# gradslam/gradslam

Measured on AMD Instinct MI355X. Metric: frames/sec PointFusion 640x480 RGB-D, higher is better.
Workload: dtype f32

## Files before the change

gradslam_amd/_C.py:

```python
import ctypes as C
import os

import torch

_HERE = os.path.dirname(os.path.abspath(__file__))
LIB_PATH = os.environ.get("GRADSLAM_HIP_LIB") or os.path.join(_HERE, "csrc", "libgradslam_hip.so")
if os.environ.get("GRADSLAM_HIP_LIB"):
    import warnings
    warnings.warn("GRADSLAM_HIP_LIB overrides the product library: %s" % LIB_PATH, RuntimeWarning)
ABI_VERSION = 3

_lib = None

_vp, _i64, _i32, _f = C.c_void_p, C.c_int64, C.c_int, C.c_float


class IcpParams(C.Structure):
    _fields_ = [("mode", C.c_int), ("numiters", C.c_int), ("damp", C.c_float),
                ("dist_thresh", C.c_float), ("lambda_max", C.c_float), ("B", C.c_float),
                ("B2", C.c_float), ("nu", C.c_float)]


class MapView(C.Structure):
    _fields_ = [("points", C.c_void_p), ("normals", C.c_void_p), ("colors", C.c_void_p), ("ccounts", C.c_void_p),
# ... 31 lines not shown
                ("depth_bar", C.c_void_p), ("color_bar", C.c_void_p), ("normal_bar", C.c_void_p),
                ("confidence_bar", C.c_void_p), ("points_bar", C.c_void_p), ("normals_bar", C.c_void_p),
                ("colors_bar", C.c_void_p), ("ccounts_bar", C.c_void_p), ("poses_bar", C.c_void_p),
                ("scratch", C.c_void_p)]


_PROTOS = {
    "gs_abi_version": [],
    "gs_last_error": [],
    "gs_scratch_bytes": [_i64, _i64],
    "gs_profile_begin": [_i32],
    "gs_profile_end": [],
    "gs_profile_read": [_i32, C.POINTER(C.c_double), C.POINTER(C.c_int64), C.POINTER(C.c_double)],
    "gs_frame_maps_f32": [_vp, _vp, _i32, _i32, _f, _vp, _vp, _vp, _vp, _vp],
    "gs_global_maps_f32": [_vp, _vp, _vp, _vp, _i32, _i32, _vp, _vp, _vp],
    "gs_alpha_f32": [_vp, _i64, _f, _f, _vp, _vp],
    "gs_alpha_backward_f32": [_vp, _i64, _f, _f, _vp, _vp, _vp, _vp],
    "gs_downsample_frame_f32": [_vp, _vp, _vp, _vp, _i32, _i32, _i32, _vp, _vp, _vp, _vp, _vp, _vp],
    "gs_project_map_f32": [_vp, _i64, _vp, _vp, _i32, _i32, _vp, _vp],
    "gs_active_table_i64": [_vp, _i64, _i32, _i64, _vp, _vp, _vp, _vp],
    "gs_select_targets_f32": [_vp, _i64, _i32, _i32, _vp, _vp, _vp, _vp, _vp, _vp, _i64, _vp, _vp, _vp],
    "gs_downsample_table_f32": [_vp, _i64, _i32, _vp, _vp, _vp, _vp, _vp, _vp, _vp, _vp, _vp],
    "gs_knn1_f32": [_vp, _i64, _vp, _i64, _vp, _vp, _vp, _vp],
    "gs_knn1_grid_scratch_bytes": [_i64, _i64],
    "gs_knn1_grid_f32": [_vp, _i64, _vp, _i64, _vp, _vp, _vp, C.POINTER(C.c_int64), _vp],
    "gs_gauss_newton_rows_f32": [_vp, _i64, _vp, _vp, _i64, _f, _vp, _vp, _vp, _vp, _vp, _vp],
    "gs_solve_normal_eq_f32": [_vp, _vp, _vp, _i64, _i32, _f, _vp, _vp],
    "gs_se3_exp_f32": [_vp, _vp, _vp],
    "gs_se3_exp_backward_f32": [_vp, _vp, _vp, _vp],
    "gs_transform_points_f32": [_vp, _i64, _vp, _vp, _vp],
    "gs_icp_scratch_bytes": [_i64, _i64],
    "gs_icp_f32": [_vp, _i64, _vp, _vp, _i64, _vp, _vp, C.POINTER(IcpParams), _vp, _vp, _vp, _vp],
    "gs_icp_trace_f32": [_vp, _i32, _vp, _vp],
    "gs_icp_dc_f32": [_vp, _i64, _vp, _vp, _vp, _i64, _vp, _vp, _vp, C.POINTER(IcpParams), _vp, _vp, _vp, _vp],
    "gs_frame_maps_backward_f32": [_vp, _vp, _i32, _i32, _f, _vp, _vp, _vp, _vp, _vp, _vp, _vp, _vp],
    "gs_frame_maps_backward_kbar_scratch_bytes": [_i32, _i32],
    "gs_global_maps_backward_f32": [_vp, _vp, _vp, _vp, _i32, _i32, _vp, _vp, _vp],
    "gs_downsample_frame_backward_f32": [_vp, _vp, _i32, _i32, _i32, _vp, _vp, _vp],
    "gs_icp_tape_bytes": [_i64, _i32],
    "gs_icp_tape_f32": [_vp, _i64, _vp, _vp, _i64, _vp, _vp, C.POINTER(IcpParams), _vp, _vp, _vp, _vp, _vp],
    "gs_icp_backward_scratch_bytes": [_i64, _i64],
    "gs_icp_backward_f32": [_vp, _vp, _i64, _vp, _vp, _i64, _vp, C.POINTER(IcpParams), _vp, _vp, _vp, _vp, _vp, _vp,
                            _vp],
    "gs_similar_rows_f32": [_vp, _i64, _vp, _vp, _vp, _vp, _i32, _f, _f, _vp, _vp],
    "gs_best_unique_rows_f32": [_vp, _i64, _vp, _vp, _vp, _i32, _i32, _i64, _vp, _vp, _vp, _vp, _vp],
    "gs_associate_f32": [_vp, _i64, _vp, _vp, _vp, _vp, _vp, _i32, _i32, _f, _f, _vp, _vp, _vp, _vp],
    "gs_best_table_i64": [_vp, _i32, _i32, _i64, _vp, _vp, _vp, _vp],
    "gs_rows_to_best_pix": [_vp, _i64, _i32, _i32, _vp, _vp],
    "gs_fuse_append_f32": [_vp, _vp, _vp, _vp, _i64, _i64, _vp, _vp, _vp, _vp, _vp, _vp, _i32, _i32, _i32,
                           _vp, _vp, _vp],
    "gs_append_valid_f32": [_vp, _vp, _vp, _vp, _i64, _i64, _vp, _vp, _vp, _vp, _vp, _i32, _i32, _vp, _vp, _vp],
    "gs_ingest_depth_u16_f32": [_vp, _i32, _i32, _vp, _i32, _i32, C.c_double, _vp],
    "gs_ingest_color_u8_f32": [_vp, _i32, _i32, _vp, _i32, _i32, _i32, _vp],
    "gs_ingest_frames_native_f32": [_vp, _vp, _i64, _i32, _i32, C.c_double, _i32, _vp, _vp, _vp],
    "gs_host_device_pointer": [_vp, C.POINTER(C.c_void_p)],
    "gs_global_maps_pose_backward_scratch_bytes": [_i32, _i32],
    "gs_global_maps_pose_backward_f32": [_vp, _vp, _vp, _vp, _vp, _i32, _i32, _vp, _vp, _vp],
    "gs_fuse_append_backward_f32": [_vp, _vp, _vp, _vp, _i64, _vp, _vp, _vp, _vp, _vp, _vp, _i32, _i32, _i32, _vp, _vp,
                                    _vp, _vp, _i64, _vp, _vp, _vp, _vp, _vp, _vp, _vp, _vp, _vp, _vp],
    "gs_update_map_scratch_bytes": [_i64, _i32, _i32],
    "gs_update_map_fusion_dc_f32": [_vp, _vp, _vp, _vp, _i64, _vp, _i64, _vp, _vp, _vp, _vp, _vp, _vp, _vp, _i32, _i32,
                                    _f, _f, _i32, _vp, _vp, _vp, _vp, _vp, _vp],
    "gs_icp_map_dc_f32": [_vp, _i64, _vp, _vp, _vp, _vp, _i64, _vp, _i32, _i32, _vp, _vp, C.POINTER(IcpParams), _vp, _vp,
                          _vp],
    "gs_lattice_source_f32": [_vp, _vp, _vp, _i32, _i32, _i32, _vp, _vp],
    "gs_relative_pose_f32": [_vp, _vp, _i64, _vp, _vp],
    "gs_project_map_dc_f32": [_vp, _i64, _vp, _vp, _vp, _i32, _i32, _vp, _vp],
    "gs_select_targets_dc_f32": [_vp, _i64, _vp, _i32, _i32, _vp, _vp, _vp, _vp, _vp, _vp, _i64, _vp, _vp, _vp],
    "gs_associate_dc_f32": [_vp, _i64, _vp, _vp, _vp, _vp, _vp, _vp, _i32, _i32, _f, _f, _vp, _vp, _vp, _vp],
    "gs_fuse_append_dc_f32": [_vp, _vp, _vp, _vp, _i64, _vp, _i64, _vp, _vp, _vp, _vp, _vp, _vp, _i32, _i32, _i32,
                              _vp, _vp, _vp],
    "gs_append_valid_dc_f32": [_vp, _vp, _vp, _vp, _i64, _vp, _i64, _vp, _vp, _vp, _vp, _vp, _i32, _i32, _vp, _vp,
                               _vp],
    "gs_frame_maps_batch_f32": [_vp, _i64, _i64, _vp, _i32, _i32, _i32, _i32, _f, _vp, _vp, _vp, _vp],
    "gs_localize_scratch_bytes": [_i32, _i32, _i32, _i64],
    "gs_localize_batch_f32": [C.POINTER(LocalizeSeq), _i32, _i32, _i32, _i32, C.POINTER(IcpParams), _vp],
    "gs_update_map_fusion_batch_f32": [C.POINTER(UpdateSeq), _i32, _i32, _i32, _f, _f, _i32, _vp],
    "gs_project_points_f32": [_vp, _i32, _i64, _vp, _i64, _vp, _vp],
    "gs_unproject_points_f32": [_vp, _i32, _i64, _vp, _i64, _vp, _vp, _vp],
    "gs_lie_small_f32": [_i32, _vp, _vp, _vp],
    "gs_localize_far_stats_i64": [_vp, _i32, _i32, _i32, _i64, C.POINTER(C.c_int64), _vp],
    "gs_localize_list_stats_i64": [_vp, _i32, _i32, _i32, _i64, C.POINTER(C.c_int64), _vp],
    "gs_localize_solve_stats_i64": [_vp, _i32, _i32, _i32, _i64, C.POINTER(C.c_int64), _vp],
    "gs_pointfusion_step_batch_f32": [C.POINTER(StepSeq), _i32, _i32, _i32, _i32, C.POINTER(IcpParams), _f, _f, _f, _i32, _vp],
    "gs_render_scratch_bytes": [_i32, _i32, _i32],
    "gs_render_map_dc_f32": [C.POINTER(RenderSeq), _i32, _i32, _i32, _i32, _i32, _f, _i32, _vp],
    "gs_render_backward_scratch_bytes": [_i32, _i32, _i32, _i64],
    "gs_render_map_backward_dc_f32": [C.POINTER(RenderBackwardSeq), _i32, _i32, _i32, _i32, _i32, _vp],
}
_RESTYPE = {"gs_last_error": C.c_char_p, "gs_scratch_bytes": _i64, "gs_icp_scratch_bytes": _i64,
            "gs_knn1_grid_scratch_bytes": _i64, "gs_update_map_scratch_bytes": _i64, "gs_global_maps_pose_backward_scratch_bytes": _i64, "gs_icp_tape_bytes": _i64, "gs_icp_backward_scratch_bytes": _i64,
            "gs_localize_scratch_bytes": _i64, "gs_frame_maps_backward_kbar_scratch_bytes": _i64,
            "gs_render_scratch_bytes": _i64, "gs_render_backward_scratch_bytes": _i64}
EXPORTS = tuple(_PROTOS)


class HipExtensionError(RuntimeError):
    pass


def lib():
    global _lib
    if _lib is None:
        if not os.path.exists(LIB_PATH):
            raise HipExtensionError(
                "gradslam_amd: %s is missing. Build it with `python -m gradslam_amd.csrc.build` "
                "(hipcc --offload-arch=gfx950). There is no CPU / PyTorch fallback." % LIB_PATH)
        handle = C.CDLL(LIB_PATH)
        for name, argtypes in _PROTOS.items():
            fn = getattr(handle, name)
            fn.argtypes = argtypes
            fn.restype = _RESTYPE.get(name, C.c_int)
        if handle.gs_abi_version() != ABI_VERSION:
            raise HipExtensionError("libgradslam_hip.so ABI %d != expected %d; rebuild"
                                    % (handle.gs_abi_version(), ABI_VERSION))
        _lib = handle
    return _lib


def check(status, what):
    if status != 0:
        raise HipExtensionError("%s failed (code %d): %s" % (what, status, lib().gs_last_error().decode()))


def require_device(*tensors):
    dev = None
    for t in tensors:
        if t is None:
            continue
        if not t.is_cuda:
            raise HipExtensionError(
                "gradslam_amd kernels run on the GPU only (got a %s tensor). Move the data to a HIP "
                "device; there is no CPU fallback." % t.device)
        if not t.is_contiguous():
            raise HipExtensionError("internal error: non-contiguous tensor passed to the HIP library")
        if dev is None:
            dev = t.device
        elif t.device != dev:
            raise HipExtensionError("tensors live on different devices: %s vs %s" % (dev, t.device))
    return dev


def ptr(t):
    return None if t is None else C.c_void_p(t.data_ptr())


def stream(device):
    return C.c_void_p(torch.cuda.current_stream(device).cuda_stream)


class Workspace:
    _instances = {}

    def __init__(self, device):
        self.device = device
        self._bufs = {}

    @classmethod
    def get(cls, device):
        device = torch.device(device)
        if device.index is None:
            device = torch.device("cuda", torch.cuda.current_device())
        key = (device, torch.cuda.current_stream(device).cuda_stream)
        ws = cls._instances.get(key)
        if ws is None:
            ws = cls._instances[key] = Workspace(device)
# ... 20 lines not shown
```

gradslam_amd/csrc/gs_common.h:

```cpp
#pragma once
#include <hip/hip_runtime.h>
#include <atomic>
#include <stdint.h>
#include <stdio.h>

#include "../../include/gradslam_hip.h"

#define GS_ABI_VERSION 3

constexpr int GS_MAX_BATCH = 8;
struct GsClearJob {
  int n;
  size_t bytes;
  char* ptr[GS_MAX_BATCH];
};
constexpr int GS_CLEAR_ITEMS = 8;
struct GsPixelTables {
  int n;
  uint64_t* key_pix[GS_MAX_BATCH];
  int32_t* best_pix[GS_MAX_BATCH];
  int32_t* any_flag[GS_MAX_BATCH];
  int32_t* call_flag;
};
int gs_frame_maps_batch_clear(const float* depth, int64_t depth_stride_seq, int64_t depth_stride_frame, const float* K16,
                              int n_frames, int frames_per_K, int H, int W, float two_sigma_sq, float* vertex,
                              float* normal, float* alpha, const GsClearJob* job, void* stream,
                              const GsPixelTables* tables = nullptr);

int gs_update_map_fusion_batch_impl(const gs_update_seq* seqs_host, int B, int H, int W, float dist_th, float dot_th,
                                    int renorm_all, void* stream, bool tables_ready);
int32_t* gs_update_map_call_flag(void* scratch_of_first_sequence);
void gs_update_map_tables(void* scratch, int32_t** any_flag, uint64_t** key_pix);

void gs_set_error(const char* fmt, ...);

#define GS_REQUIRE(cond, msg)                  \
  do {                                         \
    if (!(cond)) {                             \
      gs_set_error("%s: %s", __func__, msg);   \
      return GS_ERR_INVALID;                   \
    }                                          \
  } while (0)

#define GS_HIP(call)                                                            \
  do {                                                                          \
    hipError_t e_ = (call);                                                     \
    if (e_ != hipSuccess) {                                                     \
      gs_set_error("%s: %s -> %s", __func__, #call, hipGetErrorString(e_));     \
      return GS_ERR_HIP;                                                        \
    }                                                                           \
  } while (0)

#define GS_LAUNCH_CHECK() GS_HIP(hipGetLastError())

static inline hipStream_t gs_stream(void* s) { return reinterpret_cast<hipStream_t>(s); }
static inline int64_t gs_ceil_div(int64_t a, int64_t b) { return (a + b - 1) / b; }
static inline size_t gs_align(size_t x, size_t a = 256) { return (x + a - 1) / a * a; }

enum GsProfKind { GS_PROF_KNN = 0, GS_PROF_LINEARIZE = 1, GS_PROF_FRAME = 2, GS_PROF_PROJECT = 3,
                  GS_PROF_ASSOC = 4, GS_PROF_FUSE = 5, GS_PROF_COMPACT = 6, GS_PROF_SOLVE = 7, GS_PROF_ICP_FUSED = 8,
                  GS_PROF_KINDS = 9 };
extern std::atomic<bool> g_gs_prof_on;
int gs_prof_open(int kind, double work, hipStream_t st, int launches);
void gs_prof_close(int slot, hipStream_t st);
struct GsProf {
  int slot;
  hipStream_t st;
  GsProf(int kind, double work, hipStream_t s, int launches = 1) : slot(-1), st(s) {
    if (g_gs_prof_on) slot = gs_prof_open(kind, work, s, launches);
  }
  ~GsProf() {
    if (slot >= 0) gs_prof_close(slot, st);
  }
};

#define GS_DEV __device__ __forceinline__

GS_DEV float gs_fma(float a, float b, float c) { return __builtin_fmaf(a, b, c); }

GS_DEV float gs_dot3_fma(float a0, float a1, float a2, float b0, float b1, float b2) {
  float acc = a0 * b0;
  acc = gs_fma(a1, b1, acc);
  acc = gs_fma(a2, b2, acc);
  return acc;
}
GS_DEV float gs_dot3_plain(float a0, float a1, float a2, float b0, float b1, float b2) {
  float p0 = a0 * b0, p1 = a1 * b1, p2 = a2 * b2;
  float s = p0 + p1;
  return s + p2;
}
GS_DEV float gs_norm3(float x, float y, float z) {
  float acc = x * x;
  acc = gs_fma(y, y, acc);
  acc = gs_fma(z, z, acc);
  return __builtin_sqrtf(acc);
}

GS_DEV float gs_expf_spec(float x) {
  if (x < -87.0f) return 0.0f;
  if (x > 88.0f) return __builtin_inff();
  float n = __builtin_rintf(x * 1.44269504088896341f);
  float r = gs_fma(-n, 0.693359375f, x);
  r = gs_fma(-n, -2.12194440e-4f, r);
  float p = 1.9875691500e-4f;
  p = gs_fma(p, r, 1.3981999507e-3f);
  p = gs_fma(p, r, 8.3334519073e-3f);
  p = gs_fma(p, r, 4.1665795894e-2f);
  p = gs_fma(p, r, 1.6666665459e-1f);
  p = gs_fma(p, r, 5.0000001201e-1f);
  float r2 = r * r;
  float y = gs_fma(p, r2, r);
  y = y + 1.0f;
  int32_t bits = __float_as_int(y) + (((int32_t)n) << 23);
  return __int_as_float(bits);
}
// ... 86 lines not shown
```

gradslam_amd/csrc/gs_env.h:

```cpp
#pragma once
#include <stdlib.h>
#include <string.h>

struct GsEnv {
  bool icp_lists;
  int icp_lists_from;
  bool icp_wide;
  bool icp_far;
  bool icp_binned_normals;
  float icp_weak_room;
  bool icp_persist;
  bool icp_lanes_set;
  int icp_lanes;
  int icp_blocks_per_cu;
  const char* icp_timeline;
  const char* icp_persist_timeline;
  bool icp_timeline_it_set; int icp_timeline_it;
  int timeline_it(int numiters) const { return icp_timeline_it_set ? icp_timeline_it : numiters - 1; }
  bool knn_brute;
  int knn_spt;
  bool debug_grid;
};

inline const GsEnv& gs_env() {
  static const GsEnv env = [] {
    const auto num = [](const char* name, int unset) { const char* e = getenv(name); return e ? atoi(e) : unset; };
    GsEnv v;
    v.icp_lists = num("GRADSLAM_HIP_ICP_LISTS", 1) != 0;
    v.icp_lists_from = num("GRADSLAM_HIP_ICP_LISTS_FROM", -1);
    v.icp_wide = num("GRADSLAM_HIP_ICP_WIDE", 1) != 0;
    v.icp_far = num("GRADSLAM_HIP_ICP_FAR", 0) != 0;
    v.icp_binned_normals = num("GRADSLAM_HIP_ICP_BINNED_NORMALS", 1) != 0;
    const char* room = getenv("GRADSLAM_HIP_ICP_WEAK_ROOM");
    v.icp_weak_room = room ? (float)atof(room) : 0.0f;
    if (!(v.icp_weak_room >= 0.0f && v.icp_weak_room < 1.0f)) v.icp_weak_room = 0.0f;
    v.icp_persist = num("GRADSLAM_HIP_ICP_PERSIST", 0) == 1;
    v.icp_lanes_set = getenv("GRADSLAM_HIP_ICP_LANES") != nullptr;
    v.icp_lanes = num("GRADSLAM_HIP_ICP_LANES", 0);
    v.icp_blocks_per_cu = num("GRADSLAM_HIP_ICP_BLOCKS_PER_CU", 0);
    v.icp_timeline = getenv("GRADSLAM_HIP_ICP_TIMELINE");
    v.icp_persist_timeline = getenv("GRADSLAM_HIP_ICP_PERSIST_TIMELINE");
    v.icp_timeline_it_set = getenv("GRADSLAM_HIP_ICP_TIMELINE_IT") != nullptr;
    v.icp_timeline_it = num("GRADSLAM_HIP_ICP_TIMELINE_IT", 0);
    const char* knn = getenv("GRADSLAM_HIP_KNN");
    v.knn_brute = knn && strcmp(knn, "brute") == 0;
    v.knn_spt = num("GRADSLAM_HIP_KNN_SPT", 0);
    v.debug_grid = getenv("GRADSLAM_HIP_DEBUG_GRID") != nullptr;
    return v;
  }();
  return env;
}
```

gradslam_amd/csrc/gs_fuse.hip:

```cpp
#include "gs_assoc_dev.h"
#include "gs_compact.h"

__global__ void __launch_bounds__(256) gs_fuse_init_kernel(int32_t* __restrict__ pix_of, int64_t n,
                                                           int32_t* __restrict__ any_flag) {
  const int64_t i = (int64_t)blockIdx.x * 256 + threadIdx.x;
  if (i == 0) *any_flag = 0;
  if (i < n) pix_of[i] = -1;
}

__global__ void __launch_bounds__(256) gs_fuse_scatter_kernel(const int32_t* __restrict__ best_pix,
                                                              int64_t P, GsCount n_map_c,
                                                              int32_t* __restrict__ pix_of,
                                                              int32_t* __restrict__ any_flag) {
  const int64_t p = (int64_t)blockIdx.x * 256 + threadIdx.x;
  if (p >= P) return;
  const int32_t n = best_pix[p];
  if (n >= 0 && n < gs_count(n_map_c)) {
    pix_of[n] = (int32_t)p;
    *any_flag = 1;
  }
}

struct FrameGlobalMaps {
  const float* __restrict__ gvertex;
// ... 313 lines not shown
                                           void* scratch, void* stream) {
  GS_REQUIRE(H > 0 && W > 0 && n_old >= 0 && n_new >= n_old, "bad sizes");
  GS_REQUIRE(best_pix && gvertex && gnormal && rgb && alpha && depth && P_bar && N_bar && C_bar && F_bar && gvertex_bar &&
                 gnormal_bar && rgb_bar && alpha_bar && scratch,
             "NULL pointer");
  hipStream_t st = gs_stream(stream);
  const int64_t P = (int64_t)H * W;
  GS_HIP(hipMemsetAsync(gvertex_bar, 0, 12 * (size_t)P, st));
  GS_HIP(hipMemsetAsync(gnormal_bar, 0, 12 * (size_t)P, st));
  GS_HIP(hipMemsetAsync(rgb_bar, 0, 12 * (size_t)P, st));
  GS_HIP(hipMemsetAsync(alpha_bar, 0, 4 * (size_t)P, st));
  char* base = reinterpret_cast<char*>(scratch) + gs_cp_scratch_bytes(P > n_old ? P : n_old);
  int32_t* any_flag = reinterpret_cast<int32_t*>(base);
  int32_t* pix_of = reinterpret_cast<int32_t*>(base + 256);
  if (n_old > 0) {
    GS_REQUIRE(points && normals && colors && ccounts && old_points_bar && old_normals_bar && old_colors_bar &&
                   old_ccounts_bar,
               "NULL pointer");
    const GsCount n_old_c{n_old, nullptr};
    hipLaunchKernelGGL(gs_fuse_init_kernel, dim3((unsigned)gs_ceil_div(n_old, 256)), dim3(256), 0, st, pix_of, n_old,
                       any_flag);
    hipLaunchKernelGGL(gs_fuse_scatter_kernel, dim3((unsigned)gs_ceil_div(P, 256)), dim3(256), 0, st, best_pix, P,
                       n_old_c, pix_of, any_flag);
    hipLaunchKernelGGL(gs_fuse_bwd_rows_kernel, dim3((unsigned)gs_ceil_div(n_old, 256)), dim3(256), 0, st, points,
                       normals, colors, ccounts, n_old, pix_of, any_flag, gvertex, gnormal, rgb, alpha, renorm_all, P_bar,
                       N_bar, C_bar, F_bar, old_points_bar, old_normals_bar, old_colors_bar, old_ccounts_bar,
                       gvertex_bar, gnormal_bar, rgb_bar, alpha_bar);
    GS_LAUNCH_CHECK();
  }
  EmitAppendBackward emit{P_bar, N_bar, C_bar, F_bar, n_old, gvertex_bar, gnormal_bar, rgb_bar, alpha_bar};
  int64_t* cnt = reinterpret_cast<int64_t*>(base + 128);
  return gs_compact(P, PredNewPixel{depth, best_pix}, emit, cnt, 0, n_new - n_old, scratch, st);
}

constexpr int32_t MU_TIE_MARK = 0x7fffffff;
struct MuSeq {
  float* points; float* normals; float* colors; float* ccounts;
  GsCount n_map;
  int64_t capacity;
  const float* vertex; const float* normal; const float* depth; const float* rgb; const float* alpha;
  const float* pose16; const float* K16;
  float* gvertex; float* gnormal;
  int32_t* best_pix;
  int64_t* new_count_out;
  int32_t* any_flag;
  uint64_t* key_pix;
  int32_t* tile_counts;
  uint64_t* key_pt;
  int32_t* pix;
  int32_t* pix_of;
};
struct MuBatch {
  int B, H, W, renorm_all;
  int64_t P, ntiles;
  float u_hi, v_hi, dist_th, dot_th;
  int32_t* call_flag;
  int zero_call_flag;
  MuSeq s[GS_MAX_BATCH];
};

__global__ void __launch_bounds__(256) gs_mu_pixel_init_kernel(const MuBatch mb) {
  const MuSeq& q = mb.s[blockIdx.x % mb.B];
  const int64_t p = (int64_t)(blockIdx.x / mb.B) * 256 + threadIdx.x;
  if (p == 0) { q.any_flag[0] = 0; q.any_flag[1] = 0; }
  if (blockIdx.x == 0 && threadIdx.x == 0 && mb.zero_call_flag) *mb.call_flag = 0;
  if (p >= mb.P) return;
  float T[12];
#pragma unroll
  for (int i = 0; i < 12; ++i) T[i] = q.pose16[i];
  const float validf = q.depth[p] > 0.0f ? 1.0f : 0.0f;
  float g0, g1, g2;
  gs_rigid_fma(T, q.vertex[3 * p], q.vertex[3 * p + 1], q.vertex[3 * p + 2], g0, g1, g2);
  q.gvertex[3 * p] = g0 * validf;
  q.gvertex[3 * p + 1] = g1 * validf;
  q.gvertex[3 * p + 2] = g2 * validf;
  const float n0 = q.normal[3 * p], n1 = q.normal[3 * p + 1], n2 = q.normal[3 * p + 2];
  q.gnormal[3 * p] = gs_dot3_fma(T[0], T[1], T[2], n0, n1, n2);
  q.gnormal[3 * p + 1] = gs_dot3_fma(T[4], T[5], T[6], n0, n1, n2);
  q.gnormal[3 * p + 2] = gs_dot3_fma(T[8], T[9], T[10], n0, n1, n2);
  q.key_pix[p] = ~0ull;
  q.best_pix[p] = -1;
}

__global__ void __launch_bounds__(256) gs_mu_project_key_kernel(const MuBatch mb) {
  const MuSeq& q = mb.s[blockIdx.x % mb.B];
  const int64_t n = (int64_t)(blockIdx.x / mb.B) * 256 + threadIdx.x;
  if (n >= gs_count(q.n_map)) return;
  const GsCamera c = gs_camera(q.pose16, q.K16);
  const int32_t p = gs_project_point(c, q.points[3 * n], q.points[3 * n + 1], q.points[3 * n + 2], mb.H, mb.W, mb.u_hi,
                                     mb.v_hi);
  int32_t pk = -1;
  if (p >= 0) {
    float fp[3], fn[3];
    if (q.gvertex) FrameGlobalMaps{q.gvertex, q.gnormal}((int64_t)p, fp, fn);
    else frame_local_maps(q.vertex, q.normal, q.pose16)((int64_t)p, fp, fn);
    if (gs_is_similar_v(q.points, q.normals, fp, fn, n, mb.dist_th, mb.dot_th)) {
      const uint64_t k = gs_assoc_key_v(q.points, q.ccounts, fp, n);
      const unsigned long long old = atomicMin(reinterpret_cast<unsigned long long*>(&q.key_pix[p]), (unsigned long long)k);
      if (old == (unsigned long long)k) {
        q.best_pix[p] = MU_TIE_MARK;
        q.any_flag[1] = 1;
      }
      q.key_pt[n] = k;
      pk = p;
    }
  }
  q.pix[n] = pk;
}

GS_DEV void mu_settle_ties(const MuSeq& q, const unsigned blk, const unsigned nblk) {
  if (q.any_flag[1] == 0) return;
  const int64_t n_map = gs_count(q.n_map);
  for (int64_t n = (int64_t)blk * GS_CP_BLOCK + threadIdx.x; n < n_map; n += (int64_t)nblk * GS_CP_BLOCK) {
    const int32_t p = q.pix[n];
    if (p < 0 || q.best_pix[p] == -1) continue;
    if (q.key_pt[n] == q.key_pix[p]) atomicMin(reinterpret_cast<unsigned*>(&q.best_pix[p]), (unsigned)n);
  }
}

__global__ void __launch_bounds__(GS_CP_BLOCK) gs_mu_winner_count_kernel(const MuBatch mb) {
  __shared__ int smem[GS_CP_BLOCK / GS_WAVE + 1];
  const MuSeq& q = mb.s[blockIdx.x % mb.B];
  const unsigned blk = blockIdx.x / mb.B;
  const int64_t base = (int64_t)blk * GS_CP_TILE + (int64_t)threadIdx.x * GS_CP_ITEMS;
  int c = 0;
  uint64_t kk[GS_CP_ITEMS];
  float dd[GS_CP_ITEMS];
#pragma unroll
  for (int i = 0; i < GS_CP_ITEMS; ++i) {
    const int64_t pc = base + i < mb.P ? base + i : mb.P - 1;
    kk[i] = q.key_pix[pc];
    dd[i] = q.depth[pc];
  }
  bool any = false;
#pragma unroll
  for (int i = 0; i < GS_CP_ITEMS; ++i) {
    const int64_t p = base + i;
    if (p < mb.P) {
      const bool matched = kk[i] != ~0ull;
      any = any || matched;
      if (dd[i] > 0.0f && !matched) ++c;
    }
  }
  if (any) {
    q.any_flag[0] = 1;
    *mb.call_flag = 1;
  }
  int total;
  (void)gs_block_excl_scan<GS_CP_BLOCK>(c, smem, &total);
  if (threadIdx.x == 0) q.tile_counts[blk] = total;
  mu_settle_ties(q, blk, gridDim.x / mb.B);
}

GS_DEV void mu_merge_body(const MuBatch& mb, const unsigned bid) {
  const MuSeq& q = mb.s[bid % mb.B];
  const int64_t n = (int64_t)(bid / mb.B) * 256 + threadIdx.x;
  if (n >= gs_count(q.n_map)) return;
  if (*mb.call_flag == 0) return;
  int32_t p = q.pix[n];
  if (p >= 0) {
    bool win = q.key_pt[n] == q.key_pix[p];
    if (win) {
      const int32_t bp = q.best_pix[p];
      win = bp == -1 || bp == (int32_t)n;
      if (win && bp == -1) q.best_pix[p] = (int32_t)n;
    }
    if (!win) p = -1;
  }
  if (p < 0 && !mb.renorm_all) return;
  if (q.gvertex) fuse_merge_row(q.points, q.normals, q.colors, q.ccounts, n, p, FrameGlobalMaps{q.gvertex, q.gnormal}, q.rgb, q.alpha);
  else fuse_merge_row(q.points, q.normals, q.colors, q.ccounts, n, p, frame_local_maps(q.vertex, q.normal, q.pose16), q.rgb, q.alpha);
}

GS_DEV void mu_append_body(const MuBatch& mb, const unsigned bid) {
  __shared__ int smem[GS_CP_BLOCK / GS_WAVE + 1];
  const MuSeq& q = mb.s[bid % mb.B];
  const unsigned blk = bid / mb.B;
  int before = 0, all = 0;
  for (int64_t t = threadIdx.x; t < mb.ntiles; t += GS_CP_BLOCK) {
    const int v = q.tile_counts[t];
    all += v;
    if (t < (int64_t)blk) before += v;
  }
  int tile_prefix, total_new, tile_new;
  (void)gs_block_excl_scan<GS_CP_BLOCK>(before, smem, &tile_prefix);
  (void)gs_block_excl_scan<GS_CP_BLOCK>(all, smem, &total_new);
  const int64_t n_map = gs_count(q.n_map);
  if (blk == 0 && threadIdx.x == 0) q.new_count_out[0] = n_map + total_new;
  const int64_t base = (int64_t)blk * GS_CP_TILE + (int64_t)threadIdx.x * GS_CP_ITEMS;
  bool keep[GS_CP_ITEMS];
  int c = 0;
  {
    uint64_t kk[GS_CP_ITEMS];
    float dd[GS_CP_ITEMS];
#pragma unroll
    for (int i = 0; i < GS_CP_ITEMS; ++i) {
      const int64_t pc = base + i < mb.P ? base + i : mb.P - 1;
      kk[i] = q.key_pix[pc];
      dd[i] = q.depth[pc];
    }
#pragma unroll
    for (int i = 0; i < GS_CP_ITEMS; ++i) {
      keep[i] = base + i < mb.P && dd[i] > 0.0f && kk[i] == ~0ull;
      c += keep[i] ? 1 : 0;
    }
  }
  int w = gs_block_excl_scan<GS_CP_BLOCK>(c, smem, &tile_new);
  __shared__ unsigned short loc_s[GS_CP_TILE];
#pragma unroll
  for (int i = 0; i < GS_CP_ITEMS; ++i) {
    if (keep[i]) loc_s[w++] = (unsigned short)(threadIdx.x * GS_CP_ITEMS + i);
  }
  __syncthreads();
  const int64_t tile_base = (int64_t)blk * GS_CP_TILE;
  if (q.gvertex) {
    const EmitAppend emit{q.points, q.normals, q.colors, q.ccounts, q.n_map, FrameGlobalMaps{q.gvertex, q.gnormal}, q.rgb, q.alpha};
    for (int r = threadIdx.x; r < tile_new; r += GS_CP_BLOCK) {
      const int64_t pos = (int64_t)tile_prefix + r;
      if (n_map + pos < q.capacity) emit(tile_base + loc_s[r], pos);
    }
  } else {
    const EmitAppendT<FrameLocalMaps> emit{q.points, q.normals, q.colors, q.ccounts, q.n_map,
                                           frame_local_maps(q.vertex, q.normal, q.pose16), q.rgb, q.alpha};
    for (int r = threadIdx.x; r < tile_new; r += GS_CP_BLOCK) {
      const int64_t pos = (int64_t)tile_prefix + r;
      if (n_map + pos < q.capacity) emit(tile_base + loc_s[r], pos);
    }
  }
}

static_assert(GS_CP_BLOCK == 256, "merge and append blocks share a launch");
__global__ void __launch_bounds__(256) gs_mu_merge_append_kernel(const MuBatch mb, const unsigned nb_append) {
  if (blockIdx.x < nb_append) mu_append_body(mb, blockIdx.x);
  else mu_merge_body(mb, blockIdx.x - nb_append);
}

extern "C" int64_t gs_update_map_scratch_bytes(int64_t n_map_bound, int H, int W) {
  const int64_t P = (int64_t)H * W;
  return (int64_t)(256 + gs_align(8 * (size_t)P) + gs_align(4 * (size_t)gs_cp_tiles(P)) +
                   gs_align(8 * (size_t)(n_map_bound > 0 ? n_map_bound : 1)) +
                   2 * gs_align(4 * (size_t)(n_map_bound > 0 ? n_map_bound : 1)) + 4096);
}

int32_t* gs_update_map_call_flag(void* scratch0) { return reinterpret_cast<int32_t*>(scratch0) + 32; }
void gs_update_map_tables(void* scratch, int32_t** any_flag, uint64_t** key_pix) {
  *any_flag = reinterpret_cast<int32_t*>(scratch);
  *key_pix = reinterpret_cast<uint64_t*>(reinterpret_cast<char*>(scratch) + 256);
}

static int update_chunk(const gs_update_seq* seqs, int B, int H, int W, float dist_th, float dot_th, int renorm_all,
                        hipStream_t st, int phase, int32_t* call_flag, bool first_chunk, bool tables_ready) {
  MuBatch mb;
  mb.B = B; mb.H = H; mb.W = W; mb.renorm_all = renorm_all;
  mb.call_flag = call_flag; mb.zero_call_flag = first_chunk ? 1 : 0;
  mb.P = (int64_t)H * W;
  mb.ntiles = gs_cp_tiles(mb.P);
  mb.u_hi = (float)((double)W - 0.999); mb.v_hi = (float)((double)H - 0.999);
  mb.dist_th = dist_th; mb.dot_th = dot_th;
  int64_t n_max = 0;
  double bytes_assoc = 0.0, bytes_fuse = 0.0;
  for (int b = 0; b < B; ++b) {
    const gs_update_seq& u = seqs[b];
    const int64_t n_map = u.map.n_bound;
    n_max = n_map > n_max ? n_map : n_max;
    char* q = reinterpret_cast<char*>(u.scratch);
    MuSeq& m = mb.s[b];
    m.points = u.map.points; m.normals = u.map.normals; m.colors = u.map.colors; m.ccounts = u.map.ccounts;
    m.n_map = GsCount{u.map.n_bound, u.map.n_dev};
    m.capacity = u.map.capacity;
    m.vertex = u.vertex; m.normal = u.normal; m.depth = u.depth; m.rgb = u.rgb; m.alpha = u.alpha;
    m.pose16 = u.pose16; m.K16 = u.K16;
    m.gvertex = u.gvertex; m.gnormal = u.gnormal; m.best_pix = u.best_pix; m.new_count_out = u.new_count_out;
    m.any_flag = reinterpret_cast<int32_t*>(q); q += 256;
    m.key_pix = reinterpret_cast<uint64_t*>(q); q += gs_align(8 * (size_t)mb.P);
    m.tile_counts = reinterpret_cast<int32_t*>(q); q += gs_align(4 * (size_t)mb.ntiles);
    m.key_pt = reinterpret_cast<uint64_t*>(q); q += gs_align(8 * (size_t)(n_map > 0 ? n_map : 1));
    m.pix = reinterpret_cast<int32_t*>(q); q += gs_align(4 * (size_t)(n_map > 0 ? n_map : 1));
    m.pix_of = reinterpret_cast<int32_t*>(q);
    bytes_assoc += 72.0 * (double)n_map;
    bytes_fuse += 104.0 * (double)n_map + 49.0 * (double)mb.P;
  }
  const unsigned uB = (unsigned)B;
  const unsigned pb = uB * (unsigned)gs_ceil_div(mb.P, 256), nb = uB * (unsigned)gs_ceil_div(n_max > 0 ? n_max : 1, 256);
  if (phase == 0) {
    if (!tables_ready) {
      GsProf prof(GS_PROF_FRAME, (double)B * (double)mb.P * 64.0, st);
      hipLaunchKernelGGL(gs_mu_pixel_init_kernel, dim3(pb), dim3(256), 0, st, mb);
    }
    if (n_max > 0) {
      GsProf prof(GS_PROF_ASSOC, bytes_assoc, st, 1);
      hipLaunchKernelGGL(gs_mu_project_key_kernel, dim3(nb), dim3(256), 0, st, mb);
    }
    GsProf prof(GS_PROF_FUSE, bytes_fuse / 3.0, st, 1);
    hipLaunchKernelGGL(gs_mu_winner_count_kernel, dim3(uB * (unsigned)mb.ntiles), dim3(GS_CP_BLOCK), 0, st, mb);
  } else {
    GsProf prof(GS_PROF_FUSE, bytes_fuse * (2.0 / 3.0), st, 1);
    const unsigned nb_append = uB * (unsigned)mb.ntiles;
    hipLaunchKernelGGL(gs_mu_merge_append_kernel, dim3(nb_append + (n_max > 0 ? nb : 0u)), dim3(256), 0, st, mb, nb_append);
  }
  GS_LAUNCH_CHECK();
  return GS_OK;
}

int gs_update_map_fusion_batch_impl(const gs_update_seq* seqs_host, int B, int H, int W, float dist_th, float dot_th,
                                    int renorm_all, void* stream, bool tables_ready) {
  GS_REQUIRE(seqs_host && B > 0 && H > 0 && W > 0, "bad arguments");
  GS_REQUIRE((int64_t)H * W < (1ll << 31), "too large for int32 indices");
  for (int b = 0; b < B; ++b) {
    const gs_update_seq& u = seqs_host[b];
    GS_REQUIRE(u.map.n_bound >= 0 && u.map.n_bound < 0x7fffffff, "bad map size");
    GS_REQUIRE(u.map.capacity >= u.map.n_bound + (int64_t)H * W, "capacity must cover n_bound + H*W rows");
    GS_REQUIRE(u.map.points && u.map.normals && u.map.colors && u.map.ccounts && u.vertex && u.normal && u.depth && u.rgb &&
                   u.alpha && u.pose16 && u.K16 && u.best_pix && u.new_count_out && u.scratch,
               "NULL pointer");
    GS_REQUIRE((u.gvertex && u.gnormal) || (tables_ready && !u.gvertex && !u.gnormal), "gvertex / gnormal: both or none");
    GS_REQUIRE(u.new_count_out != u.map.n_dev, "new_count_out must not alias the map's device count");
  }
  hipStream_t st = gs_stream(stream);
  int32_t* call_flag = gs_update_map_call_flag(seqs_host[0].scratch);
  for (int phase = 0; phase < 2; ++phase) {
    for (int c0 = 0; c0 < B; c0 += GS_MAX_BATCH) {
      const int nb = B - c0 < GS_MAX_BATCH ? B - c0 : GS_MAX_BATCH;
      const int rc = update_chunk(seqs_host + c0, nb, H, W, dist_th, dot_th, renorm_all, st, phase, call_flag, c0 == 0,
                                  tables_ready);
      if (rc != GS_OK) return rc;
    }
  }
  return GS_OK;
}

extern "C" int gs_update_map_fusion_batch_f32(const gs_update_seq* seqs_host, int B, int H, int W, float dist_th,
                                              float dot_th, int renorm_all, void* stream) {
  return gs_update_map_fusion_batch_impl(seqs_host, B, H, W, dist_th, dot_th, renorm_all, stream, false);
}

extern "C" int gs_update_map_fusion_dc_f32(float* points, float* normals, float* colors, float* ccounts,
                                           int64_t n_map_bound, const int64_t* n_map_dev, int64_t capacity,
                                           const float* vertex, const float* normal, const float* depth,
                                           const float* rgb, const float* alpha, const float* pose16,
                                           const float* K16, int H, int W, float dist_th, float dot_th,
                                           int renorm_all, float* gvertex, float* gnormal, int32_t* best_pix,
                                           int64_t* new_count_out, void* scratch, void* stream) {
  gs_update_seq u;
  u.map = gs_map_view{points, normals, colors, ccounts, capacity, n_map_bound, n_map_dev};
  u.vertex = vertex; u.normal = normal; u.depth = depth; u.rgb = rgb; u.alpha = alpha;
  u.pose16 = pose16; u.K16 = K16;
  u.gvertex = gvertex; u.gnormal = gnormal; u.best_pix = best_pix; u.new_count_out = new_count_out; u.scratch = scratch;
  return gs_update_map_fusion_batch_f32(&u, 1, H, W, dist_th, dot_th, renorm_all, stream);
}
```

gradslam_amd/csrc/gs_icp_loop.hip:

```cpp
#include <stdlib.h>
#include <string.h>

#include <memory>
#include <mutex>
#include <type_traits>

#include "gs_env.h"
#include "gs_icp_math.h"
#include "gs_knn.h"
#include "gs_knn_bbox.h"

constexpr int GS_ICP_MAX_ITERS = 1024;
struct GsIcpState {
  IcpSmall s[2];
  float trace[GS_ICP_MAX_ITERS * 12];
};

struct TapePtrs {
  float* src;
  int32_t* idx;
  float* sys;
};
GS_DEV void tape_write_sys(float* __restrict__ sys, int it, const double* S, float damp) {
  float* t = sys + 28 * it;
// ... 659 lines not shown
          rr = (double)res * (double)res;
        }
        const double sum = gs_wave_sum_f64(rr);
        if (wl == 0) red2[wave] = sum;
      }
      __syncthreads();
      if (threadIdx.x < NU && u0 + (int)threadIdx.x < u_last)
        partials_out[(int64_t)(u0 + threadIdx.x) * LIN_NV + 27] = red2[2 * threadIdx.x] + red2[2 * threadIdx.x + 1];
      __syncthreads();
      continue;
    }
    for (int w = threadIdx.x; w < NU * FS_RG * LIN_NV; w += FS_BLOCK) {
      const int i = w % LIN_NV, part = (w / LIN_NV) % FS_RG, un = w / (LIN_NV * FS_RG);
      const int ia = fs_pa(i), ib = fs_pb(i);
      const float* r0 = qa_s[un * FS_QPB + FS_RPG * part];
      double t = (double)r0[ia] * (double)r0[ib];
#pragma unroll
      for (int u = 1; u < FS_RPG; ++u) t += (double)r0[8 * u + ia] * (double)r0[8 * u + ib];
      sub_s[un][part][i] = t;
    }
    __syncthreads();
    if (threadIdx.x < NU * LIN_NV) {
      const int i = threadIdx.x % LIN_NV, un = threadIdx.x / LIN_NV;
      if (u0 + un < u_last) {
        double t = sub_s[un][0][i];
#pragma unroll
        for (int k = 1; k < FS_RG; ++k) t += sub_s[un][k][i];
        partials_out[(int64_t)(u0 + un) * LIN_NV + i] = t;
      }
    }
    __syncthreads();
  } while (!LISTS && (u0 += NU) < u_last);
}

struct IcpHalfBatch {
  int B;
  int upb;
  float weak_room;
  unsigned long long* timeline;
  IcpHalfSeq s[GS_MAX_BATCH];
  IcpHalfLists l[GS_MAX_BATCH];
  IcpHalfWide w[GS_MAX_BATCH];
};
template <bool FULL, int G, bool FAR, int LMODE>
__global__ void __launch_bounds__(FS_BLOCK, 6) gs_icp_half_batch_kernel(const IcpHalfBatch hb, GsCount n_src_c,
                                                                        float dist_thresh, gs_icp_params prm, int it,
                                                                        int rows_in_reduced) {
  const unsigned B = (unsigned)hb.B, blk = blockIdx.x / B, nblk = gridDim.x / B;
  const unsigned X = (GS_XCDS % B == 0) ? GS_XCDS / B : 1u;
#ifdef GS_ICP_TIMELINE
  unsigned long long t0 = 0;
  if (hb.timeline && threadIdx.x == 0) t0 = wall_clock64();
#endif
  icp_half_body<FULL, G, FAR, LMODE>(hb.s[blockIdx.x % B], hb.l[blockIdx.x % B], hb.w[blockIdx.x % B], n_src_c, dist_thresh, prm, it, rows_in_reduced,
                                     gs_xcd_block(blk, nblk, X), hb.upb,
                                     hb.timeline ? hb.timeline + 72 * (size_t)blockIdx.x : nullptr, hb.weak_room);
#ifdef GS_ICP_TIMELINE
  if (hb.timeline && threadIdx.x == 0) {
    unsigned long long* r = hb.timeline + 72 * (size_t)blockIdx.x;
    r[0] = t0;
    r[1] = wall_clock64();
  }
#endif
}

#include "gs_icp_persist.h"

static size_t icp_rows(int64_t n_src) { return (size_t)gs_ceil_div(n_src, FS_QPB); }

struct IcpDevice { int cus = 256; bool ps_fits = false; };
static IcpDevice icp_device() {
  constexpr int MAX_DEV = 64;
  static IcpDevice facts[MAX_DEV]; static std::once_flag asked[MAX_DEV];
  int dev = 0;
  if (hipGetDevice(&dev) != hipSuccess || dev < 0 || dev >= MAX_DEV) return IcpDevice{};
  std::call_once(asked[dev], [dev] {
    int v = 0; hipDeviceProp_t p;
    if (hipDeviceGetAttribute(&v, hipDeviceAttributeMultiprocessorCount, dev) == hipSuccess && v > 0) facts[dev].cus = v;
    facts[dev].ps_fits = hipGetDeviceProperties(&p, dev) == hipSuccess && strncmp(p.gcnArchName, "gfx950", 6) == 0 &&
                         p.multiProcessorCount == (int)(GS_XCDS * PS_CUS_PER_XCD);
  });
  return facts[dev];
}

struct IcpHalfPlan { int G, nb, upb; };
static IcpHalfPlan icp_half_plan(const GsEnv& env, int cus, int64_t n_src, int B, int g_max = 8) {
  const int forced = env.icp_lanes;
  const int nunits = (int)icp_rows(n_src);
  int share = env.icp_blocks_per_cu;
  if (share <= 0) {
    const int NU2 = FS_BLOCK / 2 / FS_QPB;
    share = (nunits + NU2 - 1) / NU2 <= cus / B ? 1 : 2;
  }
  const int budget = (share * cus) / B > 0 ? (share * cus) / B : 1;
  IcpHalfPlan pl{2, 1, 1};
  for (int G = g_max; G >= 2; G >>= 1) {
    const int NU = FS_BLOCK / G / FS_QPB, need = (nunits + NU - 1) / NU;
    if ((forced == 0 && need <= budget) || forced == G || (forced == 0 && G == 2) || (forced > g_max && G == g_max)) {
      pl.G = G;
      pl.nb = need <= budget ? need : budget;
      pl.upb = NU * ((nunits + NU * pl.nb - 1) / (NU * pl.nb));
      pl.nb = (nunits + pl.upb - 1) / pl.upb;
      break;
    }
  }
  return pl;
}

#include "gs_icp_timeline.h"

template <bool FULL>
static void icp_half_launch(const IcpHalfPlan& pl, IcpHalfBatch& hb, GsCount n_src_c, const gs_icp_params* prm, int it,
                            int rows_in_reduced, hipStream_t st, int lmode = 0) {
  hb.upb = pl.upb;
  hb.timeline = icp_tl_arm(FULL, hb.B * pl.nb, it, prm->numiters, st);
  const dim3 grid((unsigned)(hb.B * pl.nb)), block(FS_BLOCK);
  const bool far = hb.s[0].far_cq != nullptr;
#define GS_HALF_LAUNCH(G_, FAR_, LMODE_)                                                                               \
  hipLaunchKernelGGL((gs_icp_half_batch_kernel<FULL, G_, FAR_, LMODE_>), grid, block, 0, st, hb, n_src_c,              \
                     prm->dist_thresh, *prm, it, rows_in_reduced)
#define GS_HALF_LAUNCH_L(G_)                                                 \
  do {                                                                       \
    if (lmode == 2) GS_HALF_LAUNCH(G_, false, 2);                            \
    else if (lmode == 1) GS_HALF_LAUNCH(G_, false, 1);                       \
    else if (lmode == 3 && G_ == 2) GS_HALF_LAUNCH(2, false, 3);             \
    else GS_HALF_LAUNCH(G_, false, 0);                                       \
  } while (0)
  if (pl.G == 8) GS_HALF_LAUNCH_L(8);
  else if (pl.G == 4) { if (far) GS_HALF_LAUNCH(4, true, 0); else GS_HALF_LAUNCH_L(4); }
  else { if (far) GS_HALF_LAUNCH(2, true, 0); else GS_HALF_LAUNCH_L(2); }
#undef GS_HALF_LAUNCH_L
#undef GS_HALF_LAUNCH
  if (hb.timeline && !FULL) icp_tl_dump(hb, pl, lmode, st);
  hb.timeline = nullptr;
}

constexpr int FS_REDUCE_ROWS = 1024;
__global__ void __launch_bounds__(FS_BLOCK) gs_icp_reduce_rows_kernel(const double* __restrict__ partials_in,
                                                                      GsCount n_src_c, double* __restrict__ row_out) {
  __shared__ double S[32];
  __shared__ double sub[FS_BLOCK / 32][32];
  const int nrows = (int)((gs_count(n_src_c) + FS_QPB - 1) / FS_QPB);
  icp_sum_rows<FS_BLOCK>(partials_in, nrows, S, sub);
  if (threadIdx.x < LIN_NV) row_out[threadIdx.x] = S[threadIdx.x];
}

__global__ void __launch_bounds__(FS_BLOCK) gs_icp_finish_kernel(const double* __restrict__ partials_in, GsCount n_src_c,
                                                                 GsIcpState* __restrict__ st, int buf,
                                                                 gs_icp_params prm, const float* __restrict__ compose16,
                                                                 float* __restrict__ out_T16) {
  __shared__ double red[FS_BLOCK / GS_WAVE];
  const int nrows_in = (int)((gs_count(n_src_c) + FS_QPB - 1) / FS_QPB);
  const double e1 = icp_sum_col27<FS_BLOCK>(partials_in, nrows_in, red);
  if (threadIdx.x != 0) return;
  IcpSmall sm = st->s[buf];
  const int it = prm.numiters - 1;
  icp_update_math((float)e1, sm, prm, it < GS_ICP_MAX_ITERS ? st->trace + 12 * it : nullptr);
  st->s[buf ^ 1] = sm;
  icp_write_result(sm, compose16, out_T16);
}

constexpr int LIN_BLOCK = 256;
constexpr int SUM_BLOCK = 1024;

template <bool FULL>
__global__ void __launch_bounds__(LIN_BLOCK) gs_icp_linearize_kernel(
// ... 74 lines not shown
                                                                  GsIcpState* __restrict__ st, gs_icp_params prm,
                                                                  int it, const float* __restrict__ compose16,
                                                                  float* __restrict__ out_T16) {
  __shared__ double red[SUM_BLOCK / GS_WAVE];
  const double e1 = icp_sum_col27<SUM_BLOCK>(partials, nrows, red);
  if (threadIdx.x != 0) return;
  IcpSmall sm = st->s[0];
  icp_update_math((float)e1, sm, prm, it < GS_ICP_MAX_ITERS ? st->trace + 12 * it : nullptr);
  st->s[0] = sm;
  if (it == prm.numiters - 1) icp_write_result(sm, compose16, out_T16);
}

__global__ void gs_icp_init_kernel(GsIcpState* __restrict__ st, const float* __restrict__ init16, float damp,
                                   int numiters, const float* __restrict__ compose16, float* __restrict__ out_T16) {
  if (threadIdx.x != 0) return;
  IcpSmall sm;
  for (int i = 0; i < 16; ++i) {
    sm.T_total[i] = init16[i];
    sm.T_step[i] = init16[i];
    sm.Tr[i] = (i % 5 == 0) ? 1.0f : 0.0f;
  }
  for (int i = 0; i < 8; ++i) sm.xi[i] = 0.0f;
  sm.damp = damp;
  sm.err = 0.0f;
  sm.pad[0] = sm.pad[1] = 0.0f;
  st->s[0] = sm;
  st->s[1] = sm;
  if (numiters == 0) icp_write_result(sm, compose16, out_T16);
}

template <class T>
static T* gs_at(void* base, size_t offset) { return reinterpret_cast<T*>(reinterpret_cast<char*>(base) + offset); }
struct GsTake { size_t end = 0; size_t operator()(size_t n) { end += n; return end - n; } };

constexpr int ICP_ROWRED_DOUBLES = 32;
struct IcpLayout { size_t state, rowred, sync, best, srcA, srcB, partials[2], grid, total; };
static IcpLayout icp_layout(int64_t n_src, int64_t n_tgt) {
  GsTake take;
  IcpLayout L;
  L.state = take(gs_align(sizeof(GsIcpState)));
  L.rowred = take(gs_align(sizeof(double) * ICP_ROWRED_DOUBLES));
  L.sync = L.rowred + sizeof(double) * LIN_NV;
  static_assert(8 * ICP_ROWRED_DOUBLES >= 8 * LIN_NV + 4 * PS_WORDS, "the sync record does not fit behind rowred + LIN_NV");
  L.best = take(gs_align(8 * (size_t)n_src));
  L.srcA = take(gs_align(12 * (size_t)n_src)); L.srcB = take(gs_align(12 * (size_t)n_src));
  for (int k = 0; k < 2; ++k) L.partials[k] = take(gs_align(sizeof(double) * LIN_NV * icp_rows(n_src)));
  L.grid = take(gs_knn_grid_scratch_bytes(n_src, n_tgt));
  L.total = take.end + 4096;
  return L;
}
struct IcpScratch {
  GsIcpState* state;
  double* rowred;
  unsigned* sync;
  unsigned long long* best; float *srcA, *srcB;
  double* partials[2]; void* grid;
};
static IcpScratch icp_carve(void* p, const IcpLayout& L) {
  return IcpScratch{gs_at<GsIcpState>(p, L.state), gs_at<double>(p, L.rowred), gs_at<unsigned>(p, L.sync),
                    gs_at<unsigned long long>(p, L.best), gs_at<float>(p, L.srcA), gs_at<float>(p, L.srcB),
                    {gs_at<double>(p, L.partials[0]), gs_at<double>(p, L.partials[1])}, gs_at<void>(p, L.grid)};
}

extern "C" int64_t gs_icp_scratch_bytes(int64_t n_src, int64_t n_tgt) { return (int64_t)icp_layout(n_src < 1 ? 1 : n_src, n_tgt).total; }

static int icp_tape_finish(void* tape, const GsIcpState* state, int64_t n_src, int numiters, hipStream_t st) {
  GsIcpTape t = gs_icp_tape_carve(tape, n_src, numiters);
  if (numiters > 0)
    GS_HIP(hipMemcpyAsync(t.trace, state->trace, sizeof(float) * 12 * (size_t)numiters, hipMemcpyDeviceToDevice, st));
  return GS_OK;
}

static double icp_alg_bytes(int numiters, int64_t n_slots, int64_t n_queries, int64_t n_binned) {
  const double rows = (double)gs_ceil_div(n_slots, FS_QPB);
  const double full = 12.0 * n_slots + 36.0 * n_queries + 8.0 * LIN_NV * rows + 16.0 * n_binned;
  const double look = 12.0 * n_slots + 24.0 * n_queries + 8.0 * rows + 16.0 * n_binned;
  return (double)numiters * (full + look);
}

static int icp_run(const float* src, int64_t n_src, const float* tgt, const float* tgt_normals,
                   int64_t n_tgt, const float* init16, const float* compose16,
                   const gs_icp_params* prm, float* out_T16, int64_t* out_idx, void* icp_scratch,
                   void* tape, void* stream, const int64_t* n_src_dev = nullptr,
                   const int64_t* n_tgt_dev = nullptr, GsTargetFilter flt = GsTargetFilter{nullptr, 1, 1}) {
  GS_REQUIRE(prm, "params_host must not be NULL");
  GS_REQUIRE(n_src > 0 && n_tgt > 0, "empty point set");
  GS_REQUIRE(n_tgt < 0x7fffffffll && n_src < 0x7fffffffll, "too many points");
  GS_REQUIRE(src && tgt && tgt_normals && init16 && out_T16 && icp_scratch, "NULL pointer");
  GS_REQUIRE(prm->numiters >= 0 && prm->numiters <= GS_ICP_MAX_ITERS, "numiters must be in [0, 1024]");
  GS_REQUIRE(prm->mode == 0 || prm->mode == 1, "mode must be 0 (ICP) or 1 (gradICP)");
  hipStream_t st = gs_stream(stream);
  IcpScratch sc = icp_carve(icp_scratch, icp_layout(n_src, n_tgt));
  hipLaunchKernelGGL(gs_icp_init_kernel, dim3(1), dim3(64), 0, st, sc.state, init16, prm->damp, prm->numiters,
                     compose16, out_T16);
  const bool dev_counts = n_src_dev || n_tgt_dev || flt.pix;
  const bool use_grid = prm->numiters > 0 && (dev_counts || (!gs_env().knn_brute && gs_knn_use_grid(n_src, n_tgt)));
  const GsCount n_src_c{n_src, n_src_dev}, n_tgt_c{n_tgt, n_tgt_dev};
  float* bufs[2] = {sc.srcA, sc.srcB};
  TapePtrs tp = {nullptr, nullptr, nullptr};
  if (tape) {
    GsIcpTape t = gs_icp_tape_carve(tape, n_src, prm->numiters);
    tp.src = t.src; tp.idx = t.idx; tp.sys = t.sys;
  }
  auto cloud = [&](int it) { return tp.src ? tp.src + (size_t)it * 3 * (size_t)n_src : bufs[it & 1]; };
  auto tidx = [&](int it, int which) { return tp.idx ? tp.idx + ((size_t)it * 2 + which) * (size_t)n_src : nullptr; };

  if (use_grid) {
    int rc = gs_knn_grid_build(tgt, n_tgt_c, n_src, sc.grid, st, flt, tgt_normals);
    if (rc != GS_OK) return rc;
    GridMem gm = grid_carve(sc.grid, n_src, n_tgt);
    const int nfs = (int)icp_rows(n_src);
    const bool reduce_rows = nfs > FS_REDUCE_ROWS;
    const float* cur_in = src;
    int h = 0;
    double prof_bytes = 0.0;
    if (g_gs_prof_on) {
      int64_t n_binned = n_tgt;
      if (flt.pix) {
        unsigned hits = 0;
        GS_HIP(hipMemcpyAsync(&hits, gm.bbox + 6, 4, hipMemcpyDeviceToHost, st));
        GS_HIP(hipStreamSynchronize(st));
        n_binned = hits;
      }
      prof_bytes = icp_alg_bytes(prm->numiters, n_src, n_src, n_binned);
    }
    std::unique_ptr<GsProf> prof_loop(new GsProf(GS_PROF_ICP_FUSED, prof_bytes, st, 2 * prm->numiters));
    const IcpHalfPlan plan = icp_half_plan(gs_env(), icp_device().cus, n_src, 1);
    IcpHalfBatch hb;
    hb.B = 1;
    hb.weak_room = 0.0f;
    hb.l[0] = IcpHalfLists{nullptr, nullptr, nullptr, nullptr};
    hb.w[0] = IcpHalfWide{nullptr, nullptr};
    for (int it = 0; it < prm->numiters; ++it) {
      float* cur = cloud(it);
      hb.s[0] = IcpHalfSeq{cur_in, cur, tgt, tgt_normals, n_tgt_c, gm.g, gm.cell_start, gm.sorted, gm.sorted_n,
                           reinterpret_cast<float*>(sc.best), sc.partials[(h + 1) & 1], sc.partials[h & 1], &sc.state->s[h & 1], &sc.state->s[(h + 1) & 1],
                           sc.state->trace, out_idx, tidx(it, 0), nullptr};
      icp_half_launch<true>(plan, hb, n_src_c, prm, it, 0, st);
      ++h;
      if (reduce_rows) {
        GsProf prof(GS_PROF_SOLVE, 1.0, st);
        hipLaunchKernelGGL(gs_icp_reduce_rows_kernel, dim3(1), dim3(FS_BLOCK), 0, st, sc.partials[(h + 1) & 1], n_src_c,
                           sc.rowred);
      }
      hb.s[0] = IcpHalfSeq{cur, nullptr, tgt, tgt_normals, n_tgt_c, gm.g, gm.cell_start, gm.sorted, gm.sorted_n,
                           reinterpret_cast<float*>(sc.best), reduce_rows ? sc.rowred : sc.partials[(h + 1) & 1], sc.partials[h & 1], &sc.state->s[h & 1],
                           &sc.state->s[(h + 1) & 1], sc.state->trace, nullptr, tidx(it, 1), tp.sys};
      icp_half_launch<false>(plan, hb, n_src_c, prm, it, reduce_rows ? 1 : 0, st);
      ++h;
      cur_in = cur;
    }
    prof_loop.reset();
    if (prm->numiters > 0) {
      GsProf prof(GS_PROF_SOLVE, 1.0, st);
      hipLaunchKernelGGL(gs_icp_finish_kernel, dim3(1), dim3(FS_BLOCK), 0, st, sc.partials[(h + 1) & 1], n_src_c,
                         sc.state, h & 1, *prm, compose16, out_T16);
    }
    GS_LAUNCH_CHECK();
    if (tape) return icp_tape_finish(tape, sc.state, n_src, prm->numiters, st);
    return GS_OK;
  }

  GS_HIP(hipMemsetAsync(sc.best, 0xff, 8 * (size_t)n_src, st));
  const int nblk = (int)gs_ceil_div(n_src, LIN_BLOCK);
  double* partials = sc.partials[0];
  const float* cur_in = src;
  for (int it = 0; it < prm->numiters; ++it) {
    float* cur = cloud(it);
    gs_knn_brute_launch(cur_in, sc.state->s[0].T_step, cur, n_src, tgt, n_tgt, sc.best, st);
    {
      GsProf prof(GS_PROF_LINEARIZE, 44.0 * (double)n_src, st);
      hipLaunchKernelGGL((gs_icp_linearize_kernel<true>), dim3(nblk), dim3(LIN_BLOCK), 0, st, cur, nullptr, n_src,
                         tgt, tgt_normals, n_tgt, sc.best, prm->dist_thresh, partials, out_idx, tidx(it, 0));
    }
    {
      GsProf prof(GS_PROF_SOLVE, 1.0, st);
      hipLaunchKernelGGL(gs_icp_solve_kernel, dim3(1), dim3(SUM_BLOCK), 0, st, partials, nblk, sc.state, it, tp.sys);
    }
    gs_knn_brute_launch(cur, sc.state->s[0].Tr, nullptr, n_src, tgt, n_tgt, sc.best, st);
    {
      GsProf prof(GS_PROF_LINEARIZE, 44.0 * (double)n_src, st);
      hipLaunchKernelGGL((gs_icp_linearize_kernel<false>), dim3(nblk), dim3(LIN_BLOCK), 0, st, cur,
                         sc.state->s[0].Tr, n_src, tgt, tgt_normals, n_tgt, sc.best, prm->dist_thresh, partials,
                         nullptr, tidx(it, 1));
    }
    {
      GsProf prof(GS_PROF_SOLVE, 1.0, st);
      hipLaunchKernelGGL(gs_icp_update_kernel, dim3(1), dim3(SUM_BLOCK), 0, st, partials, nblk, sc.state, *prm, it,
                         compose16, out_T16);
    }
    cur_in = cur;
  }
  GS_LAUNCH_CHECK();
  if (tape) return icp_tape_finish(tape, sc.state, n_src, prm->numiters, st);
  return GS_OK;
}

extern "C" int gs_icp_f32(const float* src, int64_t n_src, const float* tgt, const float* tgt_normals,
                          int64_t n_tgt, const float* init16, const float* compose16,
                          const gs_icp_params* prm, float* out_T16, int64_t* out_idx, void* icp_scratch,
                          void* stream) {
  return icp_run(src, n_src, tgt, tgt_normals, n_tgt, init16, compose16, prm, out_T16, out_idx, icp_scratch, nullptr,
                 stream);
}

extern "C" int gs_icp_dc_f32(const float* src, int64_t n_src_bound, const int64_t* n_src_dev, const float* tgt,
                             const float* tgt_normals, int64_t n_tgt_bound, const int64_t* n_tgt_dev,
                             const float* init16, const float* compose16, const gs_icp_params* prm, float* out_T16,
                             int64_t* out_idx, void* icp_scratch, void* stream) {
  return icp_run(src, n_src_bound, tgt, tgt_normals, n_tgt_bound, init16, compose16, prm, out_T16, out_idx,
                 icp_scratch, nullptr, stream, n_src_dev, n_tgt_dev);
}

extern "C" int gs_icp_map_dc_f32(const float* src, int64_t n_src_bound, const int64_t* n_src_dev,
                                 const float* map_points, const float* map_normals, const int32_t* pix,
                                 int64_t n_map_bound, const int64_t* n_map_dev, int W, int ds, const float* init16,
                                 const float* compose16, const gs_icp_params* prm, float* out_T16,
                                 void* icp_scratch, void* stream) {
  GS_REQUIRE(pix && W > 0 && ds > 0, "bad target filter");
  return icp_run(src, n_src_bound, map_points, map_normals, n_map_bound, init16, compose16, prm, out_T16, nullptr,
                 icp_scratch, nullptr, stream, n_src_dev, n_map_dev, GsTargetFilter{pix, W, ds});
}


struct LocSeq {
  const float* vertex;
  const float* depth;
  const float* pose16;
  float* lattice;
  GsIcpState* state;
  float* out_pose16;
  char* clear_ptr;
  int64_t* n_valid;
  int* far_n;
  int* lstat;
  float4* wl_cq;
  unsigned* sync;
};
struct LocBatch {
  int B, W, ds, Wl;
  int64_t n_lat;
  size_t clear_bytes;
  float damp;
  int numiters;
  int count_valid;
  LocSeq s[GS_MAX_BATCH];
};
constexpr int LP_CLEAR_ITEMS = 8;

GS_DEV void loc_prep_block(const LocBatch& lb, const unsigned bid, const unsigned nb_lat) {
  const LocSeq& q = lb.s[bid % lb.B];
  const unsigned blk = bid / lb.B;
  if (blk < nb_lat) {
    const int64_t e = (int64_t)blk * 256 + threadIdx.x;
    int valid = 0;
    if (e < lb.n_lat) {
      const int64_t p = (e / lb.Wl) * lb.ds * (int64_t)lb.W + (e % lb.Wl) * lb.ds;
      float g0 = __builtin_nanf(""), g1 = g0, g2 = g0;
      if (q.depth[p] > 0.0f) {
        float T[12];
#pragma unroll
        for (int i = 0; i < 12; ++i) T[i] = q.pose16[i];
        gs_rigid_fma(T, q.vertex[3 * p], q.vertex[3 * p + 1], q.vertex[3 * p + 2], g0, g1, g2);
        valid = 1;
      }
      q.lattice[3 * e] = g0; q.lattice[3 * e + 1] = g1; q.lattice[3 * e + 2] = g2;
      if (q.wl_cq) q.wl_cq[e] = make_float4(0.0f, 0.0f, 0.0f, 0.0f);
    }
    const unsigned long long m = lb.count_valid ? __ballot(valid) : 0ull;
    if ((threadIdx.x & 63) == 0 && m) atomicAdd(reinterpret_cast<unsigned long long*>(q.n_valid), (unsigned long long)__popcll(m));
    if (blk == 0 && threadIdx.x == 0) {
      IcpSmall sm;
      for (int i = 0; i < 16; ++i) {
        const float id = (i % 5 == 0) ? 1.0f : 0.0f;
        sm.T_total[i] = id; sm.T_step[i] = id; sm.Tr[i] = id;
      }
      for (int i = 0; i < 8; ++i) sm.xi[i] = 0.0f;
      sm.damp = lb.damp;
      sm.err = 0.0f;
      sm.pad[0] = sm.pad[1] = 0.0f;
      q.state->s[0] = sm;
      q.state->s[1] = sm;
      if (q.far_n)
        for (int i = 0; i < FS_FAR_PASSES; ++i) q.far_n[i] = 0;
      if (q.lstat)
        for (int i = 0; i < 3 * GL_STAT_LAUNCHES; ++i) q.lstat[i] = 0;
      if (q.sync)
        for (int i = 0; i < PS_WORDS; ++i) q.sync[i] = 0u;
      if (lb.numiters == 0) icp_write_result(sm, q.pose16, q.out_pose16);
    }
    return;
  }
  float4* dst = reinterpret_cast<float4*>(q.clear_ptr);
  const size_t n16 = lb.clear_bytes / 16;
  const size_t base = (size_t)(blk - nb_lat) * 256 * LP_CLEAR_ITEMS + threadIdx.x;
#pragma unroll
  for (int u = 0; u < LP_CLEAR_ITEMS; ++u) {
    const size_t i = base + (size_t)u * 256;
    if (i < n16) dst[i] = make_float4(0.0f, 0.0f, 0.0f, 0.0f);
  }
}
__global__ void __launch_bounds__(256) gs_loc_prep_kernel(const LocBatch lb, unsigned nb_lat) {
  loc_prep_block(lb, blockIdx.x, nb_lat);
}
static_assert(GB_BLOCK == 256, "lattice and bbox blocks share a launch");
__global__ void __launch_bounds__(256) gs_loc_prep_bbox_kernel(const LocBatch lb, const GsGridBatch gb, const unsigned nb_lat,
                                                               const float u_hi, const float v_hi) {
  const unsigned n_prep = (unsigned)lb.B * nb_lat;
  if (blockIdx.x < n_prep) loc_prep_block(lb, blockIdx.x, nb_lat);
  else gridb_bbox_block(gb, blockIdx.x - n_prep, u_hi, v_hi);
}

struct IcpRowsBatch {
  int B;
  const double* in[GS_MAX_BATCH];
  double* out[GS_MAX_BATCH];
};
__global__ void __launch_bounds__(FS_BLOCK) gs_icp_reduce_rows_batch_kernel(const IcpRowsBatch rb, GsCount n_src_c) {
  __shared__ double S[32];
  __shared__ double sub[FS_BLOCK / 32][32];
  const int nrows = (int)((gs_count(n_src_c) + FS_QPB - 1) / FS_QPB);
  icp_sum_rows<FS_BLOCK>(rb.in[blockIdx.x], nrows, S, sub);
  if (threadIdx.x < LIN_NV) rb.out[blockIdx.x][threadIdx.x] = S[threadIdx.x];
}

struct IcpFinishBatch {
  int B;
  const double* partials_in[GS_MAX_BATCH];
  GsIcpState* st[GS_MAX_BATCH];
  const float* compose16[GS_MAX_BATCH];
  float* out_T16[GS_MAX_BATCH];
  unsigned* sync[GS_MAX_BATCH];
  int nb, h0;
};
__global__ void __launch_bounds__(FS_BLOCK) gs_icp_finish_batch_kernel(const IcpFinishBatch fb, GsCount n_src_c, int buf,
                                                                       gs_icp_params prm) {
  __shared__ double red[FS_BLOCK / GS_WAVE];
  const int b = blockIdx.x;
  const int nrows_in = (int)((gs_count(n_src_c) + FS_QPB - 1) / FS_QPB);
  const double e1 = icp_sum_col27<FS_BLOCK>(fb.partials_in[b], nrows_in, red);
  if (threadIdx.x != 0) return;
  GsIcpState* st = fb.st[b];
  IcpSmall sm = st->s[buf];
  const int it = prm.numiters - 1;
  icp_update_math((float)e1, sm, prm, it < GS_ICP_MAX_ITERS ? st->trace + 12 * it : nullptr);
  st->s[buf ^ 1] = sm;
  icp_write_result(sm, fb.compose16[b], fb.out_T16[b]);
  if (unsigned* sy = fb.sync[b]) {
    const unsigned arrived = sy[PS_ARRIVED], want = (unsigned)fb.nb * (unsigned)(2 * prm.numiters - fb.h0);
    if (!(sy[PS_ERROR] == 0u && arrived == want && sy[PS_TICKET] >= (unsigned)fb.nb))
      for (int i = 0; i < 16; ++i) fb.out_T16[b][i] = __builtin_nanf("");
    sy[PS_NB] = (unsigned)fb.nb;
    sy[PS_H0] = (unsigned)fb.h0;
  }
}

static int64_t loc_lattice(int H, int W, int ds) { return (int64_t)((H + ds - 1) / ds) * ((W + ds - 1) / ds); }

struct ListMem {
  float4* lq;
  uint32_t* ls;
  int* stat;
};

struct FarMem {
  uint32_t* c;
  float4* cq;
  int* idx;
  int* n;
};

struct FarBuildSeq {
  const float* src;
  const int* idx;
  const int* n;
  const GsGrid* gp;
  const int* cell_start;
  const float4* sorted;
  float* d2prev;
  FarMem m;
};
struct FarBuildBatch {
  int B;
  FarBuildSeq s[GS_MAX_BATCH];
};
constexpr int FAR_BLOCK = 512;
constexpr int FAR_BLOCKS_PER_SEQ = 64;
__global__ void __launch_bounds__(FAR_BLOCK) gs_icp_far_build_kernel(const FarBuildBatch fb) {
  const FarBuildSeq& q = fb.s[blockIdx.x % fb.B];
  const int blk = (int)(blockIdx.x / fb.B);
  const int n = *q.n;
  if (blk >= n) return;
  constexpr int NG = FAR_BLOCK / FS_HG;
  __shared__ float qs[NG][3];
  __shared__ float d1_s[NG];
  __shared__ uint8_t flag_s[NG];
  __shared__ int unres_q[NG], sq_s[NG];
  __shared__ int unres_n;
  __shared__ uint32_t stage_s[NG][GS_FAR_SLOTS + 4];
  const GsGrid g = *q.gp;
  const int grp = threadIdx.x / FS_HG, l16 = threadIdx.x & (FS_HG - 1);
  for (int base = blk; base < n; base += FAR_BLOCKS_PER_SEQ * NG) {
    if (threadIdx.x == 0) unres_n = 0;
    __syncthreads();
    const int e = base + grp * FAR_BLOCKS_PER_SEQ;
    if (e < n) {
      const int sq = q.idx[e];
      const float hx = q.src[3 * (int64_t)sq], hy = q.src[3 * (int64_t)sq + 1], hz = q.src[3 * (int64_t)sq + 2];
      const float4 found = q.m.cq[sq];
      const float d1 = sqrtf(found.x);
      const int kdone = (int)found.y;
      if (kdone >= 0) {
        const float R = far_emit_cube<FS_HG>(g, q.cell_start, q.sorted, hx, hy, hz, l16, d1, kdone, stage_s[grp],
                                             reinterpret_cast<int*>(&stage_s[grp][GS_FAR_SLOTS]));
        for (int u = l16; u < GS_FAR_SLOTS; u += FS_HG) q.m.c[GS_FAR_SLOTS * (int64_t)sq + u] = stage_s[grp][u];
        if (l16 == 0) {
          q.m.cq[sq] = make_float4(hx, hy, hz, R);
          if (R > 0.0f) q.d2prev[sq] = __uint_as_float(__float_as_uint(q.d2prev[sq]) | 0x80000000u);
        }
      } else if (l16 == 0) {
        qs[grp][0] = hx; qs[grp][1] = hy; qs[grp][2] = hz;
        d1_s[grp] = d1;
        sq_s[grp] = sq;
        unres_q[atomicAdd(&unres_n, 1)] = grp;
      }
    }
    __syncthreads();
    const int nun = unres_n;
    for (int u = 0; u < nun; u += FS_BQ) {
      const int nq = nun - u < FS_BQ ? nun - u : FS_BQ;
      block_brute_collect_multi<FAR_BLOCK, FS_BQ>(qs, unres_q + u, nq, q.sorted, q.cell_start[g.ncell], d1_s,
                                                  GS_FAR_RADD * g.c, sq_s, q.m.cq, q.m.c, flag_s);
      if ((int)threadIdx.x < nq) {
        const int gq = unres_q[u + threadIdx.x];
        const int s2 = sq_s[gq];
        if (flag_s[gq]) q.d2prev[s2] = __uint_as_float(__float_as_uint(q.d2prev[s2]) | 0x80000000u);
      }
    }
    __syncthreads();
  }
}

static int64_t loc_rows(const gs_map_view& m) { return m.capacity > m.n_bound ? m.capacity : m.n_bound; }

struct LocLayout {
  int64_t n_lat, rows;
  IcpLayout sc;
  size_t lattice, pix, n_valid, icp, lq, ls, lstat, far_c, far_cq, far_idx, far_n, far_out4, total;
};
static LocLayout loc_layout(int64_t n_lat, int64_t rows) {
  GsTake take;
  LocLayout L;
  L.n_lat = n_lat; L.rows = rows > 0 ? rows : 1;
  L.lattice = take(gs_align(12 * (size_t)n_lat));
  L.pix = take(gs_align(4 * (size_t)L.rows));
  L.n_valid = take(256);
  L.sc = icp_layout(n_lat, L.rows);
  L.icp = take(L.sc.total);
  L.lq = take(gs_align(16 * (size_t)n_lat));
  L.ls = take(gs_align(4 * GL_SLOTS * (size_t)n_lat));
  L.lstat = take(gs_align(4 * 3 * GL_STAT_LAUNCHES));
  L.far_c = take(gs_align(4 * GS_FAR_SLOTS * (size_t)n_lat));
  L.far_cq = take(gs_align(16 * (size_t)n_lat));
  L.far_idx = take(gs_align(4 * FS_FAR_PASSES * (size_t)n_lat));
  L.far_n = take(256);
  L.far_out4 = L.far_n + 4 * 8;
  static_assert(FS_FAR_PASSES <= 8, "the far-list counters run into the result words");
  L.total = take.end;
  return L;
}
static bool loc_lists_fit(const LocLayout& L) { return L.total - (L.icp + L.sc.partials[1]) >= sizeof(double) * LIN_NV * FS_BLOCK; }

extern "C" int64_t gs_localize_scratch_bytes(int H, int W, int ds, int64_t n_map_bound) {
  if (H < 1 || W < 1 || ds < 1) return 0;
  return (int64_t)loc_layout(loc_lattice(H, W, ds), n_map_bound).total;
}

struct LocCarve {
  float* lattice; int32_t* pix; int64_t* n_valid;
  IcpScratch sc; GridMem gm; ListMem lm;
  FarMem fm; int* far_out4;
};
static LocCarve loc_carve(void* p, const LocLayout& L) {
  const IcpScratch sc = icp_carve(gs_at<char>(p, L.icp), L.sc);
  return LocCarve{gs_at<float>(p, L.lattice), gs_at<int32_t>(p, L.pix), gs_at<int64_t>(p, L.n_valid), sc,
                  grid_carve(sc.grid, L.n_lat, L.rows),
                  ListMem{gs_at<float4>(p, L.lq), gs_at<uint32_t>(p, L.ls), gs_at<int>(p, L.lstat)},
                  FarMem{gs_at<uint32_t>(p, L.far_c), gs_at<float4>(p, L.far_cq), gs_at<int>(p, L.far_idx), gs_at<int>(p, L.far_n)},
                  gs_at<int>(p, L.far_out4)};
}
static LocCarve loc_carve_of(const void* scratch, int H, int W, int ds, int64_t map_rows) {
  return loc_carve(const_cast<void*>(scratch), loc_layout(loc_lattice(H, W, ds), map_rows));
}

struct IcpEnginePlan {
  bool far_on, wide_on, lists_on, persist_on;
  bool binned_normals;
  bool reduce_rows;
  int lists_from;
  IcpHalfPlan half;
  int ps_it0, ps_nb, ps_upb;
  float weak_room;
  int lmode(int it, bool look_ahead) const {
    if (!lists_on || it < lists_from) return 0;
    if (it > lists_from) return 2;
    return look_ahead ? (persist_on ? 3 : 1) : 0;
  }
};
static IcpEnginePlan icp_engine_plan(const GsEnv& env, const IcpDevice& dev, int B, int64_t n_lat, int numiters,
                                     const LocLayout* layouts) {
  IcpEnginePlan p;
  const int64_t rows = (int64_t)icp_rows(n_lat);
  p.binned_normals = env.icp_binned_normals; p.weak_room = env.icp_weak_room;
  p.lists_from = env.icp_lists_from >= 0 ? env.icp_lists_from : FS_LISTS_FROM;
  p.reduce_rows = rows > FS_REDUCE_ROWS;
  p.far_on = env.icp_far && numiters > 0;
  p.wide_on = env.icp_wide && !p.far_on && numiters > 0;
  p.ps_upb = (int)gs_ceil_div(rows, PS_CUS_PER_XCD);
  p.ps_nb = (int)gs_ceil_div(rows, p.ps_upb > 0 ? p.ps_upb : 1);
  const bool persist_asked = env.icp_persist && env.icp_lists && !p.far_on && B <= (int)GS_XCDS && p.ps_upb <= PS_UPB &&
                             numiters > p.lists_from + 1 && !env.icp_timeline && !env.icp_lanes_set && dev.ps_fits &&
                             p.binned_normals;
  p.half = icp_half_plan(env, dev.cus, n_lat, B, p.far_on ? 4 : (persist_asked ? 2 : 8));
  p.lists_on = env.icp_lists && !p.far_on && p.half.upb * p.half.G * FS_QPB <= FS_BLOCK;
  for (int b = 0; b < B && p.lists_on; ++b) p.lists_on = loc_lists_fit(layouts[b]);
  p.persist_on = persist_asked && p.half.G == 2 && p.lists_on;
  p.ps_it0 = p.persist_on ? p.lists_from + 1 : numiters;
  return p;
}

static void loc_bind(const gs_localize_seq* seqs, int B, int H, int W, int ds, const gs_icp_params* prm,
                     const IcpEnginePlan& plan, LocCarve* c, LocBatch& lb, GsGridBatch& gb) {
  lb.B = gb.B = B; lb.W = gb.W = W; gb.H = H; lb.ds = gb.ds = ds;
  lb.Wl = (W + ds - 1) / ds; lb.n_lat = loc_lattice(H, W, ds); lb.damp = prm->damp; lb.numiters = prm->numiters;
  gb.cells_cap = gs_knn_grid_cells_cap(lb.n_lat);
  for (int b = 0; b < B; ++b) {
    const gs_localize_seq& q = seqs[b];
    if (!plan.binned_normals) c[b].gm.sorted_n = nullptr;
    lb.s[b] = LocSeq{q.vertex, q.depth, q.prev_pose16, c[b].lattice, c[b].sc.state, q.out_pose16,
                     reinterpret_cast<char*>(c[b].gm.g), c[b].n_valid, c[b].fm.n, c[b].lm.stat,
                     plan.wide_on ? c[b].fm.cq : nullptr, c[b].sc.sync};
    gb.s[b] = GsGridSeq{q.map.points, GsCount{q.map.n_bound, q.map.n_dev}, c[b].pix, q.prev_pose16, q.K16,
                        plan.binned_normals ? q.map.normals : nullptr, c[b].gm};
  }
  lb.count_valid = g_gs_prof_on ? 1 : 0;
  lb.clear_bytes = gs_knn_grid_clear_bytes(c[0].gm, gb.cells_cap);
}

static int loc_prep(const gs_localize_seq* seqs, const LocBatch& lb, const GsGridBatch& gb, hipStream_t st, bool grid_cleared) {
  const int B = lb.B;
  if (g_gs_prof_on)
    for (int b = 0; b < B; ++b) GS_HIP(hipMemsetAsync(lb.s[b].n_valid, 0, 8, st));
  const unsigned nb_lat = (unsigned)gs_ceil_div(lb.n_lat, 256);
  const unsigned nb_clear = (unsigned)gs_ceil_div((int64_t)(lb.clear_bytes / 16), 256 * LP_CLEAR_ITEMS);
  double bytes = 0.0;
  for (int b = 0; b < B; ++b) bytes += 28.0 * lb.n_lat + 24.0 * seqs[b].map.n_bound + 16.0 * gb.cells_cap;
  GsProf prof(GS_PROF_COMPACT, bytes, st, grid_cleared ? 4 : 5);
  if (grid_cleared) {
    const float u_hi = (float)((double)gb.W - 0.999), v_hi = (float)((double)gb.H - 0.999);
    hipLaunchKernelGGL(gs_loc_prep_bbox_kernel, dim3((unsigned)B * nb_lat + gs_knn_gridb_bbox_blocks(gb)), dim3(256), 0, st,
                       lb, gb, nb_lat, u_hi, v_hi);
    return gs_knn_grid_build_batch(gb, st, true);
  }
  hipLaunchKernelGGL(gs_loc_prep_kernel, dim3((unsigned)B * (nb_lat + nb_clear)), dim3(256), 0, st, lb, nb_lat);
  return gs_knn_grid_build_batch(gb, st);
}

static int loc_prof_bytes(int B, const LocCarve* c, int64_t n_lat, int numiters, hipStream_t st, double* bytes) {
  for (int b = 0; b < B; ++b) {
    unsigned hits = 0; int64_t nv = 0;
    GS_HIP(hipMemcpyAsync(&hits, c[b].gm.bbox + 6, 4, hipMemcpyDeviceToHost, st));
    GS_HIP(hipMemcpyAsync(&nv, c[b].n_valid, 8, hipMemcpyDeviceToHost, st));
    GS_HIP(hipStreamSynchronize(st));
    *bytes += icp_alg_bytes(numiters, n_lat, nv, hits);
  }
  return GS_OK;
}

static void loc_half_iterations(const gs_localize_seq* seqs, int B, const IcpEnginePlan& plan, const LocCarve* c,
                                int64_t n_lat, const gs_icp_params* prm, hipStream_t st) {
  const GsCount n_src_c{n_lat, nullptr};
  const FarMem no_far{nullptr, nullptr, nullptr, nullptr};
  IcpHalfBatch hb;
  hb.B = B; hb.weak_room = plan.weak_room;
  for (int it = 0; it < plan.ps_it0; ++it) {
    int h = 2 * it;
    for (int b = 0; b < B; ++b) {
      const gs_localize_seq& q = seqs[b];
      const IcpScratch& sc = c[b].sc; const GridMem& gm = c[b].gm;
      const FarMem& fm = plan.far_on ? c[b].fm : no_far;
      const float* cur_in = it == 0 ? c[b].lattice : (((it - 1) & 1) ? sc.srcB : sc.srcA);
      float* cur = (it & 1) ? sc.srcB : sc.srcA;
      hb.s[b] = IcpHalfSeq{cur_in, cur, q.map.points, q.map.normals, GsCount{q.map.n_bound, q.map.n_dev}, gm.g,
                           gm.cell_start, gm.sorted, gm.sorted_n, reinterpret_cast<float*>(sc.best),
                           sc.partials[(h + 1) & 1], sc.partials[h & 1], &sc.state->s[h & 1], &sc.state->s[(h + 1) & 1],
                           sc.state->trace, nullptr, nullptr, nullptr, fm.cq, fm.c, fm.idx, fm.n};
      hb.w[b] = plan.wide_on ? IcpHalfWide{c[b].fm.cq, c[b].fm.c} : IcpHalfWide{nullptr, nullptr};
      hb.l[b] = plan.lists_on ? IcpHalfLists{c[b].lm.lq, c[b].lm.ls, c[b].lm.stat, sc.sync + PS_WEAK}
                              : IcpHalfLists{nullptr, nullptr, nullptr, nullptr};
    }
    icp_half_launch<true>(plan.half, hb, n_src_c, prm, it, 0, st, plan.lmode(it, false));
    if (plan.far_on && fs_far_pass(it) >= 0) {
      const int fp = fs_far_pass(it);
      FarBuildBatch fbb; fbb.B = B;
      for (int b = 0; b < B; ++b)
        fbb.s[b] = FarBuildSeq{(it & 1) ? c[b].sc.srcB : c[b].sc.srcA, c[b].fm.idx + (int64_t)fp * n_lat, c[b].fm.n + fp,
                               c[b].gm.g, c[b].gm.cell_start, c[b].gm.sorted, reinterpret_cast<float*>(c[b].sc.best), c[b].fm};
      hipLaunchKernelGGL(gs_icp_far_build_kernel, dim3((unsigned)B * FAR_BLOCKS_PER_SEQ), dim3(FAR_BLOCK), 0, st, fbb);
    }
    ++h;
    if (plan.reduce_rows) {
      IcpRowsBatch rb; rb.B = B;
      for (int b = 0; b < B; ++b) { rb.in[b] = c[b].sc.partials[(h + 1) & 1]; rb.out[b] = c[b].sc.rowred; }
      hipLaunchKernelGGL(gs_icp_reduce_rows_batch_kernel, dim3((unsigned)B), dim3(FS_BLOCK), 0, st, rb, n_src_c);
    }
    for (int b = 0; b < B; ++b) {
      const IcpScratch& sc = c[b].sc;
      IcpHalfSeq& u = hb.s[b];
      u.src_in = (it & 1) ? sc.srcB : sc.srcA; u.src_out = nullptr;
      u.partials_in = plan.reduce_rows ? sc.rowred : sc.partials[(h + 1) & 1];
      u.partials_out = sc.partials[h & 1];
      u.st_in = &sc.state->s[h & 1]; u.st_out = &sc.state->s[(h + 1) & 1];
    }
    icp_half_launch<false>(plan.half, hb, n_src_c, prm, it, plan.reduce_rows ? 1 : 0, st, plan.lmode(it, true));
  }
// ... 67 lines not shown
  GS_REQUIRE((int64_t)H * W < (1ll << 31), "image too large for int32 pixel ids");
  for (int b = 0; b < B; ++b) {
    const gs_localize_seq& q = seqs_host[b];
    GS_REQUIRE(q.vertex && q.depth && q.K16 && q.prev_pose16 && q.out_pose16 && q.scratch, "NULL pointer");
    GS_REQUIRE(q.map.points && q.map.normals && q.map.n_bound > 0 && q.map.n_bound < 0x7fffffffll,
               "every sequence needs a non-empty map (points + normals)");
    GS_REQUIRE(q.map.capacity <= 0 || q.map.n_bound <= q.map.capacity, "map.n_bound exceeds map.capacity");
  }
  hipStream_t st = gs_stream(stream);
  for (int c0 = 0; c0 < B; c0 += GS_MAX_BATCH) {
    const int nb = B - c0 < GS_MAX_BATCH ? B - c0 : GS_MAX_BATCH;
    const int rc = localize_chunk(seqs_host + c0, nb, H, W, ds, prm, st, grid_cleared);
    if (rc != GS_OK) return rc;
  }
  return GS_OK;
}
extern "C" int gs_localize_batch_f32(const gs_localize_seq* seqs_host, int B, int H, int W, int ds,
                                     const gs_icp_params* prm, void* stream) {
  return localize_batch(seqs_host, B, H, W, ds, prm, stream, false);
}

__global__ void __launch_bounds__(256) gs_far_stats_kernel(const int* __restrict__ far_idx, const int* __restrict__ far_n,
                                                          const float* __restrict__ d2prev, const float4* __restrict__ far_cq,
                                                          int64_t n_lat, int* __restrict__ out4) {
  const int n0 = far_n[0], n = n0 < 0 ? 0 : (n0 > (int)n_lat ? (int)n_lat : n0);
  if (blockIdx.x == 0 && threadIdx.x == 0) { out4[0] = n; out4[2] = far_n[1]; }
  int c = 0, built = 0;
  for (int i = blockIdx.x * 256 + threadIdx.x; i < n; i += gridDim.x * 256) {
    const int s = far_idx[i];
    if (s < 0 || s >= (int)n_lat) continue;
    c += (__float_as_uint(d2prev[s]) >> 31) ? 1 : 0;
    built += far_cq[s].w > 0.0f ? 1 : 0;
  }
  if (c) atomicAdd(&out4[1], c);
  if (built) atomicAdd(&out4[3], built);
}
extern "C" int gs_localize_far_stats_i64(const void* scratch, int H, int W, int ds, int64_t map_rows, int64_t* out4_host,
                                         void* stream) {
  GS_REQUIRE(scratch && out4_host && H > 0 && W > 0 && ds > 0 && map_rows > 0, "bad arguments");
  const int64_t n_lat = loc_lattice(H, W, ds);
  const LocCarve cv = loc_carve_of(scratch, H, W, ds, map_rows);
  const FarMem& fm = cv.fm; hipStream_t st = gs_stream(stream);
  int* out4 = cv.far_out4;
  GS_HIP(hipMemsetAsync(out4, 0, 16, st));
  hipLaunchKernelGGL(gs_far_stats_kernel, dim3(64), dim3(256), 0, st, fm.idx, fm.n, reinterpret_cast<const float*>(cv.sc.best),
                     fm.cq, n_lat, out4);
  int h[4] = {0, 0, 0, 0};
  GsGrid g;
  GS_HIP(hipMemcpyAsync(h, out4, 16, hipMemcpyDeviceToHost, st));
  GS_HIP(hipMemcpyAsync(&g, cv.gm.g, sizeof(g), hipMemcpyDeviceToHost, st));
  GS_HIP(hipStreamSynchronize(st));
  for (int i = 0; i < 4; ++i) out4_host[i] = h[i];
  if (gs_env().debug_grid)
    fprintf(stderr, "grid: box (%.3f %.3f %.3f)-(%.3f %.3f %.3f) c %.4f cells %d x %d x %d = %d\n", g.ox, g.oy, g.oz, g.mx,
            g.my, g.mz, g.c, g.nx, g.ny, g.nz, g.ncell);
  return GS_OK;
}

extern "C" int gs_localize_list_stats_i64(const void* scratch, int H, int W, int ds, int64_t map_rows, int64_t* out192_host,
                                          void* stream) {
  GS_REQUIRE(scratch && out192_host && H > 0 && W > 0 && ds > 0 && map_rows > 0, "bad arguments");
  const ListMem lm = loc_carve_of(scratch, H, W, ds, map_rows).lm;
  int h[3 * GL_STAT_LAUNCHES];
  hipStream_t st = gs_stream(stream);
  GS_HIP(hipMemcpyAsync(h, lm.stat, sizeof(h), hipMemcpyDeviceToHost, st));
  GS_HIP(hipStreamSynchronize(st));
  for (int i = 0; i < 3 * GL_STAT_LAUNCHES; ++i) out192_host[i] = h[i];
  return GS_OK;
}

extern "C" int gs_localize_solve_stats_i64(const void* scratch, int H, int W, int ds, int64_t map_rows, int64_t* out8_host,
                                           void* stream) {
  GS_REQUIRE(scratch && out8_host && H > 0 && W > 0 && ds > 0 && map_rows > 0, "bad arguments");
  const LocCarve cv = loc_carve_of(scratch, H, W, ds, map_rows);
  unsigned h[PS_WORDS];
  hipStream_t st = gs_stream(stream);
  GS_HIP(hipMemcpyAsync(h, cv.sc.sync, sizeof(h), hipMemcpyDeviceToHost, st));
  GS_HIP(hipStreamSynchronize(st));
  static_assert(PS_WORDS == 8, "out8");
  for (int i = 0; i < PS_WORDS; ++i) out8_host[i] = h[i];
  return GS_OK;
}

extern "C" int gs_pointfusion_step_batch_f32(const gs_step_seq* seqs_host, int B, int H, int W, int ds,
                                             const gs_icp_params* prm, float two_sigma_sq, float dist_th, float dot_th,
                                             int renorm_all, void* stream) {
  GS_REQUIRE(seqs_host && prm && B > 0 && H > 0 && W > 0 && ds > 0, "bad arguments");
  const int64_t P = (int64_t)H * W;
  const gs_step_seq& s0 = seqs_host[0];
  const int64_t dstride = B > 1 ? seqs_host[1].depth - s0.depth : P;
  for (int b = 0; b < B; ++b) {
    const gs_step_seq& q = seqs_host[b];
    GS_REQUIRE(q.depth && q.rgb && q.K16 && q.prev_pose16 && q.out_pose16 && q.vertex && q.normal && q.alpha &&
                   q.best_pix && q.new_count_out && q.loc_scratch && q.upd_scratch, "NULL pointer");
    GS_REQUIRE((q.gvertex != nullptr) == (q.gnormal != nullptr) && (q.gvertex != nullptr) == (s0.gvertex != nullptr),
               "gvertex / gnormal: both or none, the same choice for every sequence");
    GS_REQUIRE(q.out_pose16 != q.prev_pose16, "out_pose16 must not alias prev_pose16");
    GS_REQUIRE(q.vertex == s0.vertex + 3 * P * b && q.normal == s0.normal + 3 * P * b && q.alpha == s0.alpha + P * b,
               "vertex / normal / alpha of the batch must be dense");
    GS_REQUIRE(q.depth == s0.depth + dstride * b && q.K16 == s0.K16 + 16 * (int64_t)b, "depth / K16 must be equally strided");
  }
  GS_REQUIRE(dstride >= P || B == 1, "overlapping depth images");
  const bool implicit_global = s0.gvertex == nullptr;
  std::unique_ptr<gs_update_seq[]> us(new gs_update_seq[B]);
  for (int c0 = 0; c0 < B; c0 += GS_MAX_BATCH) {
    const int nb = B - c0 < GS_MAX_BATCH ? B - c0 : GS_MAX_BATCH;
    const gs_step_seq* sq = seqs_host + c0;
    gs_localize_seq ls[GS_MAX_BATCH];
    for (int b = 0; b < nb; ++b) {
      const gs_step_seq& q = sq[b];
      ls[b].vertex = q.vertex; ls[b].depth = q.depth; ls[b].K16 = q.K16; ls[b].prev_pose16 = q.prev_pose16;
      ls[b].map = q.map; ls[b].out_pose16 = q.out_pose16; ls[b].scratch = q.loc_scratch;
      gs_update_seq& u = us[c0 + b];
      u.map = q.map; u.vertex = q.vertex; u.normal = q.normal; u.depth = q.depth; u.rgb = q.rgb;
      u.alpha = q.alpha; u.pose16 = q.out_pose16; u.K16 = q.K16; u.gvertex = q.gvertex;
      u.gnormal = q.gnormal; u.best_pix = q.best_pix; u.new_count_out = q.new_count_out;
      u.scratch = q.upd_scratch;
    }
    GsClearJob job;
    job.n = nb;
    for (int b = 0; b < nb; ++b) {
      GS_REQUIRE(ls[b].map.points && ls[b].map.n_bound > 0, "every sequence needs a non-empty map");
      const LocCarve cv = loc_carve_of(ls[b].scratch, H, W, ds, loc_rows(ls[b].map));
      job.ptr[b] = reinterpret_cast<char*>(cv.gm.g);
      if (b == 0) job.bytes = gs_knn_grid_clear_bytes(cv.gm, gs_knn_grid_cells_cap(loc_lattice(H, W, ds)));
    }
    GsPixelTables tabs{};
    tabs.n = implicit_global ? nb : 0;
    tabs.call_flag = c0 == 0 ? gs_update_map_call_flag(seqs_host[0].upd_scratch) : nullptr;
    for (int b = 0; b < tabs.n; ++b) {
      gs_update_map_tables(sq[b].upd_scratch, &tabs.any_flag[b], &tabs.key_pix[b]);
      tabs.best_pix[b] = sq[b].best_pix;
    }
    int rc = gs_frame_maps_batch_clear(sq[0].depth, dstride, P, sq[0].K16, nb, 1, H, W, two_sigma_sq, sq[0].vertex,
                                       sq[0].normal, sq[0].alpha, &job, stream, &tabs);
    if (rc != GS_OK) return rc;
    rc = localize_batch(ls, nb, H, W, ds, prm, stream, true);
    if (rc != GS_OK) return rc;
  }
  return gs_update_map_fusion_batch_impl(us.get(), B, H, W, dist_th, dot_th, renorm_all, stream, implicit_global);
}

extern "C" int64_t gs_icp_tape_bytes(int64_t n_src, int numiters) { return (int64_t)gs_icp_tape_size(n_src, numiters); }

extern "C" int gs_icp_tape_f32(const float* src, int64_t n_src, const float* tgt, const float* tgt_normals,
                               int64_t n_tgt, const float* init16, const float* compose16,
                               const gs_icp_params* prm, float* out_T16, int64_t* out_idx, void* icp_scratch,
                               void* tape, void* stream) {
  GS_REQUIRE(tape, "tape must not be NULL");
  return icp_run(src, n_src, tgt, tgt_normals, n_tgt, init16, compose16, prm, out_T16, out_idx, icp_scratch, tape,
                 stream);
}

extern "C" int gs_icp_trace_f32(const void* icp_scratch, int numiters, float* trace_out, void* stream) {
  GS_REQUIRE(icp_scratch && trace_out && numiters >= 0 && numiters <= GS_ICP_MAX_ITERS, "bad arguments");
  const GsIcpState* st = reinterpret_cast<const GsIcpState*>(icp_scratch);
  GS_HIP(hipMemcpyAsync(trace_out, st->trace, sizeof(float) * 12 * (size_t)numiters, hipMemcpyDeviceToDevice,
                        gs_stream(stream)));
  return GS_OK;
}
```

gradslam_amd/csrc/gs_knn.h:

```cpp
#pragma once
#include "gs_common.h"

GS_DEV unsigned long long knn_pack(float d, uint32_t idx) {
  return ((unsigned long long)__float_as_uint(d) << 32) | (unsigned long long)idx;
}

int gs_knn_brute_launch(const float* src_in, const float* Tapply, float* src_out, int64_t n_src,
                        const float* tgt, int64_t n_tgt, unsigned long long* best, hipStream_t st);

constexpr int GS_GRID_MAXCELL = 1 << 22;
constexpr int GS_GRID_RINGS = 3;
constexpr int GS_GRID_TILE = 1024;

struct GsGrid {
  float ox, oy, oz;
  float mx, my, mz;
  float c, inv_c;
  int nx, ny, nz, ncell;
};

struct GsTargetFilter {
  const int32_t* pix;
  int W, ds;
};
GS_DEV bool gs_is_target(const GsTargetFilter& f, int64_t n) {
  if (!f.pix) return true;
  const int32_t p = f.pix[n];
  return p >= 0 && ((p / f.W) % f.ds == 0) && ((p % f.W) % f.ds == 0);
}

struct GridMem {
  GsGrid* g;
  unsigned* bbox;
  int* unres_count;
  int* cell_count;
  int* cell_start;
  int* tile_sums;
  float4* sorted;
  float4* sorted_n;
  float4* tlist;
  int* unres_list;
};

static inline GridMem grid_carve(void* scratch, int64_t n_src, int64_t n_tgt) {
  char* p = reinterpret_cast<char*>(scratch);
  GridMem m;
  m.g = reinterpret_cast<GsGrid*>(p); p += 128;
  m.bbox = reinterpret_cast<unsigned*>(p); p += 128;
  m.unres_count = reinterpret_cast<int*>(p); p += 256;
  m.tile_sums = reinterpret_cast<int*>(p); p += gs_align(4 * (size_t)(GS_GRID_MAXCELL / GS_GRID_TILE + 2));
  m.cell_count = reinterpret_cast<int*>(p); p += gs_align(4 * (size_t)(GS_GRID_MAXCELL + 1));
  m.cell_start = reinterpret_cast<int*>(p); p += gs_align(4 * (size_t)(GS_GRID_MAXCELL + 1));
  m.sorted = reinterpret_cast<float4*>(p); p += gs_align(16 * (size_t)(n_tgt > 0 ? n_tgt : 1));
  m.sorted_n = reinterpret_cast<float4*>(p); p += gs_align(16 * (size_t)(n_tgt > 0 ? n_tgt : 1));
  m.tlist = reinterpret_cast<float4*>(p); p += gs_align(16 * (size_t)(n_tgt > 0 ? n_tgt : 1));
  m.unres_list = reinterpret_cast<int*>(p);
  (void)n_src;
  return m;
}

size_t gs_knn_grid_scratch_bytes(int64_t n_src, int64_t n_tgt);

struct GsGridSeq {
  const float* tgt;
  GsCount n_tgt;
  int32_t* pix;
  const float* pose16;
  const float* K16;
  const float* nrm;
  GridMem m;
};
struct GsGridBatch {
  int B, H, W, ds;
  int cells_cap;
  GsGridSeq s[GS_MAX_BATCH];
};
int gs_knn_grid_cells_cap(int64_t n_src);
size_t gs_knn_grid_clear_bytes(const GridMem& m, int cells_cap);
int gs_knn_grid_build_batch(const GsGridBatch& gb, hipStream_t st, bool bbox_done = false);

int gs_knn_grid_build(const float* tgt, GsCount n_tgt, int64_t n_src, void* grid_scratch, hipStream_t st,
                      GsTargetFilter filter = GsTargetFilter{nullptr, 1, 1}, const float* nrm = nullptr);
int gs_knn_grid_query(const float* src_in, const float* Tapply, float* src_out, int64_t n_src,
                      const float* tgt, int64_t n_tgt, unsigned long long* best, void* grid_scratch,
                      hipStream_t st);
static inline bool gs_knn_use_grid(int64_t n_src, int64_t n_tgt) { return n_tgt >= 2048 && n_src >= 256; }

GS_DEV int grid_axis(float v, float o, float inv_c, int n) {
  const float f = (v - o) * inv_c;
  return f >= 0.0f ? (f < (float)n ? (int)f : n - 1) : 0;
}
GS_DEV int grid_cell(const GsGrid& g, float x, float y, float z) {
  const int ix = grid_axis(x, g.ox, g.inv_c, g.nx);
  const int iy = grid_axis(y, g.oy, g.inv_c, g.ny);
  const int iz = grid_axis(z, g.oz, g.inv_c, g.nz);
  return (iz * g.ny + iy) * g.nx + ix;
}

constexpr int GQ_G = 8;
constexpr int GL_RING_NF = 2;

GS_DEV unsigned long long grid_key(float qx, float qy, float qz, const float4 p) {
  const float dx = qx - p.x, dy = qy - p.y, dz = qz - p.z;
  float d = dx * dx;
  d = gs_fma(dy, dy, d);
  d = gs_fma(dz, dz, d);
  return d == d ? knn_pack(d, (uint32_t)__float_as_int(p.w)) : ~0ull;
}

template <int G>
GS_DEV unsigned long long grid_group_min(unsigned long long key) {
#pragma unroll
  for (int d = G / 2; d > 0; d >>= 1) {
    const unsigned long long o = __shfl_xor(key, d, G);
    key = o < key ? o : key;
  }
  return key;
}

struct GsQueryCell {
  float px, py, pz;
  int cx, cy, cz;
};
GS_DEV GsQueryCell grid_query_cell(const GsGrid& g, float qx, float qy, float qz) {
  GsQueryCell c;
  c.px = qx < g.ox ? g.ox : (qx > g.mx ? g.mx : qx);
  c.py = qy < g.oy ? g.oy : (qy > g.my ? g.my : qy);
  c.pz = qz < g.oz ? g.oz : (qz > g.mz ? g.mz : qz);
  c.cx = grid_axis(c.px, g.ox, g.inv_c, g.nx); c.cy = grid_axis(c.py, g.oy, g.inv_c, g.ny);
  c.cz = grid_axis(c.pz, g.oz, g.inv_c, g.nz);
  return c;
}

template <int G>
GS_DEV unsigned long long grid_search_stage0(const GsGrid& g, const int* __restrict__ cell_start,
                                             const float4* __restrict__ sorted, float qx, float qy, float qz, int lane,
                                             bool* resolved, int* win, const float rball = __builtin_inff()) {
  const GsQueryCell qc = grid_query_cell(g, qx, qy, qz);
  const float px = qc.px, py = qc.py, pz = qc.pz;
  const int cx = qc.cx, cy = qc.cy, cz = qc.cz;
  unsigned long long key = ~0ull;
  int bt = -1;
  const float fx = (px - g.ox) * g.inv_c - (float)cx, fy = (py - g.oy) * g.inv_c - (float)cy,
              fz = (pz - g.oz) * g.inv_c - (float)cz;
  const int x0 = (fx < 0.5f) ? cx - 1 : cx, y0 = (fy < 0.5f) ? cy - 1 : cy, z0 = (fz < 0.5f) ? cz - 1 : cz;
  const float BIG = 3.0e38f;
  const float ax = fminf(x0 >= 1 ? fx + (float)(cx - x0) : BIG, x0 + 2 < g.nx ? (float)(x0 + 2 - cx) - fx : BIG);
  const float ay = fminf(y0 >= 1 ? fy + (float)(cy - y0) : BIG, y0 + 2 < g.ny ? (float)(y0 + 2 - cy) - fy : BIG);
  const float az = fminf(z0 >= 1 ? fz + (float)(cz - z0) : BIG, z0 + 2 < g.nz ? (float)(z0 + 2 - cz) - fz : BIG);
  const float amin = fminf(ax, fminf(ay, az));
  const float rc = rball * g.inv_c * 1.0001f + 0.002f;
  const bool prune = rc < amin - 0.001f;
  bool ulx = true, uhx = true, uly = true, uhy = true, ulz = true, uhz = true;
  if (prune) {
    const float tx = fx + (float)(cx - x0), ty = fy + (float)(cy - y0), tz = fz + (float)(cz - z0);
    ulx = tx - rc < 1.0f; uhx = tx + rc >= 1.0f;
    uly = ty - rc < 1.0f; uhy = ty + rc >= 1.0f;
    ulz = tz - rc < 1.0f; uhz = tz + rc >= 1.0f;
  }
  int sb0 = 0, sb1 = 0, sb2 = 0, sb3 = 0, e1 = 0, e2 = 0, e3 = 0, total = 0;
  {
    const int xa = (x0 >= 0 && ulx) ? x0 : x0 + 1, xb = (x0 + 1 < g.nx && uhx) ? x0 + 1 : x0;
    const bool zl = z0 >= 0 && ulz, zh = z0 + 1 < g.nz && uhz, yl = y0 >= 0 && uly, yh = y0 + 1 < g.ny && uhy;
    const int r0 = (z0 * g.ny + y0) * g.nx, r1 = r0 + g.nx, r2 = r0 + g.ny * g.nx, r3 = r2 + g.nx;
    int se0 = 0, se1 = 0, se2 = 0, se3 = 0;
// ... 620 lines not shown
```

gradslam_amd/csrc/gs_knn.hip:

```cpp
#include "gs_knn.h"

#include <stdlib.h>

#include "gs_assoc_dev.h"
#include "gs_env.h"
#include "gs_knn_bbox.h"

constexpr int KNN_BLOCK = 256;
constexpr int KNN_TCHUNK = 512;

template <bool LISTED, int KNN_SPT>
__global__ void __launch_bounds__(KNN_BLOCK) gs_knn1_kernel(
    const float* __restrict__ src_in, const float* __restrict__ Tapply, float* __restrict__ src_out,
    int64_t n_src, const float* __restrict__ tgt, int64_t n_tgt, unsigned long long* __restrict__ best,
    const int* __restrict__ list, const int* __restrict__ count) {
  constexpr int KNN_STILE = KNN_BLOCK * KNN_SPT;
  __shared__ float4 tl[KNN_TCHUNK];
  const int64_t n_q = LISTED ? (int64_t)(*count) : n_src;
  if (LISTED && n_q == 0) return;
  const int64_t j0 = (int64_t)blockIdx.y * KNN_TCHUNK;
  const int cnt = (int)((n_tgt - j0) < KNN_TCHUNK ? (n_tgt - j0) : KNN_TCHUNK);
  if (cnt <= 0) return;
  for (int i = threadIdx.x; i < cnt; i += KNN_BLOCK) {
    const float* t = tgt + 3 * (j0 + i);
// ... 3 lines not shown
  if (Tapply) {
#pragma unroll
    for (int i = 0; i < 12; ++i) T[i] = Tapply[i];
  }
  __syncthreads();
  for (int64_t tile = blockIdx.x; tile * KNN_STILE < n_q; tile += gridDim.x) {
    float sx[KNN_SPT], sy[KNN_SPT], sz[KNN_SPT], bd[KNN_SPT];
    int bi[KNN_SPT];
    int64_t sidx[KNN_SPT];
#pragma unroll
    for (int k = 0; k < KNN_SPT; ++k) {
      const int64_t q = tile * KNN_STILE + k * KNN_BLOCK + threadIdx.x;
      int64_t s = -1;
      if (q < n_q) s = LISTED ? (int64_t)list[q] : q;
      float p0 = 0.0f, p1 = 0.0f, p2 = 0.0f;
      if (s >= 0) {
        p0 = src_in[3 * s];
        p1 = src_in[3 * s + 1];
        p2 = src_in[3 * s + 2];
        if (Tapply) {
          float q0, q1, q2;
          gs_rigid_fma(T, p0, p1, p2, q0, q1, q2);
          p0 = q0; p1 = q1; p2 = q2;
        }
        if (!LISTED && src_out && blockIdx.y == 0) {
          src_out[3 * s] = p0;
          src_out[3 * s + 1] = p1;
          src_out[3 * s + 2] = p2;
        }
      }
      sidx[k] = s;
      sx[k] = p0; sy[k] = p1; sz[k] = p2;
      bd[k] = __builtin_inff();
      bi[k] = 0;
    }
#pragma unroll 4
    for (int j = 0; j < cnt; ++j) {
      const float4 t = tl[j];
#pragma unroll
      for (int k = 0; k < KNN_SPT; ++k) {
        const float dx = sx[k] - t.x, dy = sy[k] - t.y, dz = sz[k] - t.z;
        float d = dx * dx;
        d = gs_fma(dy, dy, d);
        d = gs_fma(dz, dz, d);
        const bool lt = d < bd[k];
        bd[k] = lt ? d : bd[k];
        bi[k] = lt ? j : bi[k];
      }
    }
#pragma unroll
    for (int k = 0; k < KNN_SPT; ++k)
      if (sidx[k] >= 0) atomicMin(&best[sidx[k]], knn_pack(bd[k], (uint32_t)(j0 + bi[k])));
    if (!LISTED) break;
  }
}

int gs_knn_brute_launch(const float* src_in, const float* Tapply, float* src_out, int64_t n_src,
                        const float* tgt, int64_t n_tgt, unsigned long long* best, hipStream_t st) {
  const int spt_env = gs_env().knn_spt;
  const int spt = spt_env == 4 || spt_env == 8 ? spt_env : (n_src * n_tgt >= (int64_t)1 << 27 ? 8 : 4);
  GsProf prof(GS_PROF_KNN, (double)n_src * (double)n_tgt, st);
  if (spt == 8) {
    dim3 grid((unsigned)gs_ceil_div(n_src, KNN_BLOCK * 8), (unsigned)gs_ceil_div(n_tgt, KNN_TCHUNK));
    hipLaunchKernelGGL((gs_knn1_kernel<false, 8>), grid, dim3(KNN_BLOCK), 0, st, src_in, Tapply, src_out, n_src, tgt,
                       n_tgt, best, nullptr, nullptr);
  } else {
    dim3 grid((unsigned)gs_ceil_div(n_src, KNN_BLOCK * 4), (unsigned)gs_ceil_div(n_tgt, KNN_TCHUNK));
    hipLaunchKernelGGL((gs_knn1_kernel<false, 4>), grid, dim3(KNN_BLOCK), 0, st, src_in, Tapply, src_out, n_src, tgt,
                       n_tgt, best, nullptr, nullptr);
  }
  return GS_OK;
}

size_t gs_knn_grid_scratch_bytes(int64_t n_src, int64_t n_tgt) {
  return 512 + 2 * gs_align(4 * (size_t)(GS_GRID_MAXCELL + 1)) + gs_align(4 * (size_t)(GS_GRID_MAXCELL / GS_GRID_TILE + 2)) +
         3 * gs_align(16 * (size_t)(n_tgt > 0 ? n_tgt : 1)) + gs_align(4 * (size_t)(n_src > 0 ? n_src : 1)) + 256;
}

__global__ void __launch_bounds__(GB_BLOCK) gs_grid_bbox_kernel(const float* __restrict__ tgt, GsCount n_tgt_c,
                                                                 const GsTargetFilter flt,
                                                                 unsigned* __restrict__ bbox,
                                                                 int* __restrict__ unres_count,
                                                                 float4* __restrict__ tlist) {
  grid_bbox_body(tgt, gs_count(n_tgt_c), flt, nullptr, 0, 0.0f, 0.0f, nullptr, bbox, unres_count, tlist, blockIdx.x);
}

GS_DEV GsGrid grid_from_bbox(const unsigned* __restrict__ bbox, int64_t n_tgt, int cells_cap) {
  float o[3], m[3];
#pragma unroll
  for (int k = 0; k < 3; ++k) {
    const unsigned cl = bbox[k], ch = bbox[3 + k];
    float a = 0.0f, b = 0.0f;
    if (cl != 0u && ch != 0u) { a = grid_decode(~cl); b = grid_decode(ch); }
    o[k] = a; m[k] = b;
  }
  const float tiny = 1e-6f;
  const float ex = (m[0] - o[0]) + tiny, ey = (m[1] - o[1]) + tiny, ez = (m[2] - o[2]) + tiny;
  const float n = (float)(n_tgt > 0 ? n_tgt : 1);
  const float area = ex * ey + ey * ez + ex * ez;
  float c = 1.5f * sqrtf(area / n);
  const float cv = 0.5f * cbrtf((ex * ey * ez) / n);
  c = cv > c ? cv : c;
  const float emax = ex > ey ? (ex > ez ? ex : ez) : (ey > ez ? ey : ez);
  c = c > emax * (1.0f / 1024.0f) ? c : emax * (1.0f / 1024.0f);
  c = c > 1e-6f ? c : 1e-6f;
  int nx, ny, nz;
  for (;;) {
    nx = (int)(ex / c) + 1; ny = (int)(ey / c) + 1; nz = (int)(ez / c) + 1;
    if ((double)nx * (double)ny * (double)nz <= (double)cells_cap) break;
    c *= 1.26f;
  }
  GsGrid g;
  g.ox = o[0]; g.oy = o[1]; g.oz = o[2];
  g.mx = m[0]; g.my = m[1]; g.mz = m[2];
  g.c = c; g.inv_c = 1.0f / c;
  g.nx = nx; g.ny = ny; g.nz = nz; g.ncell = nx * ny * nz;
  return g;
}

GS_DEV void grid_count_body(const float* __restrict__ tgt, const int64_t n_tgt, const GsTargetFilter flt,
                            const unsigned* __restrict__ bbox, GsGrid* __restrict__ gp, int* __restrict__ cell_count,
                            int* __restrict__ tile_sums, int cells_cap, const float4* __restrict__ tlist,
                            const unsigned blk, const unsigned nblk) {
  __shared__ GsGrid gsh;
  __shared__ int th[GS_GRID_MAXCELL / GS_GRID_TILE + 1];
  const int64_t n_items = flt.pix ? (int64_t)bbox[6] : n_tgt;
  if ((int64_t)blk * 256 >= n_items && blk != 0) return;
  if (threadIdx.x == 0) {
    gsh = grid_from_bbox(bbox, n_items, cells_cap);
    if (blk == 0) *gp = gsh;
  }
  __syncthreads();
  const GsGrid g = gsh;
  const int ntile = g.ncell / GS_GRID_TILE + 1;
  for (int t = threadIdx.x; t < ntile; t += 256) th[t] = 0;
  __syncthreads();
  if (flt.pix) {
    for (int64_t i = (int64_t)blk * 256 + threadIdx.x; i < n_items; i += (int64_t)nblk * 256) {
      const float4 t = tlist[i];
      const int cid = grid_cell(g, t.x, t.y, t.z);
      atomicAdd(&cell_count[cid], 1);
      atomicAdd(&th[cid / GS_GRID_TILE], 1);
    }
  } else {
    const int64_t i = (int64_t)blk * 256 + threadIdx.x;
    if (i < n_tgt) {
      const int cid = grid_cell(g, tgt[3 * i], tgt[3 * i + 1], tgt[3 * i + 2]);
      atomicAdd(&cell_count[cid], 1);
      atomicAdd(&th[cid / GS_GRID_TILE], 1);
    }
  }
  __syncthreads();
  for (int t = threadIdx.x; t < ntile; t += 256) {
    const int v = th[t];
    if (v) atomicAdd(&tile_sums[t], v);
  }
}
__global__ void __launch_bounds__(256) gs_grid_count_kernel(const float* __restrict__ tgt, GsCount n_tgt_c,
                                                            const GsTargetFilter flt,
                                                            const unsigned* __restrict__ bbox,
                                                            GsGrid* __restrict__ gp,
                                                            int* __restrict__ cell_count, int* __restrict__ tile_sums,
                                                            int cells_cap, const float4* __restrict__ tlist) {
  grid_count_body(tgt, gs_count(n_tgt_c), flt, bbox, gp, cell_count, tile_sums, cells_cap, tlist, blockIdx.x, gridDim.x);
}

GS_DEV void grid_scan_body(const int* __restrict__ cell_count, const GsGrid* __restrict__ gp,
                           const int* __restrict__ tile_sums, int* __restrict__ cell_start, const unsigned blk) {
  __shared__ int smem[256 / GS_WAVE + 1];
  const int n = gp->ncell + 1;
  if ((int)(blk * GS_GRID_TILE) >= n) return;
  int pre = 0;
  for (int t = threadIdx.x; t < (int)blk; t += 256) pre += tile_sums[t];
  int tile_prefix;
  (void)gs_block_excl_scan<256>(pre, smem, &tile_prefix);
  const int base = blk * GS_GRID_TILE + threadIdx.x * 4;
  int v[4], c = 0;
#pragma unroll
  for (int i = 0; i < 4; ++i) {
    v[i] = (base + i < n) ? cell_count[base + i] : 0;
    c += v[i];
  }
  int total;
  int run = tile_prefix + gs_block_excl_scan<256>(c, smem, &total);
#pragma unroll
  for (int i = 0; i < 4; ++i) {
    if (base + i < n) cell_start[base + i] = run;
    run += v[i];
  }
}
__global__ void __launch_bounds__(256) gs_grid_scan_kernel(const int* __restrict__ cell_count,
                                                           const GsGrid* __restrict__ gp,
                                                           const int* __restrict__ tile_sums,
                                                           int* __restrict__ cell_start) {
  grid_scan_body(cell_count, gp, tile_sums, cell_start, blockIdx.x);
}

GS_DEV void grid_scatter_body(const float* __restrict__ tgt, const int64_t n_tgt, const GsTargetFilter flt,
                              const GsGrid* __restrict__ gp, const int* __restrict__ cell_start,
                              int* __restrict__ cell_count, float4* __restrict__ sorted,
                              const float4* __restrict__ tlist, const unsigned* __restrict__ bbox,
                              const float* __restrict__ nrm, float4* __restrict__ sorted_n, const unsigned blk,
                              const unsigned nblk) {
  if (flt.pix) {
    const int64_t n_list = (int64_t)bbox[6];
    if ((int64_t)blk * 256 >= n_list) return;
    const GsGrid g = *gp;
    for (int64_t i = (int64_t)blk * 256 + threadIdx.x; i < n_list; i += (int64_t)nblk * 256) {
      const float4 t = tlist[i];
      const int cid = grid_cell(g, t.x, t.y, t.z);
      const int slot = cell_start[cid] + atomicSub(&cell_count[cid], 1) - 1;
      sorted[slot] = t;
      if (nrm) {
        const int64_t r = (int64_t)__float_as_int(t.w);
        sorted_n[slot] = make_float4(nrm[3 * r], nrm[3 * r + 1], nrm[3 * r + 2], 0.0f);
      }
    }
    return;
  }
  const int64_t i = (int64_t)blk * 256 + threadIdx.x;
  if (i >= n_tgt) return;
  const GsGrid g = *gp;
  const float x = tgt[3 * i], y = tgt[3 * i + 1], z = tgt[3 * i + 2];
  const int cid = grid_cell(g, x, y, z);
  const int slot = cell_start[cid] + atomicSub(&cell_count[cid], 1) - 1;
  sorted[slot] = make_float4(x, y, z, __int_as_float((int)i));
  if (nrm) sorted_n[slot] = make_float4(nrm[3 * i], nrm[3 * i + 1], nrm[3 * i + 2], 0.0f);
}
__global__ void __launch_bounds__(256) gs_grid_scatter_kernel(const float* __restrict__ tgt, GsCount n_tgt_c,
                                                              const GsTargetFilter flt,
                                                              const GsGrid* __restrict__ gp,
                                                              const int* __restrict__ cell_start,
                                                              int* __restrict__ cell_count,
                                                              float4* __restrict__ sorted,
                                                              const float4* __restrict__ tlist,
                                                              const unsigned* __restrict__ bbox,
                                                              const float* __restrict__ nrm,
                                                              float4* __restrict__ sorted_n) {
  grid_scatter_body(tgt, gs_count(n_tgt_c), flt, gp, cell_start, cell_count, sorted, tlist, bbox, nrm, sorted_n, blockIdx.x,
                    gridDim.x);
}

__global__ void __launch_bounds__(GB_BLOCK) gs_gridb_bbox_kernel(const GsGridBatch gb, float u_hi, float v_hi) {
  gridb_bbox_block(gb, blockIdx.x, u_hi, v_hi);
}
__global__ void __launch_bounds__(256) gs_gridb_count_kernel(const GsGridBatch gb) {
  const GsGridSeq& q = gb.s[blockIdx.x % gb.B];
  grid_count_body(q.tgt, gs_count(q.n_tgt), GsTargetFilter{q.pix, gb.W, gb.ds}, q.m.bbox, q.m.g, q.m.cell_count,
                  q.m.tile_sums, gb.cells_cap, q.m.tlist, blockIdx.x / gb.B, gridDim.x / gb.B);
}
__global__ void __launch_bounds__(256) gs_gridb_scan_kernel(const GsGridBatch gb) {
  const GsGridSeq& q = gb.s[blockIdx.x % gb.B];
  grid_scan_body(q.m.cell_count, q.m.g, q.m.tile_sums, q.m.cell_start, blockIdx.x / gb.B);
}
__global__ void __launch_bounds__(256) gs_gridb_scatter_kernel(const GsGridBatch gb) {
  const GsGridSeq& q = gb.s[blockIdx.x % gb.B];
  grid_scatter_body(q.tgt, gs_count(q.n_tgt), GsTargetFilter{q.pix, gb.W, gb.ds}, q.m.g, q.m.cell_start, q.m.cell_count,
                    q.m.sorted, q.m.tlist, q.m.bbox, q.nrm, q.m.sorted_n, blockIdx.x / gb.B, gridDim.x / gb.B);
}

static int grid_cells_cap(int64_t n_src, int64_t n_tgt_exact) {
  int64_t want = 48 * n_src;
  if (16 * n_tgt_exact > want) want = 16 * n_tgt_exact;
  int cells_cap = 1 << 20;
  while (cells_cap < GS_GRID_MAXCELL && cells_cap < want) cells_cap <<= 1;
  return cells_cap;
}
int gs_knn_grid_cells_cap(int64_t n_src) { return grid_cells_cap(n_src, 0); }
size_t gs_knn_grid_clear_bytes(const GridMem& m, int cells_cap) {
  return gs_align((size_t)(reinterpret_cast<char*>(m.cell_count) - reinterpret_cast<char*>(m.g)) +
                  4 * (size_t)(cells_cap + 1));
}

int gs_knn_grid_build_batch(const GsGridBatch& gb, hipStream_t st, bool bbox_done) {
  int64_t n_max = 1;
  for (int b = 0; b < gb.B; ++b) n_max = gb.s[b].n_tgt.host > n_max ? gb.s[b].n_tgt.host : n_max;
  const unsigned B = (unsigned)gb.B;
  const float u_hi = (float)((double)gb.W - 0.999), v_hi = (float)((double)gb.H - 0.999);
  if (!bbox_done)
    hipLaunchKernelGGL(gs_gridb_bbox_kernel, dim3(gs_knn_gridb_bbox_blocks(gb)), dim3(GB_BLOCK), 0, st, gb, u_hi, v_hi);
  bool listed = true;
  for (int b = 0; b < gb.B; ++b) listed = listed && gb.s[b].pix != nullptr;
  const int64_t slots = (int64_t)gs_ceil_div(gb.H, gb.ds) * gs_ceil_div(gb.W, gb.ds);
  unsigned nb_pts = (unsigned)gs_ceil_div(n_max, 256);
  if (listed && gb.H > 0 && (unsigned)gs_ceil_div(3 * slots, 256) < nb_pts) nb_pts = (unsigned)gs_ceil_div(3 * slots, 256);
  hipLaunchKernelGGL(gs_gridb_count_kernel, dim3(B * nb_pts), dim3(256), 0, st, gb);
  const unsigned ntile = (unsigned)gs_ceil_div(gb.cells_cap + 1, GS_GRID_TILE);
  hipLaunchKernelGGL(gs_gridb_scan_kernel, dim3(B * ntile), dim3(256), 0, st, gb);
  hipLaunchKernelGGL(gs_gridb_scatter_kernel, dim3(B * nb_pts), dim3(256), 0, st, gb);
  hipError_t e = hipGetLastError();
  if (e != hipSuccess) { gs_set_error("gs_knn_grid_build_batch: %s", hipGetErrorString(e)); return GS_ERR_HIP; }
  return GS_OK;
}

int gs_knn_grid_build(const float* tgt, GsCount n_tgt_c, int64_t n_src, void* grid_scratch, hipStream_t st,
                      GsTargetFilter flt, const float* nrm) {
  const int64_t n_tgt = n_tgt_c.host;
  GridMem m = grid_carve(grid_scratch, n_src, n_tgt);
  const int cells_cap = grid_cells_cap(n_src, n_tgt_c.dev ? 0 : n_tgt);
  GsProf prof(GS_PROF_COMPACT, 28.0 * (double)n_tgt + 8.0 * (double)cells_cap, st);
  const size_t clear = gs_knn_grid_clear_bytes(m, cells_cap);
  hipError_t e = hipMemsetAsync(m.g, 0, clear, st);
  if (e != hipSuccess) { gs_set_error("gs_knn_grid_build: %s", hipGetErrorString(e)); return GS_ERR_HIP; }
  hipLaunchKernelGGL(gs_grid_bbox_kernel, dim3((unsigned)gs_ceil_div(n_tgt > 0 ? n_tgt : 1, GB_BLOCK * GB_ITEMS)),
                     dim3(GB_BLOCK), 0, st, tgt, n_tgt_c, flt, m.bbox, m.unres_count, m.tlist);
  hipLaunchKernelGGL(gs_grid_count_kernel, dim3((unsigned)gs_ceil_div(n_tgt > 0 ? n_tgt : 1, 256)), dim3(256), 0, st,
                     tgt, n_tgt_c, flt, m.bbox, m.g, m.cell_count, m.tile_sums, cells_cap, m.tlist);
  const unsigned ntile = (unsigned)gs_ceil_div(cells_cap + 1, GS_GRID_TILE);
  hipLaunchKernelGGL(gs_grid_scan_kernel, dim3(ntile), dim3(256), 0, st, m.cell_count, m.g, m.tile_sums,
                     m.cell_start);
  hipLaunchKernelGGL(gs_grid_scatter_kernel, dim3((unsigned)gs_ceil_div(n_tgt, 256)), dim3(256), 0, st, tgt,
                     n_tgt_c, flt, m.g, m.cell_start, m.cell_count, m.sorted, m.tlist, m.bbox, nrm, m.sorted_n);
  return GS_OK;
}

constexpr int GQ_BLOCK = 256;

__global__ void __launch_bounds__(GQ_BLOCK) gs_grid_query_kernel(
    const float* __restrict__ src_in, const float* __restrict__ Tapply, float* __restrict__ src_out,
    int64_t n_src, const GsGrid* __restrict__ gp, const int* __restrict__ cell_start,
    const float4* __restrict__ sorted, unsigned long long* __restrict__ best, int* __restrict__ unres_count,
    int* __restrict__ unres_next, int* __restrict__ unres_list) {
  const int lane = threadIdx.x & (GQ_G - 1);
  const int64_t s = ((int64_t)blockIdx.x * GQ_BLOCK + threadIdx.x) / GQ_G;
  if (blockIdx.x == 0 && threadIdx.x == 0) *unres_next = 0;
  if (s >= n_src) return;
  const GsGrid g = *gp;
  float qx = src_in[3 * s], qy = src_in[3 * s + 1], qz = src_in[3 * s + 2];
  if (Tapply) {
    float T[12];
#pragma unroll
    for (int i = 0; i < 12; ++i) T[i] = Tapply[i];
    float t0, t1, t2;
    gs_rigid_fma(T, qx, qy, qz, t0, t1, t2);
    qx = t0; qy = t1; qz = t2;
  }
  if (src_out && lane == 0) {
    src_out[3 * s] = qx;
    src_out[3 * s + 1] = qy;
    src_out[3 * s + 2] = qz;
  }
  bool done;
  const unsigned long long key = grid_search_group(g, cell_start, sorted, qx, qy, qz, lane, &done);
  if (lane == 0) {
    if (done) {
      best[s] = key;
    } else {
      best[s] = ~0ull;
      unres_list[atomicAdd(unres_count, 1)] = (int)s;
    }
  }
}

int gs_knn_grid_query(const float* src_in, const float* Tapply, float* src_out, int64_t n_src,
                      const float* tgt, int64_t n_tgt, unsigned long long* best, void* grid_scratch,
                      hipStream_t st) {
  static unsigned seq = 0;
  GridMem m = grid_carve(grid_scratch, n_src, n_tgt);
  int* cnt = m.unres_count + (seq & 1);
  int* nxt = m.unres_count + ((seq + 1) & 1);
  ++seq;
  GsProf prof(GS_PROF_KNN, (double)n_src * (double)n_tgt, st);
  hipLaunchKernelGGL(gs_grid_query_kernel, dim3((unsigned)gs_ceil_div(n_src * GQ_G, GQ_BLOCK)), dim3(GQ_BLOCK), 0, st,
                     src_in, Tapply, src_out, n_src, m.g, m.cell_start, m.sorted, best, cnt, nxt, m.unres_list);
  unsigned gx = (unsigned)gs_ceil_div(n_src, KNN_BLOCK * 4);
// ... 64 lines not shown
```

gradslam_amd/csrc/gs_knn_bbox.h:

```cpp
#pragma once
#include "gs_assoc_dev.h"
#include "gs_knn.h"

GS_DEV unsigned grid_code(float v) {
  const unsigned b = __float_as_uint(v);
  return (b & 0x80000000u) ? ~b : (b | 0x80000000u);
}
GS_DEV float grid_decode(unsigned c) {
  return __uint_as_float((c & 0x80000000u) ? (c & 0x7fffffffu) : ~c);
}
constexpr int GB_BLOCK = 256;
constexpr int GB_ITEMS = 8;
GS_DEV void grid_bbox_body(const float* __restrict__ tgt, const int64_t n_tgt, const GsTargetFilter flt,
                           const GsCamera* cam, int H, float u_hi, float v_hi, int32_t* __restrict__ pix_out,
                           unsigned* __restrict__ bbox, int* __restrict__ unres_count, float4* __restrict__ tlist,
                           const unsigned blk) {
  if (blk == 0 && threadIdx.x == 0) { unres_count[0] = 0; unres_count[1] = 0; }
  if ((int64_t)blk * GB_BLOCK * GB_ITEMS >= n_tgt) return;
  __shared__ float red[6][GB_BLOCK / GS_WAVE];
  __shared__ int scan_s[GB_BLOCK / GS_WAVE + 1];
  __shared__ unsigned base_s;
  int hits = 0;
  unsigned hitmask = 0;
  float lo[3] = {3.0e38f, 3.0e38f, 3.0e38f}, hi[3] = {-3.0e38f, -3.0e38f, -3.0e38f};
  const int64_t i0 = (int64_t)blk * GB_ITEMS * GB_BLOCK + threadIdx.x;
  if (cam) {
    float v[GB_ITEMS][3];
#pragma unroll
    for (int u = 0; u < GB_ITEMS; ++u) {
      const int64_t i = i0 + (int64_t)u * GB_BLOCK, ic = i < n_tgt ? i : n_tgt - 1;
      v[u][0] = tgt[3 * ic]; v[u][1] = tgt[3 * ic + 1]; v[u][2] = tgt[3 * ic + 2];
    }
#pragma unroll
    for (int u = 0; u < GB_ITEMS; ++u) {
      const int64_t i = i0 + (int64_t)u * GB_BLOCK;
      if (i < n_tgt) {
        int ph = 0, pw = 0;
        const bool in = gs_project_point_hw(*cam, v[u][0], v[u][1], v[u][2], H, flt.W, u_hi, v_hi, ph, pw);
        pix_out[i] = in ? (int32_t)(ph * flt.W + pw) : -1;
        if (in && gs_on_lattice(ph, pw, flt.ds)) {
          ++hits;
          hitmask |= 1u << u;
#pragma unroll
          for (int k = 0; k < 3; ++k) {
            const float w = v[u][k];
            if (w > -3.0e38f && w < 3.0e38f) {
              lo[k] = w < lo[k] ? w : lo[k];
              hi[k] = w > hi[k] ? w : hi[k];
            }
          }
        }
      }
    }
  } else {
    bool t[GB_ITEMS];
    if (flt.pix) {
      int32_t px[GB_ITEMS];
#pragma unroll
      for (int u = 0; u < GB_ITEMS; ++u) {
        const int64_t i = i0 + (int64_t)u * GB_BLOCK;
        px[u] = flt.pix[i < n_tgt ? i : n_tgt - 1];
      }
#pragma unroll
      for (int u = 0; u < GB_ITEMS; ++u) {
        const int32_t p = px[u];
        t[u] = (i0 + (int64_t)u * GB_BLOCK < n_tgt) && p >= 0 && ((p / flt.W) % flt.ds == 0) && ((p % flt.W) % flt.ds == 0);
      }
    } else {
#pragma unroll
      for (int u = 0; u < GB_ITEMS; ++u) t[u] = i0 + (int64_t)u * GB_BLOCK < n_tgt;
    }
#pragma unroll
    for (int u = 0; u < GB_ITEMS; ++u) {
      if (t[u]) {
        const int64_t i = i0 + (int64_t)u * GB_BLOCK;
        ++hits;
        hitmask |= 1u << u;
#pragma unroll
        for (int k = 0; k < 3; ++k) {
          const float w = tgt[3 * i + k];
          if (w > -3.0e38f && w < 3.0e38f) {
            lo[k] = w < lo[k] ? w : lo[k];
            hi[k] = w > hi[k] ? w : hi[k];
          }
        }
      }
    }
  }
  const int lane = threadIdx.x & 63, wave = threadIdx.x >> 6;
#pragma unroll
  for (int k = 0; k < 3; ++k) {
    float a = lo[k], b = hi[k];
#pragma unroll
    for (int d = 32; d > 0; d >>= 1) {
      const float a2 = __shfl_down(a, d, GS_WAVE), b2 = __shfl_down(b, d, GS_WAVE);
      a = a2 < a ? a2 : a;
      b = b2 > b ? b2 : b;
    }
    if (lane == 0) { red[k][wave] = a; red[3 + k][wave] = b; }
  }
  const bool filtered = flt.pix != nullptr || cam != nullptr;
  __syncthreads();
  if (filtered) {
    int total;
    int pos = gs_block_excl_scan<GB_BLOCK>(hits, scan_s, &total);
    if (threadIdx.x == 0 && total) base_s = atomicAdd(&bbox[6], (unsigned)total);
    __syncthreads();
    if (hitmask) {
      const unsigned base = base_s;
#pragma unroll
      for (int u = 0; u < GB_ITEMS; ++u) {
        if (hitmask & (1u << u)) {
          const int64_t i = ((int64_t)blk * GB_ITEMS + u) * GB_BLOCK + threadIdx.x;
          tlist[base + (unsigned)pos] = make_float4(tgt[3 * i], tgt[3 * i + 1], tgt[3 * i + 2], __int_as_float((int)i));
          ++pos;
        }
      }
    }
  }
  if (threadIdx.x < 3) {
    const int k = threadIdx.x;
    float a = red[k][0], b = red[3 + k][0];
    for (int w = 1; w < GB_BLOCK / GS_WAVE; ++w) {
      a = red[k][w] < a ? red[k][w] : a;
      b = red[3 + k][w] > b ? red[3 + k][w] : b;
    }
    if (a <= b) {
      atomicMax(&bbox[k], ~grid_code(a));
      atomicMax(&bbox[3 + k], grid_code(b));
    }
  }
}

GS_DEV void gridb_bbox_block(const GsGridBatch& gb, const unsigned bid, float u_hi, float v_hi) {
  const GsGridSeq& q = gb.s[bid % gb.B];
  const unsigned blk = bid / gb.B;
  const GsTargetFilter flt{q.pix, gb.W, gb.ds};
  if (q.pose16) {
    const GsCamera cam = gs_camera(q.pose16, q.K16);
    grid_bbox_body(q.tgt, gs_count(q.n_tgt), flt, &cam, gb.H, u_hi, v_hi, q.pix, q.m.bbox, q.m.unres_count, q.m.tlist,
                   blk);
  } else {
    grid_bbox_body(q.tgt, gs_count(q.n_tgt), flt, nullptr, 0, 0.0f, 0.0f, nullptr, q.m.bbox, q.m.unres_count, q.m.tlist,
                   blk);
  }
}
static inline unsigned gs_knn_gridb_bbox_blocks(const GsGridBatch& gb) {
  int64_t n_max = 1;
  for (int b = 0; b < gb.B; ++b) n_max = gb.s[b].n_tgt.host > n_max ? gb.s[b].n_tgt.host : n_max;
  return (unsigned)gb.B * (unsigned)gs_ceil_div(n_max, GB_BLOCK * GB_ITEMS);
}
```

gradslam_amd/ops.py:

```python
import collections
import os

import torch

from . import _C
from ._C import Workspace, check, lib, ptr, require_device, stream

f32 = torch.float32

DEVICE_COUNTS = os.environ.get("GRADSLAM_HIP_DEVICE_COUNTS", "1") != "0"


def _thresh(dist_thresh):
    if dist_thresh is None:
        return -1.0
    return max(float(dist_thresh), 0.0)


def two_sigma_sq(sigma):
    if torch.is_tensor(sigma):
        sigma = float(sigma)
    return float(torch.tensor(2 * (float(sigma) ** 2), dtype=torch.float64).to(torch.float32))


# ... 602 lines not shown


def _batch_view(t, inner_ndim):
    if t.dtype != f32:
        t = t.to(f32)
    inner = t.shape[t.ndim - inner_ndim:]
    want, acc = [], 1
    for d in reversed(inner):
        want.append(acc)
        acc *= int(d)
    if tuple(t.stride()[t.ndim - inner_ndim:]) != tuple(reversed(want)) or (t.shape[0] > 1 and t.stride(0) < acc):
        t = t.contiguous()
    return t, t.data_ptr(), (t.stride(0) if t.shape[0] > 1 else acc) * 4


def _map_view(bufs, cap, n_bound, n_dev):
    P, N, Cc, F = bufs
    return _C.MapView(P.data_ptr(), N.data_ptr(), 0 if Cc is None else Cc.data_ptr(), 0 if F is None else F.data_ptr(),
                      int(cap), int(n_bound), 0 if n_dev is None else n_dev.data_ptr())


def localize_batch(vertex, depth, K, prev_poses, maps, ds, mode=1, numiters=20, damp=1e-8, dist_thresh=None,
                   lambda_max=2.0, B=1.0, B2=1.0, nu=200.0, out=None):
    K, prev_poses = _c(K), _c(prev_poses)
    Bn, H, W = depth.shape
    vertex, v0, vs = _batch_view(vertex, 3)
    depth, d0, dstr = _batch_view(depth, 2)
    dev = require_device(K, prev_poses)
    if vertex.device != dev or depth.device != dev or not vertex.is_cuda:
        raise _C.HipExtensionError("gradslam_amd kernels run on the GPU only; all tensors on one device")
    T = torch.empty((Bn, 4, 4), dtype=f32, device=dev) if out is None else out
    assert T.shape == (Bn, 4, 4) and T.dtype == f32 and T.is_contiguous() and T.device == dev
    prm = _C.IcpParams(int(mode), int(numiters), float(damp), _thresh(dist_thresh), float(lambda_max), float(B),
                       float(B2), float(nu))
    ws = Workspace.get(dev)
    seqs = (_C.LocalizeSeq * Bn)()
    L = lib()
    k0, p0, t0 = K.data_ptr(), prev_poses.data_ptr(), T.data_ptr()
    for b in range(Bn):
        P, N, n_bound, n_dev = maps[b]
        require_device(P, N, n_dev)
        if P.dtype != f32 or N.dtype != f32 or N.shape[0] < P.shape[0]:
            raise _C.HipExtensionError("localize_batch needs float32 map points / normals on buffers of equal capacity "
                                       "(got %s / %s, %d / %d rows)" % (P.dtype, N.dtype, P.shape[0], N.shape[0]))
        cap = P.shape[0]
        scratch = ws.bytes("localize%d" % b, L.gs_localize_scratch_bytes(H, W, int(ds), cap))
        q = seqs[b]
        q.vertex, q.depth, q.K16, q.prev_pose16 = v0 + b * vs, d0 + b * dstr, k0 + b * 64, p0 + b * 64
        q.map = _map_view((P, N, None, None), cap, n_bound, n_dev)
        q.out_pose16, q.scratch = t0 + b * 64, scratch.data_ptr()
    check(L.gs_localize_batch_f32(seqs, Bn, H, W, int(ds), prm, stream(dev)), "gs_localize_batch_f32")
    return T


def localize_far_stats(device, b, H, W, ds, capacity):
    L = lib()
    scratch = Workspace.get(device).bytes("localize%d" % b, L.gs_localize_scratch_bytes(H, W, int(ds), int(capacity)))
    import ctypes
    out = (ctypes.c_int64 * 4)()
    check(L.gs_localize_far_stats_i64(scratch.data_ptr(), H, W, int(ds), int(capacity), out, stream(device)),
          "gs_localize_far_stats_i64")
    return tuple(int(v) for v in out)


def localize_list_stats(device, b, H, W, ds, capacity):
    L = lib()
    scratch = Workspace.get(device).bytes("localize%d" % b, L.gs_localize_scratch_bytes(H, W, int(ds), int(capacity)))
    import ctypes
    out = (ctypes.c_int64 * 192)()
    check(L.gs_localize_list_stats_i64(scratch.data_ptr(), H, W, int(ds), int(capacity), out, stream(device)),
          "gs_localize_list_stats_i64")
    v = [int(x) for x in out]
    return v[:64], v[64:128], v[128:]


def localize_solve_stats(device, b, H, W, ds, capacity):
    L = lib()
    scratch = Workspace.get(device).bytes("localize%d" % b, L.gs_localize_scratch_bytes(H, W, int(ds), int(capacity)))
    import ctypes
    out = (ctypes.c_int64 * 8)()
    check(L.gs_localize_solve_stats_i64(scratch.data_ptr(), H, W, int(ds), int(capacity), out, stream(device)),
          "gs_localize_solve_stats_i64")
    return dict(zip(("ticket", "arrived", "error", "weak", "nb", "h0"), (int(x) for x in out[:6])))


def update_map_fusion_batch_(maps, vertex, normal, depth, rgb, alpha, poses, K, dist_th, dot_th, renorm_all=True,
                             out=None):
    poses, K = _c(poses), _c(K)
    dev = require_device(poses, K)
    Bn, H, W = depth.shape
    views = [_batch_view(t, nd) for t, nd in ((vertex, 3), (normal, 3), (depth, 2), (rgb, 3), (alpha, 2))]
    if any(v[0].device != dev for v in views):
        raise _C.HipExtensionError("gradslam_amd kernels run on the GPU only; all tensors on one device")
    gv, gn = out if out is not None else (torch.empty((Bn, H, W, 3), dtype=f32, device=dev),
                                          torch.empty((Bn, H, W, 3), dtype=f32, device=dev))
    gviews = [_batch_view(t, 3) for t in (gv, gn)]
    assert gviews[0][0] is gv and gviews[1][0] is gn, "output global maps must have contiguous (H, W, 3) slices"
    best = torch.empty((Bn, H * W), dtype=torch.int32, device=dev)
    cnt = torch.empty(Bn, dtype=torch.int64, device=dev)
    ws = Workspace.get(dev)
    seqs = (_C.UpdateSeq * Bn)()
    L = lib()
    P1 = H * W * 4
    base = [t.data_ptr() for t in (poses, K, best, cnt)]
    for b in range(Bn):
        P, N, Cc, F, n_bound, n_dev = maps[b]
        require_device(P, N, Cc, F, n_dev)
        cap = P.shape[0]
        scratch = ws.bytes("map_update%d" % b, L.gs_update_map_scratch_bytes(cap, H, W))
        u = seqs[b]
        u.map = _map_view((P, N, Cc, F), cap, n_bound, n_dev)
        u.vertex, u.normal, u.depth, u.rgb, u.alpha = (v[1] + b * v[2] for v in views)
        u.pose16, u.K16 = base[0] + b * 64, base[1] + b * 64
        u.gvertex, u.gnormal = gviews[0][1] + b * gviews[0][2], gviews[1][1] + b * gviews[1][2]
        u.best_pix, u.new_count_out, u.scratch = base[2] + b * P1, base[3] + b * 8, scratch.data_ptr()
    check(L.gs_update_map_fusion_batch_f32(seqs, Bn, H, W, float(dist_th), float(dot_th), 1 if renorm_all else 0,
                                           stream(dev)), "gs_update_map_fusion_batch_f32")
    return cnt, gv, gn, best


RenderedViews = collections.namedtuple("RenderedViews", ["depth", "color", "normal", "confidence", "index"])


def render_map_batch(maps, poses, K, H, W, radius=0, min_confidence=0.0, cull_backfaces=False, out=None,
                     differentiable=False, guard=None):
    if differentiable:
        if out is not None:
            raise ValueError("render_map: out= cannot be combined with differentiable=True (autograd owns the outputs)")
        if len(maps) != int(poses.shape[0]) or K.ndim != 3 or K.shape[0] != len(maps):
            raise ValueError("render_map: expected poses (B, L, 4, 4) and K (B, 4, 4) for B = %d maps; got %s and %s"
                             % (len(maps), tuple(poses.shape), tuple(K.shape)))
        poses = poses.to(f32)
        per = [RenderMapFunction.apply(m[0], m[1], m[2], m[3], poses[b], K[b].detach(), m[4], m[5], int(H), int(W),
                                       int(radius), float(min_confidence), bool(cull_backfaces), guard)
               for b, m in enumerate(maps)]
        if any((per[0][i] is None) != (r[i] is None) for r in per for i in range(5)):
            raise ValueError("render_map: every map of a batch must carry the same attributes")
        return RenderedViews(*[None if per[0][i] is None else
                               (per[0][i].unsqueeze(0) if len(per) == 1 else torch.stack([r[i] for r in per]))
                               for i in range(5)])
    _warn_detached("render_map", poses, K, *[t for m in maps for t in m[:4]])
    poses, K = _c(poses.detach()), _c(K.detach())
    dev = require_device(poses, K)
    Bn, Lv = int(poses.shape[0]), int(poses.shape[1])
    H, W = int(H), int(W)
    if len(maps) != Bn or tuple(poses.shape[2:]) != (4, 4) or tuple(K.shape) != (Bn, 4, 4):
        raise ValueError("render_map: expected poses (B, L, 4, 4) and K (B, 4, 4) for B = %d maps; got %s and %s"
                         % (len(maps), tuple(poses.shape), tuple(K.shape)))
    if Lv == 0 or H <= 0 or W <= 0:
        raise ValueError("render_map: needs at least one view and a positive image size")
    held = [tuple(None if t is None else _c(t.detach()) for t in m[:4]) for m in maps]
    have = [all(h[i] is not None for h in held) for i in range(4)]
    if not have[0]:
        raise ValueError("render_map: a map without points")
    shapes = ((Bn, Lv, H, W, 1), (Bn, Lv, H, W, 3), (Bn, Lv, H, W, 3), (Bn, Lv, H, W, 1), (Bn, Lv, H, W))
    wanted = (True, have[2], have[1], have[3], True)
    imgs = []
    for i, (shape, want) in enumerate(zip(shapes, wanted)):
        t = None if out is None else out[i]
        if t is None and want:
            t = torch.empty(shape, dtype=torch.int64 if i == 4 else f32, device=dev)
        elif t is not None:
            if not want:
                raise ValueError("render_map: out.%s given but the maps lack the attribute it shows" % RenderedViews._fields[i])
            if tuple(t.shape) != shape or t.dtype != (torch.int64 if i == 4 else f32) or not t.is_contiguous():
                raise ValueError("render_map: out.%s must be a contiguous %s tensor of shape %s"
# ... 310 lines not shown
```

include/gradslam_hip.h:

```cpp
#ifndef GRADSLAM_HIP_H
#define GRADSLAM_HIP_H

#include <stdint.h>

#ifdef __cplusplus
extern "C" {
#endif

#define GS_API __attribute__((visibility("default")))

#define GS_OK 0
#define GS_ERR_INVALID 1
#define GS_ERR_HIP 2
#define GS_ERR_CAPACITY 3

GS_API int gs_abi_version(void);
GS_API const char* gs_last_error(void);
GS_API int64_t gs_scratch_bytes(int64_t n_map, int64_t n_pix);

GS_API int gs_profile_begin(int max_records);
GS_API int gs_profile_end(void);
GS_API int gs_profile_read(int kind, double* ms_total, int64_t* launches, double* work_total);

GS_API int gs_frame_maps_f32(const float* depth, const float* K16, int H, int W, float two_sigma_sq,
// ... 147 lines not shown
                                 float* out_pts, void* stream);

GS_API int gs_ingest_depth_u16_f32(const uint16_t* raw, int H0, int W0, float* out, int H, int W,
                                   double scale_div, void* stream);
GS_API int gs_ingest_color_u8_f32(const uint8_t* raw, int H0, int W0, float* out, int H, int W, int normalize,
                                  void* stream);
GS_API int gs_ingest_frames_native_f32(const uint16_t* depth_raw, const uint8_t* color_raw, int64_t n_frames, int H, int W,
                                       double scale_div, int normalize, float* depth_out, float* color_out, void* stream);
GS_API int gs_host_device_pointer(const void* host_ptr, void** dev_ptr_out);

GS_API int gs_project_map_dc_f32(const float* points, int64_t n_map_bound, const int64_t* n_map_dev,
                                 const float* pose16, const float* K16, int H, int W, int32_t* pix,
                                 void* stream);
GS_API int gs_select_targets_dc_f32(const int32_t* pix, int64_t n_map_bound, const int64_t* n_map_dev, int W,
                                    int ds, const float* points, const float* normals, const float* colors,
                                    float* out_pts, float* out_nrm, float* out_rgb, int64_t cap,
                                    int64_t* count_out, void* scratch, void* stream);
GS_API int gs_associate_dc_f32(const int32_t* pix, int64_t n_map_bound, const int64_t* n_map_dev,
                               const float* points, const float* normals, const float* ccounts,
                               const float* gvertex, const float* gnormal, int H, int W, float dist_th,
                               float dot_th, int32_t* best_pix, uint8_t* similar, void* scratch, void* stream);
GS_API int gs_fuse_append_dc_f32(float* points, float* normals, float* colors, float* ccounts,
                                 int64_t n_map_bound, const int64_t* n_map_dev, int64_t capacity,
                                 const int32_t* best_pix, const float* gvertex, const float* gnormal,
                                 const float* rgb, const float* alpha, const float* depth, int H, int W,
                                 int renorm_all, int64_t* new_count_out, void* scratch, void* stream);
GS_API int gs_append_valid_dc_f32(float* points, float* normals, float* colors, float* ccounts,
                                  int64_t n_map_bound, const int64_t* n_map_dev, int64_t capacity,
                                  const float* gvertex, const float* gnormal, const float* rgb,
                                  const float* alpha, const float* depth, int H, int W,
                                  int64_t* new_count_out, void* scratch, void* stream);

GS_API int gs_fuse_append_backward_f32(const float* points, const float* normals, const float* colors,
                                       const float* ccounts, int64_t n_old, const int32_t* best_pix,
                                       const float* gvertex, const float* gnormal, const float* rgb,
                                       const float* alpha, const float* depth, int H, int W, int renorm_all,
                                       const float* P_bar, const float* N_bar, const float* C_bar,
                                       const float* F_bar, int64_t n_new, float* old_points_bar,
                                       float* old_normals_bar, float* old_colors_bar, float* old_ccounts_bar,
                                       float* gvertex_bar, float* gnormal_bar, float* rgb_bar, float* alpha_bar,
                                       void* scratch, void* stream);

GS_API int64_t gs_update_map_scratch_bytes(int64_t n_map_bound, int H, int W);
GS_API int gs_update_map_fusion_dc_f32(float* points, float* normals, float* colors, float* ccounts,
                                       int64_t n_map_bound, const int64_t* n_map_dev, int64_t capacity,
                                       const float* vertex, const float* normal, const float* depth,
                                       const float* rgb, const float* alpha, const float* pose16, const float* K16,
                                       int H, int W, float dist_th, float dot_th, int renorm_all, float* gvertex,
                                       float* gnormal, int32_t* best_pix, int64_t* new_count_out, void* scratch,
                                       void* stream);

typedef struct gs_map_view {
  float* points;
  float* normals;
  float* colors;
  float* ccounts;
  int64_t capacity;
  int64_t n_bound;
  const int64_t* n_dev;
} gs_map_view;

GS_API int gs_frame_maps_batch_f32(const float* depth, int64_t depth_stride_seq, int64_t depth_stride_frame,
                                   const float* K16, int n_frames, int frames_per_K, int H, int W, float two_sigma_sq,
                                   float* vertex, float* normal, float* alpha, void* stream);

typedef struct gs_localize_seq {
  const float* vertex;
  const float* depth;
  const float* K16;
  const float* prev_pose16;
  gs_map_view map;
  float* out_pose16;
  void* scratch;
} gs_localize_seq;
GS_API int64_t gs_localize_scratch_bytes(int H, int W, int ds, int64_t n_map_bound);
GS_API int gs_localize_batch_f32(const gs_localize_seq* seqs_host, int B, int H, int W, int ds,
                                 const gs_icp_params* params_host, void* stream);
GS_API int gs_localize_far_stats_i64(const void* scratch, int H, int W, int ds, int64_t map_rows, int64_t* out4_host,
                                     void* stream);
GS_API int gs_localize_list_stats_i64(const void* scratch, int H, int W, int ds, int64_t map_rows, int64_t* out192_host,
                                      void* stream);
GS_API int gs_localize_solve_stats_i64(const void* scratch, int H, int W, int ds, int64_t map_rows, int64_t* out8_host,
                                       void* stream);

typedef struct gs_update_seq {
  gs_map_view map;
  const float* vertex;
  const float* normal;
  const float* depth;
  const float* rgb;
  const float* alpha;
  const float* pose16;
  const float* K16;
  float* gvertex;
  float* gnormal;
  int32_t* best_pix;
  int64_t* new_count_out;
  void* scratch;
} gs_update_seq;
GS_API int gs_update_map_fusion_batch_f32(const gs_update_seq* seqs_host, int B, int H, int W, float dist_th,
                                          float dot_th, int renorm_all, void* stream);

typedef struct gs_step_seq {
  const float* depth;
  const float* rgb;
  const float* K16;
  const float* prev_pose16;
  float* out_pose16;
  float* vertex;
  float* normal;
  float* alpha;
  float* gvertex;
  float* gnormal;
  int32_t* best_pix;
  int64_t* new_count_out;
  gs_map_view map;
  void* loc_scratch;
  void* upd_scratch;
} gs_step_seq;
GS_API int gs_pointfusion_step_batch_f32(const gs_step_seq* seqs_host, int B, int H, int W, int ds,
                                         const gs_icp_params* params_host, float two_sigma_sq, float dist_th,
                                         float dot_th, int renorm_all, void* stream);

GS_API int gs_project_points_f32(const float* cam_coords, int cdim, int64_t n, const float* proj16, int64_t pts_per_mat,
                                 float* out_uv, void* stream);
GS_API int gs_unproject_points_f32(const float* pixel_coords, int pdim, int64_t n, const float* kinv9,
                                   int64_t pts_per_mat, const float* depths, float* out_xyz, void* stream);
GS_API int gs_lie_small_f32(int op, const float* in, float* out, void* stream);

typedef struct gs_render_seq {
  gs_map_view map;
  const float* poses16;
  const float* K16;
  float* depth;
  float* color;
  float* normal;
  float* confidence;
  int64_t* index;
  void* scratch;
} gs_render_seq;
GS_API int64_t gs_render_scratch_bytes(int views, int H, int W);
GS_API int gs_render_map_dc_f32(const gs_render_seq* seqs_host, int B, int L, int H, int W, int radius,
                                float min_confidence, int cull_backfaces, void* stream);

typedef struct gs_render_backward_seq {
  gs_map_view map;
  const float* poses16;
  const float* K16;
  const int64_t* index;
  const float* depth_bar;
  const float* color_bar;
  const float* normal_bar;
  const float* confidence_bar;
  float* points_bar;
  float* normals_bar;
  float* colors_bar;
  float* ccounts_bar;
  float* poses_bar;
  void* scratch;
} gs_render_backward_seq;
GS_API int64_t gs_render_backward_scratch_bytes(int views, int H, int W, int64_t n_bound);
GS_API int gs_render_map_backward_dc_f32(const gs_render_backward_seq* seqs_host, int B, int L, int H, int W,
                                         int radius, void* stream);

#ifdef __cplusplus
}
// ... 3 lines not shown
```

Before: 3669.

## Add grid-stride map passes and drop per-row pixel buffer in localize bbox

Turns the map-row kernels (fusion project-key, merge, and grid bbox) into grid-stride loops whose block count comes from a new helper that can cap blocks per CU or take an env override. The default per-CU constant is zero, so the block count still equals the full need. Localization no longer writes a per-map-row pixel index array, because the target list is driven by a new 'listed' flag. A debug export for reading the target list is also added. The main intended saving is the dropped pixel-array stores and its scratch, at the cost of templated bbox code with more branching.

```diff
diff --git a/gradslam_amd/_C.py b/gradslam_amd/_C.py
--- a/gradslam_amd/_C.py
+++ b/gradslam_amd/_C.py
@@ -137,6 +137,7 @@
     "gs_localize_far_stats_i64": [_vp, _i32, _i32, _i32, _i64, C.POINTER(C.c_int64), _vp],
     "gs_localize_list_stats_i64": [_vp, _i32, _i32, _i32, _i64, C.POINTER(C.c_int64), _vp],
     "gs_localize_solve_stats_i64": [_vp, _i32, _i32, _i32, _i64, C.POINTER(C.c_int64), _vp],
+    "gs_localize_targets_f32": [_vp, _i32, _i32, _i32, _i64, C.POINTER(C.c_uint32), _vp, _i64, _vp],
     "gs_pointfusion_step_batch_f32": [C.POINTER(StepSeq), _i32, _i32, _i32, _i32, C.POINTER(IcpParams), _f, _f, _f, _i32, _vp],
     "gs_render_scratch_bytes": [_i32, _i32, _i32],
     "gs_render_map_dc_f32": [C.POINTER(RenderSeq), _i32, _i32, _i32, _i32, _i32, _f, _i32, _vp],
diff --git a/gradslam_amd/csrc/gs_common.h b/gradslam_amd/csrc/gs_common.h
--- a/gradslam_amd/csrc/gs_common.h
+++ b/gradslam_amd/csrc/gs_common.h
@@ -31,6 +31,9 @@
                                     int renorm_all, void* stream, bool tables_ready);
 int32_t* gs_update_map_call_flag(void* scratch_of_first_sequence);
 void gs_update_map_tables(void* scratch, int32_t** any_flag, uint64_t** key_pix);
+
+constexpr int GS_MAP_PASS_BLOCKS_PER_CU = 0;
+unsigned gs_map_pass_blocks(int B, int64_t rows_bound, int rows_per_block);
 
 void gs_set_error(const char* fmt, ...);
 
diff --git a/gradslam_amd/csrc/gs_env.h b/gradslam_amd/csrc/gs_env.h
--- a/gradslam_amd/csrc/gs_env.h
+++ b/gradslam_amd/csrc/gs_env.h
@@ -13,6 +13,7 @@
   bool icp_lanes_set;
   int icp_lanes;
   int icp_blocks_per_cu;
+  int map_pass_blocks;
   const char* icp_timeline;
   const char* icp_persist_timeline;
   bool icp_timeline_it_set; int icp_timeline_it;
@@ -38,6 +39,7 @@
     v.icp_lanes_set = getenv("GRADSLAM_HIP_ICP_LANES") != nullptr;
     v.icp_lanes = num("GRADSLAM_HIP_ICP_LANES", 0);
     v.icp_blocks_per_cu = num("GRADSLAM_HIP_ICP_BLOCKS_PER_CU", 0);
+    v.map_pass_blocks = num("GRADSLAM_HIP_MAP_PASS_BLOCKS", 0);
     v.icp_timeline = getenv("GRADSLAM_HIP_ICP_TIMELINE");
     v.icp_persist_timeline = getenv("GRADSLAM_HIP_ICP_PERSIST_TIMELINE");
     v.icp_timeline_it_set = getenv("GRADSLAM_HIP_ICP_TIMELINE_IT") != nullptr;
diff --git a/gradslam_amd/csrc/gs_fuse.hip b/gradslam_amd/csrc/gs_fuse.hip
--- a/gradslam_amd/csrc/gs_fuse.hip
+++ b/gradslam_amd/csrc/gs_fuse.hip
@@ -419,30 +419,38 @@
   q.best_pix[p] = -1;
 }
 
+template <class Frame>
+GS_DEV void mu_key_rows(const MuBatch& mb, const MuSeq& q, const GsCamera& c, const Frame& frame, const int64_t n_map,
+                        const unsigned blk, const unsigned nblk) {
+  for (int64_t n = (int64_t)blk * 256 + threadIdx.x; n < n_map; n += (int64_t)nblk * 256) {
+    const int32_t p = gs_project_point(c, q.points[3 * n], q.points[3 * n + 1], q.points[3 * n + 2], mb.H, mb.W, mb.u_hi,
+                                       mb.v_hi);
+    int32_t pk = -1;
+    if (p >= 0) {
+      float fp[3], fn[3];
+      frame((int64_t)p, fp, fn);
+      if (gs_is_similar_v(q.points, q.normals, fp, fn, n, mb.dist_th, mb.dot_th)) {
+        const uint64_t k = gs_assoc_key_v(q.points, q.ccounts, fp, n);
+        const unsigned long long old = atomicMin(reinterpret_cast<unsigned long long*>(&q.key_pix[p]), (unsigned long long)k);
+        if (old == (unsigned long long)k) {
+          q.best_pix[p] = MU_TIE_MARK;
+          q.any_flag[1] = 1;
+        }
+        q.key_pt[n] = k;
+        pk = p;
+      }
+    }
+    q.pix[n] = pk;
+  }
+}
 __global__ void __launch_bounds__(256) gs_mu_project_key_kernel(const MuBatch mb) {
   const MuSeq& q = mb.s[blockIdx.x % mb.B];
-  const int64_t n = (int64_t)(blockIdx.x / mb.B) * 256 + threadIdx.x;
-  if (n >= gs_count(q.n_map)) return;
+  const unsigned blk = blockIdx.x / mb.B, nblk = gridDim.x / mb.B;
+  const int64_t n_map = gs_count(q.n_map);
+  if ((int64_t)blk * 256 >= n_map) return;
   const GsCamera c = gs_camera(q.pose16, q.K16);
-  const int32_t p = gs_project_point(c, q.points[3 * n], q.points[3 * n + 1], q.points[3 * n + 2], mb.H, mb.W, mb.u_hi,
-                                     mb.v_hi);
-  int32_t pk = -1;
-  if (p >= 0) {
-    float fp[3], fn[3];
-    if (q.gvertex) FrameGlobalMaps{q.gvertex, q.gnormal}((int64_t)p, fp, fn);
-    else frame_local_maps(q.vertex, q.normal, q.pose16)((int64_t)p, fp, fn);
-    if (gs_is_similar_v(q.points, q.normals, fp, fn, n, mb.dist_th, mb.dot_th)) {
-      const uint64_t k = gs_assoc_key_v(q.points, q.ccounts, fp, n);
-      const unsigned long long old = atomicMin(reinterpret_cast<unsigned long long*>(&q.key_pix[p]), (unsigned long long)k);
-      if (old == (unsigned long long)k) {
-        q.best_pix[p] = MU_TIE_MARK;
-        q.any_flag[1] = 1;
-      }
-      q.key_pt[n] = k;
-      pk = p;
-    }
-  }
-  q.pix[n] = pk;
+  if (q.gvertex) mu_key_rows(mb, q, c, FrameGlobalMaps{q.gvertex, q.gnormal}, n_map, blk, nblk);
+  else mu_key_rows(mb, q, c, frame_local_maps(q.vertex, q.normal, q.pose16), n_map, blk, nblk);
 }
 
 GS_DEV void mu_settle_ties(const MuSeq& q, const unsigned blk, const unsigned nblk) {
@@ -489,24 +497,32 @@
   mu_settle_ties(q, blk, gridDim.x / mb.B);
 }
 
-GS_DEV void mu_merge_body(const MuBatch& mb, const unsigned bid) {
+template <class Frame>
+GS_DEV void mu_merge_rows(const MuBatch& mb, const MuSeq& q, const Frame& frame, const int64_t n_map, const unsigned blk,
+                          const unsigned nblk) {
+  for (int64_t n = (int64_t)blk * 256 + threadIdx.x; n < n_map; n += (int64_t)nblk * 256) {
+    int32_t p = q.pix[n];
+    if (p >= 0) {
+      bool win = q.key_pt[n] == q.key_pix[p];
+      if (win) {
+        const int32_t bp = q.best_pix[p];
+        win = bp == -1 || bp == (int32_t)n;
+        if (win && bp == -1) q.best_pix[p] = (int32_t)n;
+      }
+      if (!win) p = -1;
+    }
+    if (p < 0 && !mb.renorm_all) continue;
+    fuse_merge_row(q.points, q.normals, q.colors, q.ccounts, n, p, frame, q.rgb, q.alpha);
+  }
+}
+GS_DEV void mu_merge_body(const MuBatch& mb, const unsigned bid, const unsigned nblk) {
   const MuSeq& q = mb.s[bid % mb.B];
-  const int64_t n = (int64_t)(bid / mb.B) * 256 + threadIdx.x;
-  if (n >= gs_count(q.n_map)) return;
+  const unsigned blk = bid / mb.B;
+  const int64_t n_map = gs_count(q.n_map);
+  if ((int64_t)blk * 256 >= n_map) return;
   if (*mb.call_flag == 0) return;
-  int32_t p = q.pix[n];
-  if (p >= 0) {
-    bool win = q.key_pt[n] == q.key_pix[p];
-    if (win) {
-      const int32_t bp = q.best_pix[p];
-      win = bp == -1 || bp == (int32_t)n;
-      if (win && bp == -1) q.best_pix[p] = (int32_t)n;
-    }
-    if (!win) p = -1;
-  }
-  if (p < 0 && !mb.renorm_all) return;
-  if (q.gvertex) fuse_merge_row(q.points, q.normals, q.colors, q.ccounts, n, p, FrameGlobalMaps{q.gvertex, q.gnormal}, q.rgb, q.alpha);
-  else fuse_merge_row(q.points, q.normals, q.colors, q.ccounts, n, p, frame_local_maps(q.vertex, q.normal, q.pose16), q.rgb, q.alpha);
+  if (q.gvertex) mu_merge_rows(mb, q, FrameGlobalMaps{q.gvertex, q.gnormal}, n_map, blk, nblk);
+  else mu_merge_rows(mb, q, frame_local_maps(q.vertex, q.normal, q.pose16), n_map, blk, nblk);
 }
 
 GS_DEV void mu_append_body(const MuBatch& mb, const unsigned bid) {
@@ -569,7 +585,7 @@
 static_assert(GS_CP_BLOCK == 256, "merge and append blocks share a launch");
 __global__ void __launch_bounds__(256) gs_mu_merge_append_kernel(const MuBatch mb, const unsigned nb_append) {
   if (blockIdx.x < nb_append) mu_append_body(mb, blockIdx.x);
-  else mu_merge_body(mb, blockIdx.x - nb_append);
+  else mu_merge_body(mb, blockIdx.x - nb_append, (gridDim.x - nb_append) / mb.B);
 }
 
 extern "C" int64_t gs_update_map_scratch_bytes(int64_t n_map_bound, int H, int W) {
@@ -618,7 +634,7 @@
     bytes_fuse += 104.0 * (double)n_map + 49.0 * (double)mb.P;
   }
   const unsigned uB = (unsigned)B;
-  const unsigned pb = uB * (unsigned)gs_ceil_div(mb.P, 256), nb = uB * (unsigned)gs_ceil_div(n_max > 0 ? n_max : 1, 256);
+  const unsigned pb = uB * (unsigned)gs_ceil_div(mb.P, 256), nb = uB * gs_map_pass_blocks(B, n_max, 256);
   if (phase == 0) {
     if (!tables_ready) {
       GsProf prof(GS_PROF_FRAME, (double)B * (double)mb.P * 64.0, st);
diff --git a/gradslam_amd/csrc/gs_icp_loop.hip b/gradslam_amd/csrc/gs_icp_loop.hip
--- a/gradslam_amd/csrc/gs_icp_loop.hip
+++ b/gradslam_amd/csrc/gs_icp_loop.hip
@@ -765,6 +765,15 @@
   });
   return facts[dev];
 }
+unsigned gs_map_pass_blocks(int B, int64_t rows_bound, int rows_per_block) {
+  const int forced = gs_env().map_pass_blocks;
+  const int64_t need0 = gs_ceil_div(rows_bound > 0 ? rows_bound : 1, rows_per_block);
+  int64_t cap = forced > 0 ? forced
+                : (GS_MAP_PASS_BLOCKS_PER_CU > 0 ? (int64_t)icp_device().cus * GS_MAP_PASS_BLOCKS_PER_CU / (B > 0 ? B : 1) : need0);
+  cap = cap > 0 ? cap : 1;
+  const int64_t need = gs_ceil_div(rows_bound > 0 ? rows_bound : 1, rows_per_block);
+  return (unsigned)(need < cap ? need : cap);
+}
 
 struct IcpHalfPlan { int G, nb, upb; };
 static IcpHalfPlan icp_half_plan(const GsEnv& env, int cus, int64_t n_src, int B, int g_max = 8) {
@@ -1005,7 +1014,7 @@
                    int64_t n_tgt, const float* init16, const float* compose16,
                    const gs_icp_params* prm, float* out_T16, int64_t* out_idx, void* icp_scratch,
                    void* tape, void* stream, const int64_t* n_src_dev = nullptr,
-                   const int64_t* n_tgt_dev = nullptr, GsTargetFilter flt = GsTargetFilter{nullptr, 1, 1}) {
+                   const int64_t* n_tgt_dev = nullptr, GsTargetFilter flt = GsTargetFilter{nullptr, 1, 1, 0}) {
   GS_REQUIRE(prm, "params_host must not be NULL");
   GS_REQUIRE(n_src > 0 && n_tgt > 0, "empty point set");
   GS_REQUIRE(n_tgt < 0x7fffffffll && n_src < 0x7fffffffll, "too many points");
@@ -1142,7 +1151,7 @@
                                  void* icp_scratch, void* stream) {
   GS_REQUIRE(pix && W > 0 && ds > 0, "bad target filter");
   return icp_run(src, n_src_bound, map_points, map_normals, n_map_bound, init16, compose16, prm, out_T16, nullptr,
-                 icp_scratch, nullptr, stream, n_src_dev, n_map_dev, GsTargetFilter{pix, W, ds});
+                 icp_scratch, nullptr, stream, n_src_dev, n_map_dev, gs_target_filter(pix, W, ds));
 }
 
 
@@ -1231,7 +1240,7 @@
                                                                const float u_hi, const float v_hi) {
   const unsigned n_prep = (unsigned)lb.B * nb_lat;
   if (blockIdx.x < n_prep) loc_prep_block(lb, blockIdx.x, nb_lat);
-  else gridb_bbox_block(gb, blockIdx.x - n_prep, u_hi, v_hi);
+  else gridb_bbox_block(gb, blockIdx.x - n_prep, (gridDim.x - n_prep) / gb.B, u_hi, v_hi);
 }
 
 struct IcpRowsBatch {
@@ -1369,14 +1378,13 @@
 struct LocLayout {
   int64_t n_lat, rows;
   IcpLayout sc;
-  size_t lattice, pix, n_valid, icp, lq, ls, lstat, far_c, far_cq, far_idx, far_n, far_out4, total;
+  size_t lattice, n_valid, icp, lq, ls, lstat, far_c, far_cq, far_idx, far_n, far_out4, total;
 };
 static LocLayout loc_layout(int64_t n_lat, int64_t rows) {
   GsTake take;
   LocLayout L;
   L.n_lat = n_lat; L.rows = rows > 0 ? rows : 1;
   L.lattice = take(gs_align(12 * (size_t)n_lat));
-  L.pix = take(gs_align(4 * (size_t)L.rows));
   L.n_valid = take(256);
   L.sc = icp_layout(n_lat, L.rows);
   L.icp = take(L.sc.total);
@@ -1400,13 +1408,13 @@
 }
 
 struct LocCarve {
-  float* lattice; int32_t* pix; int64_t* n_valid;
+  float* lattice; int64_t* n_valid;
   IcpScratch sc; GridMem gm; ListMem lm;
   FarMem fm; int* far_out4;
 };
 static LocCarve loc_carve(void* p, const LocLayout& L) {
   const IcpScratch sc = icp_carve(gs_at<char>(p, L.icp), L.sc);
-  return LocCarve{gs_at<float>(p, L.lattice), gs_at<int32_t>(p, L.pix), gs_at<int64_t>(p, L.n_valid), sc,
+  return LocCarve{gs_at<float>(p, L.lattice), gs_at<int64_t>(p, L.n_valid), sc,
                   grid_carve(sc.grid, L.n_lat, L.rows),
                   ListMem{gs_at<float4>(p, L.lq), gs_at<uint32_t>(p, L.ls), gs_at<int>(p, L.lstat)},
                   FarMem{gs_at<uint32_t>(p, L.far_c), gs_at<float4>(p, L.far_cq), gs_at<int>(p, L.far_idx), gs_at<int>(p, L.far_n)},
@@ -1463,7 +1471,7 @@
     lb.s[b] = LocSeq{q.vertex, q.depth, q.prev_pose16, c[b].lattice, c[b].sc.state, q.out_pose16,
                      reinterpret_cast<char*>(c[b].gm.g), c[b].n_valid, c[b].fm.n, c[b].lm.stat,
                      plan.wide_on ? c[b].fm.cq : nullptr, c[b].sc.sync};
-    gb.s[b] = GsGridSeq{q.map.points, GsCount{q.map.n_bound, q.map.n_dev}, c[b].pix, q.prev_pose16, q.K16,
+    gb.s[b] = GsGridSeq{q.map.points, GsCount{q.map.n_bound, q.map.n_dev}, nullptr, q.prev_pose16, q.K16,
                         plan.binned_normals ? q.map.normals : nullptr, c[b].gm};
   }
   lb.count_valid = g_gs_prof_on ? 1 : 0;
@@ -1697,6 +1705,21 @@
   return GS_OK;
 }
 
+extern "C" int gs_localize_targets_f32(const void* scratch, int H, int W, int ds, int64_t map_rows, uint32_t* bbox7_host,
+                                       float* targets_out, int64_t cap, void* stream) {
+  GS_REQUIRE(scratch && bbox7_host && H > 0 && W > 0 && ds > 0 && map_rows > 0 && cap >= 0, "bad arguments");
+  GS_REQUIRE(targets_out || cap == 0, "NULL pointer");
+  const GridMem gm = loc_carve_of(scratch, H, W, ds, map_rows).gm;
+  hipStream_t st = gs_stream(stream);
+  GS_HIP(hipMemcpyAsync(bbox7_host, gm.bbox, 7 * sizeof(uint32_t), hipMemcpyDeviceToHost, st));
+  GS_HIP(hipStreamSynchronize(st));
+  int64_t n = (int64_t)bbox7_host[6];
+  n = n < cap ? n : cap;
+  n = n < map_rows ? n : map_rows;
+  if (n > 0) GS_HIP(hipMemcpyAsync(targets_out, gm.tlist, 16 * (size_t)n, hipMemcpyDeviceToDevice, st));
+  return GS_OK;
+}
+
 extern "C" int gs_pointfusion_step_batch_f32(const gs_step_seq* seqs_host, int B, int H, int W, int ds,
                                              const gs_icp_params* prm, float two_sigma_sq, float dist_th, float dot_th,
                                              int renorm_all, void* stream) {
diff --git a/gradslam_amd/csrc/gs_knn.h b/gradslam_amd/csrc/gs_knn.h
--- a/gradslam_amd/csrc/gs_knn.h
+++ b/gradslam_amd/csrc/gs_knn.h
@@ -22,11 +22,10 @@
 struct GsTargetFilter {
   const int32_t* pix;
   int W, ds;
+  int listed;
 };
-GS_DEV bool gs_is_target(const GsTargetFilter& f, int64_t n) {
-  if (!f.pix) return true;
-  const int32_t p = f.pix[n];
-  return p >= 0 && ((p / f.W) % f.ds == 0) && ((p % f.W) % f.ds == 0);
+static inline GsTargetFilter gs_target_filter(const int32_t* pix, int W, int ds) {
+  return GsTargetFilter{pix, W, ds, pix != nullptr ? 1 : 0};
 }
 
 struct GridMem {
@@ -75,12 +74,16 @@
   int cells_cap;
   GsGridSeq s[GS_MAX_BATCH];
 };
+static inline __host__ __device__ bool gs_gridb_listed(const GsGridSeq& q) { return q.pix != nullptr || q.pose16 != nullptr; }
+static inline __host__ __device__ GsTargetFilter gs_gridb_filter(const GsGridBatch& gb, const GsGridSeq& q) {
+  return GsTargetFilter{q.pix, gb.W, gb.ds, gs_gridb_listed(q) ? 1 : 0};
+}
 int gs_knn_grid_cells_cap(int64_t n_src);
 size_t gs_knn_grid_clear_bytes(const GridMem& m, int cells_cap);
 int gs_knn_grid_build_batch(const GsGridBatch& gb, hipStream_t st, bool bbox_done = false);
 
 int gs_knn_grid_build(const float* tgt, GsCount n_tgt, int64_t n_src, void* grid_scratch, hipStream_t st,
-                      GsTargetFilter filter = GsTargetFilter{nullptr, 1, 1}, const float* nrm = nullptr);
+                      GsTargetFilter filter = GsTargetFilter{nullptr, 1, 1, 0}, const float* nrm = nullptr);
 int gs_knn_grid_query(const float* src_in, const float* Tapply, float* src_out, int64_t n_src,
                       const float* tgt, int64_t n_tgt, unsigned long long* best, void* grid_scratch,
                       hipStream_t st);
diff --git a/gradslam_amd/csrc/gs_knn.hip b/gradslam_amd/csrc/gs_knn.hip
--- a/gradslam_amd/csrc/gs_knn.hip
+++ b/gradslam_amd/csrc/gs_knn.hip
@@ -109,7 +109,8 @@
                                                                  unsigned* __restrict__ bbox,
                                                                  int* __restrict__ unres_count,
                                                                  float4* __restrict__ tlist) {
-  grid_bbox_body(tgt, gs_count(n_tgt_c), flt, nullptr, 0, 0.0f, 0.0f, nullptr, bbox, unres_count, tlist, blockIdx.x);
+  grid_bbox_body<false>(tgt, gs_count(n_tgt_c), flt, GsCamera{}, 0, 0.0f, 0.0f, nullptr, bbox, unres_count, tlist,
+                        blockIdx.x, gridDim.x);
 }
 
 GS_DEV GsGrid grid_from_bbox(const unsigned* __restrict__ bbox, int64_t n_tgt, int cells_cap) {
@@ -151,7 +152,7 @@
                             const unsigned blk, const unsigned nblk) {
   __shared__ GsGrid gsh;
   __shared__ int th[GS_GRID_MAXCELL / GS_GRID_TILE + 1];
-  const int64_t n_items = flt.pix ? (int64_t)bbox[6] : n_tgt;
+  const int64_t n_items = flt.listed ? (int64_t)bbox[6] : n_tgt;
   if ((int64_t)blk * 256 >= n_items && blk != 0) return;
   if (threadIdx.x == 0) {
     gsh = grid_from_bbox(bbox, n_items, cells_cap);
@@ -162,7 +163,7 @@
   const int ntile = g.ncell / GS_GRID_TILE + 1;
   for (int t = threadIdx.x; t < ntile; t += 256) th[t] = 0;
   __syncthreads();
-  if (flt.pix) {
+  if (flt.listed) {
     for (int64_t i = (int64_t)blk * 256 + threadIdx.x; i < n_items; i += (int64_t)nblk * 256) {
       const float4 t = tlist[i];
       const int cid = grid_cell(g, t.x, t.y, t.z);
@@ -229,7 +230,7 @@
                               const float4* __restrict__ tlist, const unsigned* __restrict__ bbox,
                               const float* __restrict__ nrm, float4* __restrict__ sorted_n, const unsigned blk,
                               const unsigned nblk) {
-  if (flt.pix) {
+  if (flt.listed) {
     const int64_t n_list = (int64_t)bbox[6];
     if ((int64_t)blk * 256 >= n_list) return;
     const GsGrid g = *gp;
@@ -269,11 +270,11 @@
 }
 
 __global__ void __launch_bounds__(GB_BLOCK) gs_gridb_bbox_kernel(const GsGridBatch gb, float u_hi, float v_hi) {
-  gridb_bbox_block(gb, blockIdx.x, u_hi, v_hi);
+  gridb_bbox_block(gb, blockIdx.x, gridDim.x / gb.B, u_hi, v_hi);
 }
 __global__ void __launch_bounds__(256) gs_gridb_count_kernel(const GsGridBatch gb) {
   const GsGridSeq& q = gb.s[blockIdx.x % gb.B];
-  grid_count_body(q.tgt, gs_count(q.n_tgt), GsTargetFilter{q.pix, gb.W, gb.ds}, q.m.bbox, q.m.g, q.m.cell_count,
+  grid_count_body(q.tgt, gs_count(q.n_tgt), gs_gridb_filter(gb, q), q.m.bbox, q.m.g, q.m.cell_count,
                   q.m.tile_sums, gb.cells_cap, q.m.tlist, blockIdx.x / gb.B, gridDim.x / gb.B);
 }
 __global__ void __launch_bounds__(256) gs_gridb_scan_kernel(const GsGridBatch gb) {
@@ -282,7 +283,7 @@
 }
 __global__ void __launch_bounds__(256) gs_gridb_scatter_kernel(const GsGridBatch gb) {
   const GsGridSeq& q = gb.s[blockIdx.x % gb.B];
-  grid_scatter_body(q.tgt, gs_count(q.n_tgt), GsTargetFilter{q.pix, gb.W, gb.ds}, q.m.g, q.m.cell_start, q.m.cell_count,
+  grid_scatter_body(q.tgt, gs_count(q.n_tgt), gs_gridb_filter(gb, q), q.m.g, q.m.cell_start, q.m.cell_count,
                     q.m.sorted, q.m.tlist, q.m.bbox, q.nrm, q.m.sorted_n, blockIdx.x / gb.B, gridDim.x / gb.B);
 }
 
@@ -307,7 +308,7 @@
   if (!bbox_done)
     hipLaunchKernelGGL(gs_gridb_bbox_kernel, dim3(gs_knn_gridb_bbox_blocks(gb)), dim3(GB_BLOCK), 0, st, gb, u_hi, v_hi);
   bool listed = true;
-  for (int b = 0; b < gb.B; ++b) listed = listed && gb.s[b].pix != nullptr;
+  for (int b = 0; b < gb.B; ++b) listed = listed && gs_gridb_listed(gb.s[b]);
   const int64_t slots = (int64_t)gs_ceil_div(gb.H, gb.ds) * gs_ceil_div(gb.W, gb.ds);
   unsigned nb_pts = (unsigned)gs_ceil_div(n_max, 256);
   if (listed && gb.H > 0 && (unsigned)gs_ceil_div(3 * slots, 256) < nb_pts) nb_pts = (unsigned)gs_ceil_div(3 * slots, 256);
diff --git a/gradslam_amd/csrc/gs_knn_bbox.h b/gradslam_amd/csrc/gs_knn_bbox.h
--- a/gradslam_amd/csrc/gs_knn_bbox.h
+++ b/gradslam_amd/csrc/gs_knn_bbox.h
@@ -11,39 +11,78 @@
 }
 constexpr int GB_BLOCK = 256;
 constexpr int GB_ITEMS = 8;
+template <bool CAM>
 GS_DEV void grid_bbox_body(const float* __restrict__ tgt, const int64_t n_tgt, const GsTargetFilter flt,
-                           const GsCamera* cam, int H, float u_hi, float v_hi, int32_t* __restrict__ pix_out,
+                           const GsCamera& cam, int H, float u_hi, float v_hi, int32_t* __restrict__ pix_out,
                            unsigned* __restrict__ bbox, int* __restrict__ unres_count, float4* __restrict__ tlist,
-                           const unsigned blk) {
+                           const unsigned blk, const unsigned nblk) {
   if (blk == 0 && threadIdx.x == 0) { unres_count[0] = 0; unres_count[1] = 0; }
-  if ((int64_t)blk * GB_BLOCK * GB_ITEMS >= n_tgt) return;
+  constexpr int64_t CHUNK = (int64_t)GB_BLOCK * GB_ITEMS;
+  if ((int64_t)blk * CHUNK >= n_tgt) return;
   __shared__ float red[6][GB_BLOCK / GS_WAVE];
   __shared__ int scan_s[GB_BLOCK / GS_WAVE + 1];
   __shared__ unsigned base_s;
-  int hits = 0;
-  unsigned hitmask = 0;
+  const bool filtered = flt.listed != 0;
   float lo[3] = {3.0e38f, 3.0e38f, 3.0e38f}, hi[3] = {-3.0e38f, -3.0e38f, -3.0e38f};
-  const int64_t i0 = (int64_t)blk * GB_ITEMS * GB_BLOCK + threadIdx.x;
-  if (cam) {
-    float v[GB_ITEMS][3];
+  for (int64_t chunk = blk; chunk * CHUNK < n_tgt; chunk += nblk) {
+    int hits = 0;
+    unsigned hitmask = 0;
+    const int64_t i0 = chunk * CHUNK + threadIdx.x;
+    if (CAM) {
+      float v[GB_ITEMS][3];
 #pragma unroll
-    for (int u = 0; u < GB_ITEMS; ++u) {
-      const int64_t i = i0 + (int64_t)u * GB_BLOCK, ic = i < n_tgt ? i : n_tgt - 1;
-      v[u][0] = tgt[3 * ic]; v[u][1] = tgt[3 * ic + 1]; v[u][2] = tgt[3 * ic + 2];
-    }
+      for (int u = 0; u < GB_ITEMS; ++u) {
+        const int64_t i = i0 + (int64_t)u * GB_BLOCK, ic = i < n_tgt ? i : n_tgt - 1;
+        v[u][0] = tgt[3 * ic]; v[u][1] = tgt[3 * ic + 1]; v[u][2] = tgt[3 * ic + 2];
+      }
 #pragma unroll
-    for (int u = 0; u < GB_ITEMS; ++u) {
-      const int64_t i = i0 + (int64_t)u * GB_BLOCK;
-      if (i < n_tgt) {
-        int ph = 0, pw = 0;
-        const bool in = gs_project_point_hw(*cam, v[u][0], v[u][1], v[u][2], H, flt.W, u_hi, v_hi, ph, pw);
-        pix_out[i] = in ? (int32_t)(ph * flt.W + pw) : -1;
-        if (in && gs_on_lattice(ph, pw, flt.ds)) {
+      for (int u = 0; u < GB_ITEMS; ++u) {
+        const int64_t i = i0 + (int64_t)u * GB_BLOCK;
+        if (i < n_tgt) {
+          int ph = 0, pw = 0;
+          const bool in = gs_project_point_hw(cam, v[u][0], v[u][1], v[u][2], H, flt.W, u_hi, v_hi, ph, pw);
+          if (pix_out) pix_out[i] = in ? (int32_t)(ph * flt.W + pw) : -1;
+          if (in && gs_on_lattice(ph, pw, flt.ds)) {
+            ++hits;
+            hitmask |= 1u << u;
+#pragma unroll
+            for (int k = 0; k < 3; ++k) {
+              const float w = v[u][k];
+              if (w > -3.0e38f && w < 3.0e38f) {
+                lo[k] = w < lo[k] ? w : lo[k];
+                hi[k] = w > hi[k] ? w : hi[k];
+              }
+            }
+          }
+        }
+      }
+    } else {
+      bool t[GB_ITEMS];
+      if (flt.pix) {
+        int32_t px[GB_ITEMS];
+#pragma unroll
+        for (int u = 0; u < GB_ITEMS; ++u) {
+          const int64_t i = i0 + (int64_t)u * GB_BLOCK;
+          px[u] = flt.pix[i < n_tgt ? i : n_tgt - 1];
+        }
+#pragma unroll
+        for (int u = 0; u < GB_ITEMS; ++u) {
+          const int32_t p = px[u];
+          t[u] = (i0 + (int64_t)u * GB_BLOCK < n_tgt) && p >= 0 && ((p / flt.W) % flt.ds == 0) && ((p % flt.W) % flt.ds == 0);
+        }
+      } else {
+#pragma unroll
+        for (int u = 0; u < GB_ITEMS; ++u) t[u] = i0 + (int64_t)u * GB_BLOCK < n_tgt;
+      }
+#pragma unroll
+      for (int u = 0; u < GB_ITEMS; ++u) {
+        if (t[u]) {
+          const int64_t i = i0 + (int64_t)u * GB_BLOCK;
           ++hits;
           hitmask |= 1u << u;
 #pragma unroll
           for (int k = 0; k < 3; ++k) {
-            const float w = v[u][k];
+            const float w = tgt[3 * i + k];
             if (w > -3.0e38f && w < 3.0e38f) {
               lo[k] = w < lo[k] ? w : lo[k];
               hi[k] = w > hi[k] ? w : hi[k];
@@ -52,36 +91,19 @@
         }
       }
     }
-  } else {
-    bool t[GB_ITEMS];
-    if (flt.pix) {
-      int32_t px[GB_ITEMS];
+    if (filtered) {
+      int total;
+      int pos = gs_block_excl_scan<GB_BLOCK>(hits, scan_s, &total);
+      if (threadIdx.x == 0 && total) base_s = atomicAdd(&bbox[6], (unsigned)total);
+      __syncthreads();
+      if (hitmask) {
+        const unsigned base = base_s;
 #pragma unroll
-      for (int u = 0; u < GB_ITEMS; ++u) {
-        const int64_t i = i0 + (int64_t)u * GB_BLOCK;
-        px[u] = flt.pix[i < n_tgt ? i : n_tgt - 1];
-      }
-#pragma unroll
-      for (int u = 0; u < GB_ITEMS; ++u) {
-        const int32_t p = px[u];
-        t[u] = (i0 + (int64_t)u * GB_BLOCK < n_tgt) && p >= 0 && ((p / flt.W) % flt.ds == 0) && ((p % flt.W) % flt.ds == 0);
-      }
-    } else {
-#pragma unroll
-      for (int u = 0; u < GB_ITEMS; ++u) t[u] = i0 + (int64_t)u * GB_BLOCK < n_tgt;
-    }
-#pragma unroll
-    for (int u = 0; u < GB_ITEMS; ++u) {
-      if (t[u]) {
-        const int64_t i = i0 + (int64_t)u * GB_BLOCK;
-        ++hits;
-        hitmask |= 1u << u;
-#pragma unroll
-        for (int k = 0; k < 3; ++k) {
-          const float w = tgt[3 * i + k];
-          if (w > -3.0e38f && w < 3.0e38f) {
-            lo[k] = w < lo[k] ? w : lo[k];
-            hi[k] = w > hi[k] ? w : hi[k];
+        for (int u = 0; u < GB_ITEMS; ++u) {
+          if (hitmask & (1u << u)) {
+            const int64_t i = i0 + (int64_t)u * GB_BLOCK;
+            tlist[base + (unsigned)pos] = make_float4(tgt[3 * i], tgt[3 * i + 1], tgt[3 * i + 2], __int_as_float((int)i));
+            ++pos;
           }
         }
       }
@@ -99,25 +121,7 @@
     }
     if (lane == 0) { red[k][wave] = a; red[3 + k][wave] = b; }
   }
-  const bool filtered = flt.pix != nullptr || cam != nullptr;
   __syncthreads();
-  if (filtered) {
-    int total;
-    int pos = gs_block_excl_scan<GB_BLOCK>(hits, scan_s, &total);
-    if (threadIdx.x == 0 && total) base_s = atomicAdd(&bbox[6], (unsigned)total);
-    __syncthreads();
-    if (hitmask) {
-      const unsigned base = base_s;
-#pragma unroll
-      for (int u = 0; u < GB_ITEMS; ++u) {
-        if (hitmask & (1u << u)) {
-          const int64_t i = ((int64_t)blk * GB_ITEMS + u) * GB_BLOCK + threadIdx.x;
-          tlist[base + (unsigned)pos] = make_float4(tgt[3 * i], tgt[3 * i + 1], tgt[3 * i + 2], __int_as_float((int)i));
-          ++pos;
-        }
-      }
-    }
-  }
   if (threadIdx.x < 3) {
     const int k = threadIdx.x;
     float a = red[k][0], b = red[3 + k][0];
@@ -132,21 +136,21 @@
   }
 }
 
-GS_DEV void gridb_bbox_block(const GsGridBatch& gb, const unsigned bid, float u_hi, float v_hi) {
+GS_DEV void gridb_bbox_block(const GsGridBatch& gb, const unsigned bid, const unsigned nblk, float u_hi, float v_hi) {
   const GsGridSeq& q = gb.s[bid % gb.B];
   const unsigned blk = bid / gb.B;
-  const GsTargetFilter flt{q.pix, gb.W, gb.ds};
+  const GsTargetFilter flt = gs_gridb_filter(gb, q);
   if (q.pose16) {
     const GsCamera cam = gs_camera(q.pose16, q.K16);
-    grid_bbox_body(q.tgt, gs_count(q.n_tgt), flt, &cam, gb.H, u_hi, v_hi, q.pix, q.m.bbox, q.m.unres_count, q.m.tlist,
-                   blk);
+    grid_bbox_body<true>(q.tgt, gs_count(q.n_tgt), flt, cam, gb.H, u_hi, v_hi, q.pix, q.m.bbox, q.m.unres_count,
+                         q.m.tlist, blk, nblk);
   } else {
-    grid_bbox_body(q.tgt, gs_count(q.n_tgt), flt, nullptr, 0, 0.0f, 0.0f, nullptr, q.m.bbox, q.m.unres_count, q.m.tlist,
-                   blk);
+    grid_bbox_body<false>(q.tgt, gs_count(q.n_tgt), flt, GsCamera{}, 0, 0.0f, 0.0f, nullptr, q.m.bbox, q.m.unres_count,
+                          q.m.tlist, blk, nblk);
   }
 }
 static inline unsigned gs_knn_gridb_bbox_blocks(const GsGridBatch& gb) {
   int64_t n_max = 1;
   for (int b = 0; b < gb.B; ++b) n_max = gb.s[b].n_tgt.host > n_max ? gb.s[b].n_tgt.host : n_max;
-  return (unsigned)gb.B * (unsigned)gs_ceil_div(n_max, GB_BLOCK * GB_ITEMS);
+  return (unsigned)gb.B * gs_map_pass_blocks(gb.B, n_max, GB_BLOCK * GB_ITEMS);
 }
diff --git a/gradslam_amd/ops.py b/gradslam_amd/ops.py
--- a/gradslam_amd/ops.py
+++ b/gradslam_amd/ops.py
@@ -708,6 +708,19 @@
     check(L.gs_localize_solve_stats_i64(scratch.data_ptr(), H, W, int(ds), int(capacity), out, stream(device)),
           "gs_localize_solve_stats_i64")
     return dict(zip(("ticket", "arrived", "error", "weak", "nb", "h0"), (int(x) for x in out[:6])))
+
+
+def localize_targets(device, b, H, W, ds, capacity):
+    L = lib()
+    scratch = Workspace.get(device).bytes("localize%d" % b, L.gs_localize_scratch_bytes(H, W, int(ds), int(capacity)))
+    import ctypes
+    import numpy as np
+    words = (ctypes.c_uint32 * 7)()
+    out = torch.empty((int(capacity), 4), dtype=f32, device=device)
+    check(L.gs_localize_targets_f32(scratch.data_ptr(), H, W, int(ds), int(capacity), words, out.data_ptr(), int(capacity),
+                                    stream(device)), "gs_localize_targets_f32")
+    w = np.array(list(words), dtype=np.uint32)
+    return w, out[:min(int(w[6]), int(capacity))]
 
 
 def update_map_fusion_batch_(maps, vertex, normal, depth, rgb, alpha, poses, K, dist_th, dot_th, renorm_all=True,
diff --git a/include/gradslam_hip.h b/include/gradslam_hip.h
--- a/include/gradslam_hip.h
+++ b/include/gradslam_hip.h
@@ -253,6 +253,8 @@
                                       void* stream);
 GS_API int gs_localize_solve_stats_i64(const void* scratch, int H, int W, int ds, int64_t map_rows, int64_t* out8_host,
                                        void* stream);
+GS_API int gs_localize_targets_f32(const void* scratch, int H, int W, int ds, int64_t map_rows, uint32_t* bbox7_host,
+                                   float* targets_out, int64_t cap, void* stream);
 
 typedef struct gs_update_seq {
   gs_map_view map;
```

After: 3344. 0.911x the previous value.
